# LongAoTianxia/Quantized_ViT

Hardware: AMD Instinct MI355X
Metric: images/sec ViT-B/16 int4 @224 batch 256; % int8-MFMA roofline (higher is better)
Workload: dtype int8; 1 GPU; vit_base_patch16_224 int4w/int8a forward, batch 256 per GPU; model=vit_base_patch16_224, global_batch=256, seq_len=197, parallelism=dp1

## Files before the change

### include/qvit_hip.h

```cpp
#ifndef QVIT_HIP_H
#define QVIT_HIP_H

#include <stdint.h>
#include <hip/hip_runtime_api.h>

#ifdef __cplusplus
extern "C" {
#endif

#define QVIT_OK          0
#define QVIT_EINVAL     -1
#define QVIT_EALIGN     -2
#define QVIT_ENULL      -3
#define QVIT_EHIP    -1000

#define QVIT_QT_LINEAR      0
#define QVIT_QT_NONLINEAR   1
#define QVIT_QT_ULTRA_ACT   2

#define QVIT_W4 4
#define QVIT_W8 8
#define QVIT_W4R 40
#define QVIT_W8R 80
#define QVIT_W16 16
#define QVIT_W24 24

#define QVIT_EPI_F32        0
#define QVIT_EPI_F32_RESID  1
#define QVIT_EPI_I8_GELU    2
#define QVIT_EPI_I8         3
#define QVIT_EPI_I32        4
#define QVIT_EPI_QKV_SPLIT  5

#define QVIT_ULTRA_CODES       0
#define QVIT_ULTRA_CODES_POOL  1
#define QVIT_ULTRA_F32         2

#define QVIT_ATT_F32        0
#define QVIT_ATT_I8         1

#define QVIT_U8_NCHW 0
#define QVIT_U8_NHWC 1

#define QVIT_TILE_N  256
#define QVIT_TILE_K  128

const char* qvit_strerror(int code);
const char* qvit_version(void);

int qvit_quantize_act_i8(const float* x, int64_t rows, int64_t cols, int64_t ldx,
                         int qtype, const float* d_quant, const float* q_m, const float* t_quant,
                         int levels, int8_t* codes, int64_t ldc, int64_t kpad, hipStream_t stream);

int qvit_fake_quant_f32(const float* x, int64_t n, int qtype, const float* d_quant,
                        const float* q_m, const float* t_quant, int levels, float* y,
                        hipStream_t stream);

int64_t qvit_quant_backward_workspace_bytes(int64_t n);
int qvit_quant_backward(const float* x, const float* grad_out, int64_t n, int qtype,
                        const float* d_quant, const float* q_m, const float* t_quant,
                        float clip_lo, float clip_hi, float dge_k,
                        float* grad_x, float* grad_scalars ,
                        void* workspace, int64_t workspace_bytes, hipStream_t stream);

int64_t qvit_quant_error_workspace_bytes(int64_t rows, int64_t cols, int ncand);
int qvit_quant_error(const float* x, int64_t rows, int64_t cols, int64_t ldx, int qtype, const float* d,
                     const float* q_m, const float* t, int ncand, int accumulate, double* err, int64_t* nclip,
                     void* workspace, int64_t workspace_bytes, hipStream_t stream);

#define QVIT_QAT_SGD    0
#define QVIT_QAT_ADAM   1
#define QVIT_QAT_ADAMW  2
#define QVIT_QAT_WARMUP 0
#define QVIT_QAT_RANGE  1
#define QVIT_QAT_FIX    2
int qvit_qat_step(const void* tensors, int ntensors, const void* chunks, int64_t nchunks, int variant,
                  int first_step, float lr, float lr_quant, float first_momentum, float second_momentum,
                  float alpha1, float alpha2, float weight_decay, float bias_correction1, float bias_correction2,
                  float clip_lo, float clip_hi, hipStream_t stream);
int qvit_qat_quant_step(const void* quants, int nquants, int32_t* bits, int stage, int first_fix, int variant,
                        int first_step, float lr, float lr_quant, float first_momentum, float second_momentum,
                        float alpha1, float alpha2, float weight_decay, float bias_correction1,
                        float bias_correction2, float clip_lo, float clip_hi, int min_bit_wt, int max_bit_wt,
                        int min_bit_act, int max_bit_act, hipStream_t stream);

int qvit_prune_scores(const void* groups, int ngroups, const void* members, int nmembers, const void* items,
                      int64_t nitems, double* sums, int variant, int first_step, float lr, float lr_quant,
                      float first_momentum, float second_momentum, float alpha1, float alpha2, float weight_decay,
                      float bias_correction1, float bias_correction2, float clip_lo, float clip_hi,
                      hipStream_t stream);
int qvit_prune_scores_fold(const void* groups, int ngroups, const void* items, int64_t nitems, const double* sums,
                           const void* units, int64_t nunits, double* unit_sums, hipStream_t stream);
int qvit_prune_scores_finish(const void* groups, int ngroups, const void* items, int64_t nitems, const double* sums,
                             double w_magnitude, double w_avg_magnitude, double w_cosine, double w_taylor1,
                             double w_taylor2, float* scores, hipStream_t stream);
int qvit_prune_joint_scalars(const void* quants, int nquants, int variant, int first_step, float lr, float lr_quant,
                             float first_momentum, float second_momentum, float alpha1, float alpha2,
                             float weight_decay, float bias_correction1, float bias_correction2, float clip_lo,
                             float clip_hi, int min_bit_act, int max_bit_act, hipStream_t stream);
int qvit_prune_joint_reduce(const void* groups, int ngroups, const void* members, int nmembers, const void* items,
                            int64_t nitems, double* partials, int variant, int first_step, float lr, float lr_quant,
                            float first_momentum, float second_momentum, float alpha1, float alpha2,
                            float weight_decay, float bias_correction1, float bias_correction2, float clip_lo,
                            float clip_hi, hipStream_t stream);
int qvit_prune_joint_finish(const void* groups, int ngroups, const double* partials, int64_t npartials, double lr,
                            int period, int t_in_period, int min_bit_wt, int max_bit_wt, float* gamma, int32_t* info,
                            hipStream_t stream);
int qvit_prune_joint_apply(const void* groups, int ngroups, const void* members, int nmembers, const void* items,
                           int64_t nitems, const float* gamma, int variant, int first_step, float lr, float lr_quant,
                           float first_momentum, float second_momentum, float alpha1, float alpha2,
                           float weight_decay, float bias_correction1, float bias_correction2, float clip_lo,
                           float clip_hi, hipStream_t stream);

int qvit_gelu_f32(const float* x, int64_t n, float* y, hipStream_t stream);

int64_t qvit_layernorm_quant_backward_workspace_bytes(int64_t rows, int64_t cols);
int qvit_layernorm_quant_backward(const float* x, int64_t rows, int64_t cols, int64_t ldx,
                                  const float* gamma, const float* beta, float eps,
                                  int qtype, const float* d_quant, const float* q_m, const float* t_quant,
                                  float clip_lo, float clip_hi,
                                  const float* grad_y, int64_t ldg, float* grad_x, int64_t ldo,
                                  float* grad_gamma, float* grad_beta, float* grad_scalars ,
                                  void* workspace, int64_t workspace_bytes, hipStream_t stream);
int qvit_gelu_quant_i8(const float* h, int64_t rows, int64_t cols, int64_t ldh, int qtype,
                       const float* d_quant, const float* q_m, const float* t_quant, int levels,
                       int8_t* codes, int64_t ldc, int64_t kpad, hipStream_t stream);
int64_t qvit_gelu_quant_backward_workspace_bytes(int64_t n);
int qvit_gelu_quant_backward(const float* h, const float* grad_y, int64_t n, int qtype,
                             const float* d_quant, const float* q_m, const float* t_quant,
                             float clip_lo, float clip_hi, float* grad_h, float* grad_scalars ,
                             void* workspace, int64_t workspace_bytes, hipStream_t stream);

int qvit_pack_weight(const float* w, int64_t n, int64_t k, int64_t ldw, int qtype,
                     const float* d_quant, const float* q_m, const float* t_quant, int wfmt,
                     void* packed, int64_t npad, int64_t kpad, int32_t* overflow,
                     hipStream_t stream);

int qvit_pack_weight_w4r(const void* packed, int64_t npad, int64_t kpad, void* out, hipStream_t stream);

int qvit_pack_weight_w8r(const void* packed, int64_t npad, int64_t kpad, void* out, hipStream_t stream);

int qvit_pad_bias(const float* bias, int64_t n, float* out, int64_t npad, hipStream_t stream);

int qvit_im2col_quant_i8(const float* x, int64_t B, int64_t C, int64_t H, int64_t W,
                         int kh, int kw, int sh, int sw, int ph, int pw, int dh, int dw,
                         int qtype, const float* d_quant, const float* q_m, const float* t_quant,
                         int levels, int8_t* codes, int64_t ldc, int64_t kpad, hipStream_t stream);

int qvit_im2col_u8_i8(const uint8_t* img, int64_t B, int64_t C, int64_t H, int64_t W, int layout,
                      int kh, int kw, int sh, int sw, int ph, int pw, int dh, int dw,
                      const int8_t* code_table, int8_t* codes, int64_t ldc, int64_t kpad, hipStream_t stream);

int qvit_u8_normalize_f32(const uint8_t* img, int64_t B, int64_t C, int64_t H, int64_t W, int layout,
                          const float* value_table, float* out, hipStream_t stream);

int qvit_layernorm_quant_i8(const float* x, int64_t rows, int64_t cols, int64_t ldx,
                            const float* gamma, const float* beta, float eps,
                            int qtype, const float* d_quant, const float* q_m,
                            const float* t_quant, int levels,
                            int8_t* codes, int64_t ldc, int64_t kpad,
                            const void* code_table, hipStream_t stream);

int qvit_gemm(const int8_t* A, int64_t M, int64_t K, int64_t lda,
              const void* Wp, int wfmt, int64_t N, int64_t npad,
              const float* d_act, const float* d_wt, const float* bias,
              int epilogue, void* C, int64_t ldc,
              int out_qtype, const float* out_d, const float* out_qm, const float* out_t,
              int out_levels, const void* epi_table, hipStream_t stream);

int qvit_layernorm_quant_i8_t32(const float* x, int64_t rows, int64_t cols, int64_t ldx, const float* gamma,
                                const float* beta, float eps, int qtype, const float* d_quant, const float* q_m,
                                const float* t_quant, int levels, int8_t* codes, int64_t kpad,
                                const void* code_table, hipStream_t stream);
int qvit_gemm_a32_fits(int64_t K, int wfmt, int64_t N, int64_t npad, int epilogue);
int qvit_gemm_a32(const int8_t* A, int64_t M, int64_t K, const void* Wp, int wfmt, int64_t N, int64_t npad,
                  const float* d_act, const float* d_wt, const float* bias, int epilogue, void* C, int64_t ldc,
                  int out_qtype, const float* out_d, const float* out_qm, const float* out_t, int out_levels,
                  const void* epi_table, hipStream_t stream);

int qvit_gemm_wonly(const float* X, int64_t M, int64_t K, int64_t ldx, const void* Wp, int wfmt,
                    int64_t N, int64_t npad, const float* d_wt, const float* bias, float* Y, int64_t ldy,
                    float* workspace, int64_t workspace_bytes, hipStream_t stream);

int64_t qvit_gemm_wgrad_workspace_bytes(int64_t M, int64_t N, int64_t K);
int qvit_gemm_wgrad(const float* G, int64_t M, int64_t N, int64_t ldg, const int8_t* A, int64_t K, int64_t lda,
                    const float* d_act, float* dW, int64_t ldw, void* workspace, int64_t workspace_bytes,
                    hipStream_t stream);

int64_t qvit_col2im_quant_backward_workspace_bytes(int64_t B, int64_t C, int64_t H, int64_t W, int kh, int kw,
                                                   int sh, int sw, int ph, int pw, int dh, int dw);
int qvit_col2im_quant_backward(const float* P, int64_t ldp, const float* x, int64_t B, int64_t C, int64_t H,
                               int64_t W, int kh, int kw, int sh, int sw, int ph, int pw, int dh, int dw, int qtype,
                               const float* d_quant, const float* q_m, const float* t_quant, float clip_lo,
                               float clip_hi, float* grad_x, float* grad_scalars , void* workspace,
                               int64_t workspace_bytes, hipStream_t stream);

int qvit_conv_wonly(const float* X, int64_t B, int64_t C, int64_t H, int64_t W, int kh, int kw, int sh, int sw,
                    int ph, int pw, int dh, int dw, const void* Wp, int wfmt, int64_t N, int64_t npad, int64_t K,
                    const float* d_wt, const float* bias, float* Y, float* workspace, int64_t workspace_bytes,
                    hipStream_t stream);
int qvit_conv_wonly_narrow(int enable);

int qvit_conv_wonly_bn_act(const float* X, int64_t B, int64_t C, int64_t H, int64_t W, int kh, int kw, int sh,
                           int sw, int ph, int pw, int dh, int dw, const void* Wp, int wfmt, int64_t N, int64_t npad,
                           int64_t K, const float* d_wt, const float* bias, const float* bn_alpha,
                           const float* bn_shift, int a_levels, float* Y, hipStream_t stream);

int qvit_gemm_resid_ln(const int8_t* A, int64_t M, int64_t K, int64_t lda, const void* Wp, int wfmt,
                       int64_t N, int64_t npad, const float* d_act, const float* d_wt, const float* bias,
                       float* C, int64_t ldc, const float* gamma, const float* beta, float eps,
                       int out_qtype, const float* out_d, const float* out_qm, const float* out_t,
                       int out_levels, const void* ln_table, int8_t* codes, int64_t ldcodes,
                       int64_t kpad_codes, int32_t* counters, hipStream_t stream);

#define QVIT_EPI_TABLE_MAX_NB 3800
#define QVIT_EPI_TABLE_BYTES(nb) ((16 + 8 * (nb) + 1023) / 1024 * 1024)
int qvit_epi_table_build(int epilogue, int out_qtype, const float* out_d, const float* out_qm,
                         const float* out_t, int out_levels, float v_lo, float w, int64_t nb,
                         void* table, hipStream_t stream);

int qvit_ultra_weight_codes(const float* w, int64_t cout, int64_t cin, int64_t ks, int w_bit,
                            int8_t* codes, int64_t kpad, int64_t cout_pad, float* values,
                            unsigned* workspace, hipStream_t stream);
int qvit_ultra_bn_fold(const float* gamma, const float* beta, const float* mean, const float* var,
                       float eps, int64_t n, float* alpha, float* shift, hipStream_t stream);
int qvit_ultra_conv0(const float* img, int64_t B, int64_t H, int64_t W, const float* wvals,
                     const float* alpha, const float* shift, int a_bit, int8_t* out, hipStream_t stream);
int qvit_ultra_conv(const int8_t* in, int64_t B, int64_t H, int64_t W, int64_t cin, int64_t ks,
                    const int8_t* wcodes, int64_t kpad, int64_t cout, int w_bit, int a_bit,
                    const float* alpha, const float* shift, int mode, void* out, int64_t ldo,
                    hipStream_t stream);
int qvit_ultra_tail(const int8_t* in, int64_t B, int64_t H, int64_t W, const int8_t* const* wcodes, int64_t kpad,
                    const float* const* alpha, const float* const* shift, const int8_t* hcodes, int64_t hkpad,
                    const float* hbias, int64_t hout, int w_bit, int a_bit, float* out, int64_t ldo,
                    const float* anchors, int64_t na, int64_t no, float stride, float* io, float* p,
                    hipStream_t stream);

int64_t qvit_ultra_weight_quant_backward_workspace_bytes(int64_t n);
int qvit_ultra_weight_quant_backward(const float* w, const float* grad_out, int64_t n, int w_bit, float* grad_w,
                                     void* workspace, int64_t workspace_bytes, hipStream_t stream);
int qvit_ultra_act_quant_backward(const float* x, const float* grad_out, int64_t n, float* grad_x,
                                  hipStream_t stream);
int64_t qvit_conv_wgrad_workspace_bytes(int64_t B, int64_t C, int64_t H, int64_t W, int64_t N, int kh, int kw,
                                        int sh, int sw, int ph, int pw, int dh, int dw);
int qvit_conv_wgrad(const float* G, const float* X, int64_t B, int64_t C, int64_t H, int64_t W, int64_t N, int kh,
                    int kw, int sh, int sw, int ph, int pw, int dh, int dw, int levels, float* dW, void* workspace,
                    int64_t workspace_bytes, hipStream_t stream);
int64_t qvit_bn_stats_workspace_bytes(int64_t B, int64_t C, int64_t H, int64_t W);
int qvit_bn_stats(const float* x, int64_t B, int64_t C, int64_t H, int64_t W, double eps, double factor,
                  float* running_mean, float* running_var, float* mean, float* var, float* invstd, void* workspace,
                  int64_t workspace_bytes, hipStream_t stream);
int qvit_bn_act_pool_forward(const float* x, int64_t B, int64_t C, int64_t H, int64_t W, const float* mean,
                             const float* invstd, const float* gamma, const float* beta, int levels, int pool,
                             float* out, uint8_t* flags, hipStream_t stream);
int64_t qvit_bn_act_pool_backward_workspace_bytes(int64_t B, int64_t C, int64_t H, int64_t W, int pool);
int qvit_bn_act_pool_backward_reduce(const float* x, const float* grad_out, const uint8_t* flags, int64_t B,
                                     int64_t C, int64_t H, int64_t W, const float* mean, const float* invstd,
                                     int pool, double* sums, void* workspace, int64_t workspace_bytes,
                                     hipStream_t stream);
int qvit_bn_act_pool_backward_dx(const float* x, const float* grad_out, const uint8_t* flags, int64_t B, int64_t C,
                                 int64_t H, int64_t W, const float* mean, const float* invstd, const float* gamma,
                                 const double* sums, int pool, float* dx, float* dgamma, float* dbeta,
                                 hipStream_t stream);
int qvit_ultra_conv0_int(const uint8_t* img, int64_t B, int64_t H, int64_t W, const int8_t* wcodes,
                         const int32_t* inc, const int32_t* bias, int shift_bits, int out_bit, int8_t* out,
                         hipStream_t stream);
int qvit_ultra_conv_int(const int8_t* in, int64_t B, int64_t H, int64_t W, int64_t cin, int64_t ks,
                        const int8_t* wcodes, int64_t kpad, int64_t cout, const int32_t* inc, const int32_t* bias,
                        int shift_bits, int out_bit, int pool, int8_t* out, int64_t ldo, hipStream_t stream);
int qvit_yolo_decode(const float* head, int64_t B, int64_t ny, int64_t nx, int64_t na, int64_t no,
                     int64_t ldh, const float* anchors, float stride, float* io, float* p,
                     hipStream_t stream);

int qvit_attention(const float* qkv, int64_t B, int64_t N, int64_t H, int64_t head_dim, int64_t ldq,
                   float scale, float in_scale, int out_mode, void* out, int64_t ldo,
                   int out_qtype, const float* out_d, const float* out_qm, const float* out_t,
                   int out_levels, hipStream_t stream);

int64_t qvit_attention_backward_workspace_bytes(int64_t B, int64_t N, int64_t H);
int qvit_attention_backward(const float* qkv, const float* out, const float* grad_out, int64_t B, int64_t N,
                            int64_t H, int64_t head_dim, int64_t ldq, int64_t ldo, int64_t ldgo, float scale,
                            float in_scale, float g_scale, float* grad_qkv, int64_t ldg, void* workspace,
                            int64_t workspace_bytes, hipStream_t stream);

int qvit_gemm_qkv_split(const int8_t* A, int64_t M, int64_t K, int64_t lda,
                        const void* Wp, int wfmt, int64_t N, int64_t npad,
                        const float* d_act, const float* d_wt, const float* bias,
                        int64_t seq, float in_scale, void* qkv_hi, void* qkv_lo, hipStream_t stream);

int qvit_gemm_qkv_split_hd(const int8_t* A, int64_t M, int64_t K, int64_t lda,
                           const void* Wp, int wfmt, int64_t N, int64_t npad,
                           const float* d_act, const float* d_wt, const float* bias,
                           int64_t seq, int64_t head_dim, float in_scale, void* qkv_hi, void* qkv_lo,
                           hipStream_t stream);

int qvit_attention_split(const void* qkv_hi, const void* qkv_lo, int64_t B, int64_t N, int64_t H,
                         int64_t head_dim, float scale, float in_scale, int out_mode, void* out,
                         int64_t ldo, int out_qtype, const float* out_d, const float* out_qm,
                         const float* out_t, int out_levels, const void* epi_table, hipStream_t stream);

int qvit_qkv_attention(const int8_t* A, int64_t B, int64_t N, int64_t K, int64_t lda, const void* Wp,
                       int wfmt, int64_t npad, const float* d_act, const float* d_wt, const float* bias,
                       int64_t H, int64_t head_dim, float scale, float in_scale, int out_mode, void* out,
                       int64_t ldo, int out_qtype, const float* out_d, const float* out_qm,
                       const float* out_t, int out_levels, const void* epi_table, hipStream_t stream);

int qvit_qkv_attention_q(const int8_t* A, int64_t B, int64_t N, int64_t NQ, int64_t K, int64_t lda,
                         const void* Wp, int wfmt, int64_t npad, const float* d_act, const float* d_wt,
                         const float* bias, int64_t H, int64_t head_dim, float scale, float in_scale,
                         int out_mode, void* out, int64_t ldo, int out_qtype, const float* out_d,
                         const float* out_qm, const float* out_t, int out_levels, const void* epi_table,
                         hipStream_t stream);

#ifdef __cplusplus
}
#endif
#endif
```

### quantized_vit_amd/_lib.py

```python
from __future__ import annotations

import ctypes
import os
import threading
from typing import Optional, Tuple

import torch

_HERE = os.path.dirname(os.path.abspath(__file__))
LIB_PATH = os.environ.get("QVIT_LIB") or os.path.join(_HERE, "libqvit_hip.so")

QT_LINEAR = 0
QT_NONLINEAR = 1
QT_ULTRA_ACT = 2
QT_FORCE_CAREFUL = 0x100

W4 = 4
W8 = 8
W4R = 40
W8R = 80
W16 = 16
W24 = 24

EPI_F32 = 0
EPI_F32_RESID = 1
EPI_I8_GELU = 2
EPI_I8 = 3
EPI_I32 = 4
EPI_QKV_SPLIT = 5

ATT_F32 = 0
ATT_I8 = 1

ULTRA_CODES = 0
ULTRA_CODES_POOL = 1
ULTRA_F32 = 2

EPI_TABLE_MAX_NB = 3800

QAT_SGD, QAT_ADAM, QAT_ADAMW = 0, 1, 2
QAT_WARMUP, QAT_RANGE, QAT_FIX = 0, 1, 2
QAT_CHUNK = 4096
QAT_TENSOR_BYTES = 48
QAT_QUANT_BYTES = 64
PRUNE_GROUP_BYTES = 64
PRUNE_MEMBER_BYTES = 48
PRUNE_ITEM_BYTES = 16
PRUNE_IMPORTANT, PRUNE_REDUNDANT, PRUNE_PRUNED = 0, 1, 2

U8_NCHW = 0
U8_NHWC = 1
U8_MAX_C = 16

TILE_N = 256
TILE_K = 128

_c_p = ctypes.c_void_p
_i64 = ctypes.c_int64
_i32 = ctypes.c_int
_f32 = ctypes.c_float
_f64 = ctypes.c_double

_SIGNATURES = {
    "qvit_quantize_act_i8": [_c_p, _i64, _i64, _i64, _i32, _c_p, _c_p, _c_p, _i32, _c_p, _i64, _i64, _c_p],
    "qvit_fake_quant_f32": [_c_p, _i64, _i32, _c_p, _c_p, _c_p, _i32, _c_p, _c_p],
    "qvit_quant_backward": [_c_p, _c_p, _i64, _i32, _c_p, _c_p, _c_p, _f32, _f32, _f32, _c_p, _c_p, _c_p, _i64, _c_p],
    "qvit_quant_error": [_c_p, _i64, _i64, _i64, _i32, _c_p, _c_p, _c_p, _i32, _i32, _c_p, _c_p, _c_p, _i64, _c_p],
    "qvit_qat_step": [_c_p, _i32, _c_p, _i64, _i32, _i32] + [_f32] * 11 + [_c_p],
    "qvit_qat_quant_step": [_c_p, _i32, _c_p, _i32, _i32, _i32, _i32] + [_f32] * 11 + [_i32] * 4 + [_c_p],
    "qvit_prune_scores": [_c_p, _i32, _c_p, _i32, _c_p, _i64, _c_p, _i32, _i32] + [_f32] * 11 + [_c_p],
    "qvit_prune_scores_fold": [_c_p, _i32, _c_p, _i64, _c_p, _c_p, _i64, _c_p, _c_p],
    "qvit_prune_scores_finish": [_c_p, _i32, _c_p, _i64, _c_p] + [_f64] * 5 + [_c_p, _c_p],
    "qvit_prune_joint_scalars": [_c_p, _i32, _i32, _i32] + [_f32] * 11 + [_i32, _i32, _c_p],
    "qvit_prune_joint_reduce": [_c_p, _i32, _c_p, _i32, _c_p, _i64, _c_p, _i32, _i32] + [_f32] * 11 + [_c_p],
    "qvit_prune_joint_finish": [_c_p, _i32, _c_p, _i64, _f64, _i32, _i32, _i32, _i32, _c_p, _c_p, _c_p],
    "qvit_prune_joint_apply": [_c_p, _i32, _c_p, _i32, _c_p, _i64, _c_p, _i32, _i32] + [_f32] * 11 + [_c_p],
    "qvit_gelu_f32": [_c_p, _i64, _c_p, _c_p],
    "qvit_layernorm_quant_backward": [_c_p, _i64, _i64, _i64, _c_p, _c_p, _f32, _i32, _c_p, _c_p, _c_p, _f32, _f32,
                                      _c_p, _i64, _c_p, _i64, _c_p, _c_p, _c_p, _c_p, _i64, _c_p],
    "qvit_gelu_quant_i8": [_c_p, _i64, _i64, _i64, _i32, _c_p, _c_p, _c_p, _i32, _c_p, _i64, _i64, _c_p],
    "qvit_gelu_quant_backward": [_c_p, _c_p, _i64, _i32, _c_p, _c_p, _c_p, _f32, _f32, _c_p, _c_p, _c_p, _i64, _c_p],
    "qvit_pack_weight": [_c_p, _i64, _i64, _i64, _i32, _c_p, _c_p, _c_p, _i32, _c_p, _i64, _i64, _c_p, _c_p],
    "qvit_pad_bias": [_c_p, _i64, _c_p, _i64, _c_p],
    "qvit_pack_weight_w4r": [_c_p, _i64, _i64, _c_p, _c_p],
    "qvit_pack_weight_w8r": [_c_p, _i64, _i64, _c_p, _c_p],
    "qvit_im2col_quant_i8": [_c_p, _i64, _i64, _i64, _i64, _i32, _i32, _i32, _i32, _i32, _i32, _i32, _i32,
                             _i32, _c_p, _c_p, _c_p, _i32, _c_p, _i64, _i64, _c_p],
    "qvit_im2col_u8_i8": [_c_p, _i64, _i64, _i64, _i64, _i32, _i32, _i32, _i32, _i32, _i32, _i32, _i32, _i32,
                          _c_p, _c_p, _i64, _i64, _c_p],
    "qvit_u8_normalize_f32": [_c_p, _i64, _i64, _i64, _i64, _i32, _c_p, _c_p, _c_p],
    "qvit_layernorm_quant_i8": [_c_p, _i64, _i64, _i64, _c_p, _c_p, _f32, _i32, _c_p, _c_p, _c_p, _i32,
                                _c_p, _i64, _i64, _c_p, _c_p],
    "qvit_gemm": [_c_p, _i64, _i64, _i64, _c_p, _i32, _i64, _i64, _c_p, _c_p, _c_p, _i32, _c_p, _i64,
                  _i32, _c_p, _c_p, _c_p, _i32, _c_p, _c_p],
    "qvit_layernorm_quant_i8_t32": [_c_p, _i64, _i64, _i64, _c_p, _c_p, _f32, _i32, _c_p, _c_p, _c_p, _i32, _c_p,
                                    _i64, _c_p, _c_p],
    "qvit_gemm_a32_fits": [_i64, _i32, _i64, _i64, _i32],
    "qvit_gemm_a32": [_c_p, _i64, _i64, _c_p, _i32, _i64, _i64, _c_p, _c_p, _c_p, _i32, _c_p, _i64, _i32, _c_p, _c_p,
                      _c_p, _i32, _c_p, _c_p],
    "qvit_gemm_wonly": [_c_p, _i64, _i64, _i64, _c_p, _i32, _i64, _i64, _c_p, _c_p, _c_p, _i64, _c_p, _i64, _c_p],
    "qvit_gemm_wgrad": [_c_p, _i64, _i64, _i64, _c_p, _i64, _i64, _c_p, _c_p, _i64, _c_p, _i64, _c_p],
    "qvit_col2im_quant_backward": [_c_p, _i64, _c_p, _i64, _i64, _i64, _i64, _i32, _i32, _i32, _i32, _i32, _i32, _i32,
                                   _i32, _i32, _c_p, _c_p, _c_p, _f32, _f32, _c_p, _c_p, _c_p, _i64, _c_p],
    "qvit_conv_wonly": [_c_p, _i64, _i64, _i64, _i64, _i32, _i32, _i32, _i32, _i32, _i32, _i32, _i32, _c_p, _i32,
                        _i64, _i64, _i64, _c_p, _c_p, _c_p, _c_p, _i64, _c_p],
    "qvit_conv_wonly_bn_act": [_c_p, _i64, _i64, _i64, _i64, _i32, _i32, _i32, _i32, _i32, _i32, _i32, _i32, _c_p,
                               _i32, _i64, _i64, _i64, _c_p, _c_p, _c_p, _c_p, _i32, _c_p, _c_p],
    "qvit_conv_wonly_narrow": [_i32],
    "qvit_epi_table_build": [_i32, _i32, _c_p, _c_p, _c_p, _i32, _f32, _f32, _i64, _c_p, _c_p],
    "qvit_gemm_resid_ln": [_c_p, _i64, _i64, _i64, _c_p, _i32, _i64, _i64, _c_p, _c_p, _c_p, _c_p, _i64, _c_p, _c_p,
                           _f32, _i32, _c_p, _c_p, _c_p, _i32, _c_p, _c_p, _i64, _i64, _c_p, _c_p],
    "qvit_ultra_weight_codes": [_c_p, _i64, _i64, _i64, _i32, _c_p, _i64, _i64, _c_p, _c_p, _c_p],
    "qvit_ultra_bn_fold": [_c_p, _c_p, _c_p, _c_p, _f32, _i64, _c_p, _c_p, _c_p],
    "qvit_ultra_conv0": [_c_p, _i64, _i64, _i64, _c_p, _c_p, _c_p, _i32, _c_p, _c_p],
    "qvit_ultra_conv": [_c_p, _i64, _i64, _i64, _i64, _i64, _c_p, _i64, _i64, _i32, _i32, _c_p, _c_p, _i32, _c_p,
                        _i64, _c_p],
    "qvit_ultra_tail": [_c_p, _i64, _i64, _i64, _c_p, _i64, _c_p, _c_p, _c_p, _i64, _c_p, _i64, _i32, _i32, _c_p,
                        _i64, _c_p, _i64, _i64, _f32, _c_p, _c_p, _c_p],
    "qvit_ultra_conv0_int": [_c_p, _i64, _i64, _i64, _c_p, _c_p, _c_p, _i32, _i32, _c_p, _c_p],
    "qvit_ultra_conv_int": [_c_p, _i64, _i64, _i64, _i64, _i64, _c_p, _i64, _i64, _c_p, _c_p, _i32, _i32, _i32,
                            _c_p, _i64, _c_p],
    "qvit_yolo_decode": [_c_p, _i64, _i64, _i64, _i64, _i64, _i64, _c_p, _f32, _c_p, _c_p, _c_p],
    "qvit_ultra_weight_quant_backward": [_c_p, _c_p, _i64, _i32, _c_p, _c_p, _i64, _c_p],
    "qvit_ultra_act_quant_backward": [_c_p, _c_p, _i64, _c_p, _c_p],
    "qvit_conv_wgrad": [_c_p, _c_p, _i64, _i64, _i64, _i64, _i64, _i32, _i32, _i32, _i32, _i32, _i32, _i32, _i32,
                        _i32, _c_p, _c_p, _i64, _c_p],
    "qvit_bn_stats": [_c_p, _i64, _i64, _i64, _i64, _f64, _f64, _c_p, _c_p, _c_p, _c_p, _c_p, _c_p, _i64, _c_p],
    "qvit_bn_act_pool_forward": [_c_p, _i64, _i64, _i64, _i64, _c_p, _c_p, _c_p, _c_p, _i32, _i32, _c_p, _c_p, _c_p],
    "qvit_bn_act_pool_backward_reduce": [_c_p, _c_p, _c_p, _i64, _i64, _i64, _i64, _c_p, _c_p, _i32, _c_p, _c_p, _i64,
                                         _c_p],
    "qvit_bn_act_pool_backward_dx": [_c_p, _c_p, _c_p, _i64, _i64, _i64, _i64, _c_p, _c_p, _c_p, _c_p, _i32, _c_p,
                                     _c_p, _c_p, _c_p],
    "qvit_attention": [_c_p, _i64, _i64, _i64, _i64, _i64, _f32, _f32, _i32, _c_p, _i64, _i32, _c_p, _c_p, _c_p,
                       _i32, _c_p],
    "qvit_gemm_qkv_split": [_c_p, _i64, _i64, _i64, _c_p, _i32, _i64, _i64, _c_p, _c_p, _c_p, _i64, _f32, _c_p,
                            _c_p, _c_p],
    "qvit_gemm_qkv_split_hd": [_c_p, _i64, _i64, _i64, _c_p, _i32, _i64, _i64, _c_p, _c_p, _c_p, _i64, _i64, _f32, _c_p,
                               _c_p, _c_p],
    "qvit_qkv_attention": [_c_p, _i64, _i64, _i64, _i64, _c_p, _i32, _i64, _c_p, _c_p, _c_p, _i64, _i64, _f32, _f32,
                           _i32, _c_p, _i64, _i32, _c_p, _c_p, _c_p, _i32, _c_p, _c_p],
    "qvit_qkv_attention_q": [_c_p, _i64, _i64, _i64, _i64, _i64, _c_p, _i32, _i64, _c_p, _c_p, _c_p, _i64, _i64, _f32,
                             _f32, _i32, _c_p, _i64, _i32, _c_p, _c_p, _c_p, _i32, _c_p, _c_p],
    "qvit_attention_split": [_c_p, _c_p, _i64, _i64, _i64, _i64, _f32, _f32, _i32, _c_p, _i64, _i32, _c_p, _c_p,
                             _c_p, _i32, _c_p, _c_p],
    "qvit_attention_backward": [_c_p, _c_p, _c_p, _i64, _i64, _i64, _i64, _i64, _i64, _i64, _f32, _f32, _f32, _c_p,
                                _i64, _c_p, _i64, _c_p],
}
INT64_FUNCS = {
    "qvit_quant_backward_workspace_bytes": [_i64],
    "qvit_quant_error_workspace_bytes": [_i64, _i64, _i32],
    "qvit_layernorm_quant_backward_workspace_bytes": [_i64, _i64],
    "qvit_gelu_quant_backward_workspace_bytes": [_i64],
    "qvit_attention_backward_workspace_bytes": [_i64, _i64, _i64],
    "qvit_gemm_wgrad_workspace_bytes": [_i64, _i64, _i64],
    "qvit_col2im_quant_backward_workspace_bytes": [_i64, _i64, _i64, _i64, _i32, _i32, _i32, _i32, _i32, _i32, _i32,
                                                   _i32],
    "qvit_ultra_weight_quant_backward_workspace_bytes": [_i64],
    "qvit_conv_wgrad_workspace_bytes": [_i64, _i64, _i64, _i64, _i64, _i32, _i32, _i32, _i32, _i32, _i32, _i32, _i32],
    "qvit_bn_stats_workspace_bytes": [_i64, _i64, _i64, _i64],
    "qvit_bn_act_pool_backward_workspace_bytes": [_i64, _i64, _i64, _i64, _i32],
}
STRING_FUNCS = {"qvit_strerror": [_i32], "qvit_version": []}
EXPORTED_SYMBOLS = sorted(list(_SIGNATURES) + list(INT64_FUNCS) + list(STRING_FUNCS))

_lock = threading.Lock()
_lib: Optional[ctypes.CDLL] = None


class QvitError(RuntimeError):
    pass


def load(path: str = LIB_PATH) -> ctypes.CDLL:
    global _lib
    with _lock:
        if _lib is not None:
            return _lib
        if not os.path.exists(path):
            raise QvitError(
                f"{path} is missing: build it with `python -m quantized_vit_amd.build` "
                "(the HIP extension is required; there is no CPU fallback)")
        lib = ctypes.CDLL(path, mode=ctypes.RTLD_GLOBAL)
        for name, args in _SIGNATURES.items():
            if path != LIB_PATH and not hasattr(lib, name):
                continue
            fn = getattr(lib, name)
            fn.argtypes = args
            fn.restype = ctypes.c_int
        for name, args in INT64_FUNCS.items():
            if path != LIB_PATH and not hasattr(lib, name):
                continue
            fn = getattr(lib, name)
            fn.argtypes = args
            fn.restype = ctypes.c_int64
        for name, args in STRING_FUNCS.items():
            fn = getattr(lib, name)
            fn.argtypes = args
            fn.restype = ctypes.c_char_p
        _lib = lib
        return lib


def version() -> str:
    return load().qvit_version().decode()


def build_id(path: Optional[str] = None) -> Optional[str]:
    import hashlib
    p = path or (getattr(_lib, "_name", None) if _lib is not None else None) or LIB_PATH
    try:
        with open(p + ".srcsha") as f:
            digest = f.read().strip()
        if digest:
            return "src-" + digest[:16]
    except OSError:
        pass
    try:
        with open(p, "rb") as f:
            return hashlib.sha256(f.read()).hexdigest()[:16]
    except OSError:
        return None


def _check(code: int, what: str) -> None:
    if code != 0:
        msg = load().qvit_strerror(code).decode()
        raise QvitError(f"{what} failed: {msg} (status {code})")


def _ptr(t: Optional[torch.Tensor]) -> Optional[int]:
    return None if t is None else t.data_ptr()


def _stream(dev: torch.device) -> int:
    return torch.cuda.current_stream(dev).cuda_stream


def _require_gpu(t: torch.Tensor, name: str) -> None:
    if not t.is_cuda:
        raise QvitError(f"{name} must be a ROCm device tensor (got {t.device}); the HIP path has no CPU fallback")


def quantize_act_i8(x2d: torch.Tensor, qtype: int, d: Optional[torch.Tensor], qm: Optional[torch.Tensor],
                    t: Optional[torch.Tensor], levels: int, out: torch.Tensor, kpad: int) -> torch.Tensor:
    _require_gpu(x2d, "input")
    assert x2d.dtype == torch.float32 and x2d.dim() == 2 and x2d.stride(1) == 1
    rows, cols = x2d.shape
    _check(load().qvit_quantize_act_i8(_ptr(x2d), rows, cols, x2d.stride(0), qtype, _ptr(d), _ptr(qm), _ptr(t),
                                       levels, _ptr(out), out.stride(0), kpad, _stream(x2d.device)),
           "qvit_quantize_act_i8")
    return out


def fake_quant_f32(x: torch.Tensor, qtype: int, d: Optional[torch.Tensor], qm: Optional[torch.Tensor],
                   t: Optional[torch.Tensor], levels: int = 0) -> torch.Tensor:
    _require_gpu(x, "input")
    xc = x.contiguous().float()
    y = torch.empty_like(xc)
    _check(load().qvit_fake_quant_f32(_ptr(xc), xc.numel(), qtype, _ptr(d), _ptr(qm), _ptr(t), levels, _ptr(y),
                                      _stream(x.device)), "qvit_fake_quant_f32")
    return y


def quant_backward(x: torch.Tensor, grad_out: torch.Tensor, qtype: int, d: torch.Tensor, qm: torch.Tensor,
                   t: Optional[torch.Tensor], clip_lo: float, clip_hi: float, dge_k: float = 0.0,
                   grad_x: Optional[torch.Tensor] = None):
    _require_gpu(x, "input")
    _require_gpu(grad_out, "grad_out")
    xc = x.detach().contiguous().float()
    gc = grad_out.detach().contiguous().float()
    if xc.numel() != gc.numel():
        raise QvitError(f"quant_backward: grad_out has {gc.numel()} elements for an input of {xc.numel()}")
    if grad_x is None:
        grad_x = torch.empty_like(xc)
    assert grad_x.is_cuda and grad_x.dtype == torch.float32 and grad_x.is_contiguous() and \
        grad_x.numel() == xc.numel()
    n = xc.numel()
    lib = load()
    nbytes = int(lib.qvit_quant_backward_workspace_bytes(n))
    ws = torch.empty(nbytes // 8, dtype=torch.float64, device=xc.device)
    scalars = torch.empty(3, dtype=torch.float32, device=xc.device)
    _check(lib.qvit_quant_backward(_ptr(xc), _ptr(gc), n, qtype, _ptr(d), _ptr(qm), _ptr(t), float(clip_lo),
                                   float(clip_hi), float(dge_k), _ptr(grad_x), _ptr(scalars), _ptr(ws), nbytes,
                                   _stream(xc.device)), "qvit_quant_backward")
    return grad_x, scalars


QUANT_ERROR_MAX_CAND = 64


def quant_error(x2d: torch.Tensor, qtype: int, d: torch.Tensor, q_m: torch.Tensor, t: Optional[torch.Tensor],
                err: Optional[torch.Tensor] = None, nclip: Optional[torch.Tensor] = None, accumulate: bool = False):
    _require_gpu(x2d, "input")
    if x2d.dtype != torch.float32 or x2d.dim() != 2 or (x2d.shape[1] > 1 and x2d.stride(1) != 1):
        raise QvitError(f"quant_error: the input must be a float32 matrix with unit column stride (got {x2d.dtype}, "
                        f"shape {tuple(x2d.shape)}, strides {tuple(x2d.stride())})")
    dev = x2d.device
    ncand = d.numel()
    for name, v in (("d", d), ("q_m", q_m)):
        if not (v.is_cuda and v.dtype == torch.float32 and v.dim() == 1 and v.is_contiguous() and v.numel() == ncand):
            raise QvitError(f"quant_error: {name} must be a contiguous float32 device vector of {ncand} candidates")
    if accumulate and (err is None or nclip is None):
        raise QvitError("quant_error: accumulate needs the err and nclip buffers to add to")
    if err is None:
        err = torch.empty(ncand, dtype=torch.float64, device=dev)
    if nclip is None:
        nclip = torch.empty(ncand, dtype=torch.int64, device=dev)
    for name, v, dt in (("err", err, torch.float64), ("nclip", nclip, torch.int64)):
        if not (v.is_cuda and v.dtype == dt and v.is_contiguous() and v.numel() == ncand):
            raise QvitError(f"quant_error: {name} must be a contiguous {dt} device vector of {ncand} elements")
    rows, cols = x2d.shape
    ldx = x2d.stride(0) if rows > 1 else max(cols, x2d.stride(0))
    lib = load()
    ws = _workspace(int(lib.qvit_quant_error_workspace_bytes(rows, cols, ncand)), "qvit_quant_error_workspace_bytes",
                    None, dev)
    _check(lib.qvit_quant_error(_ptr(x2d) if x2d.numel() else None, rows, cols, ldx, qtype, _ptr(d), _ptr(q_m), _ptr(t),
                                ncand, int(bool(accumulate)), _ptr(err), _ptr(nclip), _ptr(ws),
                                ws.numel() * ws.element_size(), _stream(dev)), "qvit_quant_error")
    return err, nclip


def qat_step(tensors: torch.Tensor, ntensors: int, chunks: torch.Tensor, nchunks: int, hyper: tuple) -> None:
    _require_gpu(tensors, "tensor table")
    _require_gpu(chunks, "chunk list")
    _check(load().qvit_qat_step(_ptr(tensors), ntensors, _ptr(chunks), nchunks, *hyper, _stream(tensors.device)),
           "qvit_qat_step")


def qat_quant_step(quants: torch.Tensor, nquants: int, bits: torch.Tensor, stage: int, first_fix: bool, hyper: tuple,
                   bit_ranges: tuple) -> None:
    _require_gpu(quants, "quantizer table")
    assert bits.is_cuda and bits.dtype == torch.int32 and bits.is_contiguous() and bits.numel() >= nquants
    _check(load().qvit_qat_quant_step(_ptr(quants), nquants, _ptr(bits), stage, int(bool(first_fix)), *hyper,
                                      *bit_ranges, _stream(quants.device)), "qvit_qat_quant_step")


def prune_scores(groups: torch.Tensor, ngroups: int, members: torch.Tensor, nmembers: int, items: torch.Tensor,
                 nitems: int, sums: torch.Tensor, weights: tuple, scores: torch.Tensor, hyper: tuple,
                 units: Optional[torch.Tensor] = None, nunits: int = 0,
                 unit_sums: Optional[torch.Tensor] = None) -> None:
    _require_gpu(groups, "group table")
    nscores = nitems if units is None else nunits
    assert sums.dtype == torch.float64 and sums.numel() >= 3 * nitems and scores.dtype == torch.float32 and \
        scores.numel() >= nscores
    lib, st = load(), _stream(groups.device)
    _check(lib.qvit_prune_scores(_ptr(groups), ngroups, _ptr(members), nmembers, _ptr(items), nitems, _ptr(sums),
                                 *hyper, st), "qvit_prune_scores")
    if units is not None:
        assert unit_sums is not None and unit_sums.dtype == torch.float64 and unit_sums.numel() >= 3 * nunits
        _check(lib.qvit_prune_scores_fold(_ptr(groups), ngroups, _ptr(items), nitems, _ptr(sums), _ptr(units), nunits,
                                          _ptr(unit_sums), st), "qvit_prune_scores_fold")
        items, nitems, sums = units, nunits, unit_sums
    _check(lib.qvit_prune_scores_finish(_ptr(groups), ngroups, _ptr(items), nitems, _ptr(sums),
                                        *[float(w) for w in weights], _ptr(scores), st), "qvit_prune_scores_finish")


def prune_joint_scalars(quants: torch.Tensor, nquants: int, hyper: tuple, min_bit_act: int, max_bit_act: int) -> None:
    _require_gpu(quants, "quantizer table")
    _check(load().qvit_prune_joint_scalars(_ptr(quants), nquants, *hyper, min_bit_act, max_bit_act,
                                           _stream(quants.device)), "qvit_prune_joint_scalars")


def prune_joint_reduce(groups: torch.Tensor, ngroups: int, members: torch.Tensor, nmembers: int, items: torch.Tensor,
                       nitems: int, partials: torch.Tensor, hyper: tuple) -> None:
    _require_gpu(groups, "group table")
    assert partials.dtype == torch.float64 and partials.numel() >= 6 * nitems
    _check(load().qvit_prune_joint_reduce(_ptr(groups), ngroups, _ptr(members), nmembers, _ptr(items), nitems,
                                          _ptr(partials), *hyper, _stream(groups.device)), "qvit_prune_joint_reduce")


def prune_joint_finish(groups: torch.Tensor, ngroups: int, partials: torch.Tensor, npartials: int, lr: float,
                       period: int, t_in_period: int, min_bit_wt: int, max_bit_wt: int, gamma: torch.Tensor,
                       info: torch.Tensor) -> None:
    _require_gpu(groups, "group table")
    assert partials.dtype == torch.float64 and partials.numel() >= 6 * npartials
    assert gamma.dtype == torch.float32 and gamma.numel() >= ngroups and info.dtype == torch.int32 and \
        info.numel() >= ngroups
    _check(load().qvit_prune_joint_finish(_ptr(groups), ngroups, _ptr(partials), npartials, float(lr), period,
                                          t_in_period, min_bit_wt, max_bit_wt, _ptr(gamma), _ptr(info),
                                          _stream(groups.device)), "qvit_prune_joint_finish")


def prune_joint_apply(groups: torch.Tensor, ngroups: int, members: torch.Tensor, nmembers: int, items: torch.Tensor,
                      nitems: int, gamma: torch.Tensor, hyper: tuple) -> None:
    _require_gpu(groups, "group table")
    assert gamma.dtype == torch.float32 and gamma.numel() >= ngroups
    _check(load().qvit_prune_joint_apply(_ptr(groups), ngroups, _ptr(members), nmembers, _ptr(items), nitems,
                                         _ptr(gamma), *hyper, _stream(groups.device)), "qvit_prune_joint_apply")


def gelu_f32(x: torch.Tensor) -> torch.Tensor:
    _require_gpu(x, "input")
    xc = x.contiguous().float()
    y = torch.empty_like(xc)
    _check(load().qvit_gelu_f32(_ptr(xc), xc.numel(), _ptr(y), _stream(x.device)), "qvit_gelu_f32")
    return y


LN_BWD_MAX_COLS = 2048


def _rows_ok(t: torch.Tensor) -> bool:
    return (t.is_cuda and t.dtype == torch.float32 and t.dim() == 2 and t.stride(1) == 1 and t.stride(0) % 4 == 0
            and t.stride(0) >= t.shape[1] and t.data_ptr() % 16 == 0)


def layernorm_quant_backward_fits(x2d: torch.Tensor, gamma: Optional[torch.Tensor],
                                  beta: Optional[torch.Tensor]) -> bool:
    cols = x2d.shape[1] if x2d.dim() == 2 else 0
    vec = lambda v: (v is not None and v.is_cuda and v.dtype == torch.float32 and v.is_contiguous()
                     and v.numel() == cols and v.data_ptr() % 16 == 0)
    return _rows_ok(x2d) and cols % 4 == 0 and 0 < cols <= LN_BWD_MAX_COLS and vec(gamma) and vec(beta)


def layernorm_quant_backward(x2d: torch.Tensor, gamma: torch.Tensor, beta: torch.Tensor, eps: float, qtype: int,
                             d: torch.Tensor, qm: torch.Tensor, t: Optional[torch.Tensor], clip_lo: float,
                             clip_hi: float, grad_y: torch.Tensor, grad_x: Optional[torch.Tensor] = None,
                             want_gamma: bool = True, want_beta: bool = True):
    _require_gpu(x2d, "input")
    _require_gpu(grad_y, "grad_y")
    assert x2d.dtype == torch.float32 and grad_y.dtype == torch.float32 and x2d.dim() == 2
    assert x2d.stride(1) == 1 and grad_y.stride(1) == 1 and tuple(grad_y.shape) == tuple(x2d.shape)
    rows, cols = x2d.shape
    if grad_x is None:
        grad_x = torch.empty((rows, cols), dtype=torch.float32, device=x2d.device)
    assert grad_x.is_cuda and grad_x.dtype == torch.float32 and grad_x.stride(1) == 1 and \
        tuple(grad_x.shape) == (rows, cols)
    lib = load()
    nbytes = int(lib.qvit_layernorm_quant_backward_workspace_bytes(rows, cols))
    if nbytes < 0:
        _check(nbytes, "qvit_layernorm_quant_backward_workspace_bytes")
    ws = torch.empty((nbytes + 7) // 8, dtype=torch.float64, device=x2d.device)
    gg = torch.empty(cols, dtype=torch.float32, device=x2d.device) if want_gamma else None
    gb = torch.empty(cols, dtype=torch.float32, device=x2d.device) if want_beta else None
    scalars = torch.empty(3, dtype=torch.float32, device=x2d.device)
    _check(lib.qvit_layernorm_quant_backward(_ptr(x2d), rows, cols, x2d.stride(0), _ptr(gamma), _ptr(beta),
                                             float(eps), qtype, _ptr(d), _ptr(qm), _ptr(t), float(clip_lo),
                                             float(clip_hi), _ptr(grad_y), grad_y.stride(0), _ptr(grad_x),
                                             grad_x.stride(0), _ptr(gg), _ptr(gb), _ptr(scalars), _ptr(ws),
                                             ws.numel() * 8, _stream(x2d.device)), "qvit_layernorm_quant_backward")
    return grad_x, gg, gb, scalars


def gelu_quant_i8(h2d: torch.Tensor, qtype: int, d: Optional[torch.Tensor], qm: Optional[torch.Tensor],
                  t: Optional[torch.Tensor], levels: int, out: torch.Tensor, kpad: int) -> torch.Tensor:
    _require_gpu(h2d, "input")
    assert h2d.dtype == torch.float32 and h2d.dim() == 2 and h2d.stride(1) == 1
    rows, cols = h2d.shape
    _check(load().qvit_gelu_quant_i8(_ptr(h2d), rows, cols, h2d.stride(0), qtype, _ptr(d), _ptr(qm), _ptr(t), levels,
                                     _ptr(out), out.stride(0), kpad, _stream(h2d.device)), "qvit_gelu_quant_i8")
    return out


def gelu_quant_backward(h: torch.Tensor, grad_y: torch.Tensor, qtype: int, d: torch.Tensor, qm: torch.Tensor,
                        t: Optional[torch.Tensor], clip_lo: float, clip_hi: float,
                        grad_h: Optional[torch.Tensor] = None):
    _require_gpu(h, "input")
    _require_gpu(grad_y, "grad_y")
    assert h.dtype == torch.float32 and grad_y.dtype == torch.float32 and h.is_contiguous() and \
        grad_y.is_contiguous() and h.numel() == grad_y.numel()
    if grad_h is None:
        grad_h = torch.empty_like(h)
    assert grad_h.is_cuda and grad_h.dtype == torch.float32 and grad_h.is_contiguous() and \
        grad_h.numel() == h.numel()
    n = h.numel()
    lib = load()
    nbytes = int(lib.qvit_gelu_quant_backward_workspace_bytes(n))
    ws = torch.empty(nbytes // 8, dtype=torch.float64, device=h.device)
    scalars = torch.empty(3, dtype=torch.float32, device=h.device)
    _check(lib.qvit_gelu_quant_backward(_ptr(h), _ptr(grad_y), n, qtype, _ptr(d), _ptr(qm), _ptr(t), float(clip_lo),
                                        float(clip_hi), _ptr(grad_h), _ptr(scalars), _ptr(ws), nbytes,
                                        _stream(h.device)), "qvit_gelu_quant_backward")
    return grad_h, scalars


def pack_weight(w2d: torch.Tensor, qtype: int, d: torch.Tensor, qm: torch.Tensor, t: Optional[torch.Tensor],
                wfmt: int, npad: int, kpad: int, overflow: Optional[torch.Tensor]) -> torch.Tensor:
    _require_gpu(w2d, "weight")
    assert w2d.dtype == torch.float32 and w2d.stride(1) == 1
    n, k = w2d.shape
    nbytes = npad * kpad // 2 if wfmt == W4 else npad * kpad
    packed = torch.empty(nbytes, dtype=torch.uint8, device=w2d.device)
    _check(load().qvit_pack_weight(_ptr(w2d), n, k, w2d.stride(0), qtype, _ptr(d), _ptr(qm), _ptr(t), wfmt,
                                   _ptr(packed), npad, kpad, _ptr(overflow), _stream(w2d.device)),
           "qvit_pack_weight")
    return packed


def pack_weight_w4r(packed: torch.Tensor, npad: int, kpad: int) -> torch.Tensor:
    _require_gpu(packed, "packed weights")
    assert packed.dtype == torch.uint8 and packed.is_contiguous() and packed.numel() == npad * kpad // 2
    out = torch.empty_like(packed)
    _check(load().qvit_pack_weight_w4r(_ptr(packed), npad, kpad, _ptr(out), _stream(packed.device)),
           "qvit_pack_weight_w4r")
    return out


def pack_weight_w8r(packed: torch.Tensor, npad: int, kpad: int) -> torch.Tensor:
    _require_gpu(packed, "packed weights")
    assert packed.dtype == torch.uint8 and packed.is_contiguous() and packed.numel() == npad * kpad // 2
    out = torch.empty(npad * kpad, dtype=torch.uint8, device=packed.device)
    _check(load().qvit_pack_weight_w8r(_ptr(packed), npad, kpad, _ptr(out), _stream(packed.device)),
           "qvit_pack_weight_w8r")
    return out


def pack_weight_wide(codes: torch.Tensor, npad: int, kpad: int):
    _require_gpu(codes, "weight codes")
    c = codes.detach().float().contiguous()
    cmax = float(c.abs().max()) if c.numel() else 0.0
    if cmax >= 2 ** 23:
        raise QvitError("pack_weight_wide: a weight code reaches 2^23")
    ndig = 2 if cmax <= 32639 else 3
    digits = []
    r = c
    for _ in range(ndig):
        d = torch.remainder(r + 128.0, 256.0) - 128.0
        digits.append(d)
        r = (r - d) / 256.0
    if float(r.abs().max()) if r.numel() else 0.0:
        raise QvitError("pack_weight_wide: codes do not fit the digits")
    one = torch.ones(1, device=c.device)
    big = torch.full((1,), 1024.0, device=c.device)
    ovf = torch.zeros(1, dtype=torch.int32, device=c.device)
    imgs = [pack_weight(d.contiguous(), QT_LINEAR, one, big, None, W8, npad, kpad, ovf) for d in reversed(digits)]
    if int(ovf.item()) != 0:
        raise QvitError("pack_weight_wide: a digit left the int8 range")
    return torch.cat(imgs), (W16 if ndig == 2 else W24)


def pad_bias(bias: Optional[torch.Tensor], n: int, npad: int, device: torch.device) -> torch.Tensor:
    out = torch.empty(npad, dtype=torch.float32, device=device)
    b = None if bias is None else bias.detach().contiguous().float()
    _check(load().qvit_pad_bias(_ptr(b), n, _ptr(out), npad, _stream(device)), "qvit_pad_bias")
    return out


def im2col_quant_i8(x: torch.Tensor, kh: int, kw: int, sh: int, sw: int, ph: int, pw: int, dh: int, dw: int,
                    qtype: int, d, qm, t, levels: int, out: torch.Tensor, kpad: int) -> torch.Tensor:
    _require_gpu(x, "input")
    assert x.dtype == torch.float32 and x.is_contiguous() and x.dim() == 4
    B, C, H, W = x.shape
    _check(load().qvit_im2col_quant_i8(_ptr(x), B, C, H, W, kh, kw, sh, sw, ph, pw, dh, dw, qtype, _ptr(d),
                                       _ptr(qm), _ptr(t), levels, _ptr(out), out.stride(0), kpad,
                                       _stream(x.device)), "qvit_im2col_quant_i8")
    return out


def u8_image_layout(img: torch.Tensor) -> Tuple[torch.Tensor, int]:
    assert img.dtype == torch.uint8 and img.dim() == 4
    if img.is_contiguous():
        return img, U8_NCHW
    if img.is_contiguous(memory_format=torch.channels_last):
        return img, U8_NHWC
    return img.contiguous(), U8_NCHW


def im2col_u8_i8(img: torch.Tensor, kh: int, kw: int, sh: int, sw: int, ph: int, pw: int, dh: int, dw: int,
                 code_table: torch.Tensor, out: torch.Tensor, kpad: int) -> torch.Tensor:
    _require_gpu(img, "input")
    img, layout = u8_image_layout(img)
    B, C, H, W = img.shape
    assert code_table.dtype == torch.int8 and code_table.is_contiguous() and tuple(code_table.shape) == (C, 256)
    _check(load().qvit_im2col_u8_i8(_ptr(img), B, C, H, W, layout, kh, kw, sh, sw, ph, pw, dh, dw, _ptr(code_table),
                                    _ptr(out), out.stride(0), kpad, _stream(img.device)), "qvit_im2col_u8_i8")
    return out


def u8_normalize_f32(img: torch.Tensor, value_table: torch.Tensor) -> torch.Tensor:
    _require_gpu(img, "input")
    img, layout = u8_image_layout(img)
    B, C, H, W = img.shape
    assert value_table.dtype == torch.float32 and value_table.is_contiguous() and \
        tuple(value_table.shape) == (C, 256)
    out = torch.empty((B, C, H, W), dtype=torch.float32, device=img.device)
    _check(load().qvit_u8_normalize_f32(_ptr(img), B, C, H, W, layout, _ptr(value_table), _ptr(out),
                                        _stream(img.device)), "qvit_u8_normalize_f32")
    return out


def layernorm_quant_i8(x2d: torch.Tensor, gamma: Optional[torch.Tensor], beta: Optional[torch.Tensor], eps: float,
                       qtype: int, d, qm, t, levels: int, out: torch.Tensor, kpad: int,
                       code_table: Optional[torch.Tensor] = None) -> torch.Tensor:
    _require_gpu(x2d, "input")
    assert x2d.dtype == torch.float32 and x2d.stride(1) == 1
    rows, cols = x2d.shape
    _check(load().qvit_layernorm_quant_i8(_ptr(x2d), rows, cols, x2d.stride(0), _ptr(gamma), _ptr(beta), eps, qtype,
                                          _ptr(d), _ptr(qm), _ptr(t), levels, _ptr(out), out.stride(0), kpad,
                                          _ptr(code_table), _stream(x2d.device)), "qvit_layernorm_quant_i8")
    return out


def gemm(A: torch.Tensor, M: int, K: int, packed: torch.Tensor, wfmt: int, N: int, npad: int,
         d_act: Optional[torch.Tensor], d_wt: Optional[torch.Tensor], bias_pad: Optional[torch.Tensor],
         epilogue: int, C: torch.Tensor, out_qtype: int = 0, out_d=None, out_qm=None, out_t=None,
         out_levels: int = 0, epi_table: Optional[torch.Tensor] = None) -> torch.Tensor:
    _require_gpu(A, "codes")
    _check(load().qvit_gemm(_ptr(A), M, K, A.stride(0), _ptr(packed), wfmt, N, npad, _ptr(d_act), _ptr(d_wt),
                            _ptr(bias_pad), epilogue, _ptr(C), C.stride(0), out_qtype, _ptr(out_d), _ptr(out_qm),
                            _ptr(out_t), out_levels, _ptr(epi_table), _stream(A.device)), "qvit_gemm")
    return C


def t32_rows(M: int) -> int:
    return (M + 63) // 64 * 64


def t32_to_rows(codes_t32: torch.Tensor, M: int, kpad: int) -> torch.Tensor:
    R = t32_rows(M)
    t = codes_t32.view(-1)[:R * kpad].view(R // 32, kpad // 32, 2, 32, 16)
    return t.permute(0, 3, 1, 2, 4).reshape(R, kpad)[:M]


def rows_to_t32(codes: torch.Tensor, kpad: int) -> torch.Tensor:
    M = codes.shape[0]
    R = t32_rows(M)
    full = torch.zeros((R, kpad), dtype=torch.int8, device=codes.device)
    full[:M] = codes[:, :kpad]
    return full.view(R // 32, 32, kpad // 32, 2, 16).permute(0, 2, 3, 1, 4).contiguous().view(-1)


def layernorm_quant_i8_t32(x2d: torch.Tensor, gamma: Optional[torch.Tensor], beta: Optional[torch.Tensor], eps: float,
                           qtype: int, d, qm, t, levels: int, out: torch.Tensor, kpad: int,
                           code_table: Optional[torch.Tensor] = None) -> torch.Tensor:
    _require_gpu(x2d, "input")
    assert x2d.dtype == torch.float32 and x2d.stride(1) == 1
    rows, cols = x2d.shape
    assert out.numel() >= t32_rows(rows) * kpad
    _check(load().qvit_layernorm_quant_i8_t32(_ptr(x2d), rows, cols, x2d.stride(0), _ptr(gamma), _ptr(beta), eps,
                                              qtype, _ptr(d), _ptr(qm), _ptr(t), levels, _ptr(out), kpad,
                                              _ptr(code_table), _stream(x2d.device)), "qvit_layernorm_quant_i8_t32")
    return out


def gemm_a32_fits(K: int, wfmt: int, N: int, npad: int, epilogue: int) -> bool:
    lib = load()
    if not hasattr(lib, "qvit_gemm_a32_fits"):
        return False
    return bool(lib.qvit_gemm_a32_fits(K, wfmt, N, npad, epilogue))


def gemm_a32(A: torch.Tensor, M: int, K: int, packed: torch.Tensor, wfmt: int, N: int, npad: int, d_act, d_wt,
             bias_pad: Optional[torch.Tensor], epilogue: int, C: torch.Tensor, out_qtype: int = 0, out_d=None,
             out_qm=None, out_t=None, out_levels: int = 0, epi_table: Optional[torch.Tensor] = None) -> torch.Tensor:
    _require_gpu(A, "codes")
    assert A.numel() >= t32_rows(M) * K
    _check(load().qvit_gemm_a32(_ptr(A), M, K, _ptr(packed), wfmt, N, npad, _ptr(d_act), _ptr(d_wt), _ptr(bias_pad),
                                epilogue, _ptr(C), C.stride(0), out_qtype, _ptr(out_d), _ptr(out_qm), _ptr(out_t),
                                out_levels, _ptr(epi_table), _stream(A.device)), "qvit_gemm_a32")
    return C


WONLY_WS_MAX = 64 << 20


def wonly_workspace(device: torch.device, M: int, npad: int) -> Optional[torch.Tensor]:
    need = min(256 * M * npad * 4, WONLY_WS_MAX)
    return torch.empty(need // 4 + 4, dtype=torch.float32, device=device)


def gemm_wonly(X: torch.Tensor, M: int, K: int, packed: torch.Tensor, wfmt: int, N: int, npad: int,
               d_wt: torch.Tensor, bias_pad: Optional[torch.Tensor], Y: torch.Tensor, split: bool = True) -> torch.Tensor:
    _require_gpu(X, "activations")
    small = (npad // 256) * ((M + 63) // 64) < 128
    ws = wonly_workspace(X.device, M, npad) if (split and small) else None
    _check(load().qvit_gemm_wonly(_ptr(X), M, K, X.stride(0), _ptr(packed), wfmt, N, npad, _ptr(d_wt),
                                  _ptr(bias_pad), _ptr(Y), Y.stride(0), _ptr(ws), 0 if ws is None else ws.numel() * 4,
                                  _stream(X.device)), "qvit_gemm_wonly")
    return Y


def gemm_wgrad_splits(M: int, N: int, K: int) -> int:
    r = lambda v: (v + 127) // 128 * 128
    nbytes = int(load().qvit_gemm_wgrad_workspace_bytes(M, N, K))
    if nbytes < 0:
        raise QvitError(f"qvit_gemm_wgrad_workspace_bytes({M}, {N}, {K}) failed (status {nbytes})")
    return nbytes // (r(N) * r(K) * 4)


def gemm_wgrad(G: torch.Tensor, codes: torch.Tensor, K: int, d_act: torch.Tensor,
               out: Optional[torch.Tensor] = None, workspace: Optional[torch.Tensor] = None) -> torch.Tensor:
    _require_gpu(G, "grad_out")
    _require_gpu(codes, "codes")
    assert G.dim() == 2 and codes.dim() == 2 and codes.dtype == torch.int8 and codes.shape[0] == G.shape[0]
    assert codes.shape[1] >= K >= 1
    M, N = G.shape
    if G.dtype != torch.float32 or G.stride(1) != 1 or G.stride(0) % 4 or G.stride(0) < N or G.data_ptr() % 16:
        gp = torch.zeros((M, (N + 3) // 4 * 4), dtype=torch.float32, device=G.device)
        gp[:, :N] = G
        G = gp
    if codes.stride(1) != 1 or codes.stride(0) % 16 or codes.stride(0) < K or codes.data_ptr() % 16:
        cp = torch.zeros((M, (K + 15) // 16 * 16), dtype=torch.int8, device=codes.device)
        cp[:, :K] = codes[:, :K]
        codes = cp
    if out is None:
        out = torch.empty((N, K), dtype=torch.float32, device=G.device)
    assert out.dtype == torch.float32 and out.shape[0] == N and out.shape[1] >= K and out.stride(1) == 1
    if M == 0:
        out[:, :K] = 0
        return out
    lib = load()
    nbytes = int(lib.qvit_gemm_wgrad_workspace_bytes(M, N, K))
    if nbytes < 0:
        _check(nbytes, "qvit_gemm_wgrad_workspace_bytes")
    if workspace is None:
        workspace = torch.empty(nbytes // 4, dtype=torch.float32, device=G.device)
    _check(lib.qvit_gemm_wgrad(_ptr(G), M, N, G.stride(0), _ptr(codes), K, codes.stride(0), _ptr(d_act), _ptr(out),
                               out.stride(0), _ptr(workspace), workspace.numel() * workspace.element_size(),
                               _stream(G.device)), "qvit_gemm_wgrad")
    return out


def conv_out_hw(H: int, W: int, kernel_size, stride, padding, dilation) -> Tuple[int, int]:
    (kh, kw), (sh, sw), (ph, pw), (dh, dw) = kernel_size, stride, padding, dilation
    return (H + 2 * ph - dh * (kh - 1) - 1) // sh + 1, (W + 2 * pw - dw * (kw - 1) - 1) // sw + 1


def col2im_quant_backward(P: torch.Tensor, x: Optional[torch.Tensor], xshape, kernel_size, stride, padding, dilation,
                          qtype: int = QT_LINEAR, d: Optional[torch.Tensor] = None, qm: Optional[torch.Tensor] = None,
                          t: Optional[torch.Tensor] = None, clip_lo: float = 0.0, clip_hi: float = 0.0,
                          grad_x: Optional[torch.Tensor] = None, workspace: Optional[torch.Tensor] = None):
    _require_gpu(P, "P")
    B, C, H, W = (int(v) for v in xshape)
    (kh, kw), (sh, sw), (ph, pw), (dh, dw) = kernel_size, stride, padding, dilation
    geo = (B, C, H, W, kh, kw, sh, sw, ph, pw, dh, dw)
    OH, OW = conv_out_hw(H, W, kernel_size, stride, padding, dilation)
    K = C * kh * kw
    if P.dim() != 2 or P.shape[0] != B * OH * OW or P.shape[1] < K:
        raise QvitError(f"col2im_quant_backward: P of shape {tuple(P.shape)} for {B * OH * OW} patch rows of {K}")
    if P.dtype != torch.float32 or P.stride(1) != 1 or (P.shape[0] > 1 and P.stride(0) < K):
        P = P.detach().float().contiguous()
    dev = P.device
    if x is not None:
        _require_gpu(x, "input")
        x = x.detach()
        if x.dtype != torch.float32 or not x.is_contiguous():
            x = x.float().contiguous()
        if tuple(x.shape) != (B, C, H, W):
            raise QvitError(f"col2im_quant_backward: input of shape {tuple(x.shape)} for an image of {(B, C, H, W)}")
    if grad_x is None:
        grad_x = torch.empty((B, C, H, W), dtype=torch.float32, device=dev)
    assert grad_x.is_cuda and grad_x.dtype == torch.float32 and grad_x.is_contiguous() and \
        tuple(grad_x.shape) == (B, C, H, W)
    lib = load()
    scalars, nbytes = None, 0
    if x is not None:
        nbytes = int(lib.qvit_col2im_quant_backward_workspace_bytes(*geo))
        workspace = _workspace(nbytes, "qvit_col2im_quant_backward_workspace_bytes", workspace, dev)
        nbytes = workspace.numel() * workspace.element_size()
        scalars = torch.empty(3, dtype=torch.float32, device=dev)
    ldp = P.stride(0) if P.shape[0] > 1 else max(P.shape[1], 1)
    _check(lib.qvit_col2im_quant_backward(_ptr(P), ldp, _ptr(x), *geo, qtype, _ptr(d), _ptr(qm), _ptr(t),
                                          float(clip_lo), float(clip_hi), _ptr(grad_x), _ptr(scalars),
                                          _ptr(workspace) if x is not None else None, nbytes, _stream(dev)),
           "qvit_col2im_quant_backward")
    return grad_x, scalars


def conv_wonly(x: torch.Tensor, kernel_size, stride, padding, dilation, packed: torch.Tensor, wfmt: int, N: int,
               npad: int, kpad: int, d_wt: torch.Tensor, bias_pad: Optional[torch.Tensor],
               split: bool = True) -> torch.Tensor:
    _require_gpu(x, "activations")
    if x.dtype != torch.float32 or not x.is_contiguous():
        x = x.float().contiguous()
    B, C, H, W = x.shape
    (kh, kw), (sh, sw), (ph, pw), (dh, dw) = kernel_size, stride, padding, dilation
    OH, OW = conv_out_hw(H, W, kernel_size, stride, padding, dilation)
    y = torch.empty((B, N, OH, OW), dtype=torch.float32, device=x.device)
    M = B * OH * OW
    small = split and (npad // 256) * ((M + 63) // 64) < 128 and not narrow_conv_fits(wfmt, N, C * kh * kw, H, W)
    ws = wonly_workspace(x.device, M, npad) if small else None
    _check(load().qvit_conv_wonly(_ptr(x), B, C, H, W, kh, kw, sh, sw, ph, pw, dh, dw, _ptr(packed), wfmt, N, npad,
                                  kpad, _ptr(d_wt), _ptr(bias_pad), _ptr(y), _ptr(ws),
                                  0 if ws is None else ws.numel() * 4, _stream(x.device)), "qvit_conv_wonly")
    return y


def conv_wonly_bn_act(x: torch.Tensor, kernel_size, stride, padding, dilation, packed: torch.Tensor, wfmt: int,
                      N: int, npad: int, kpad: int, d_wt: torch.Tensor, bias_pad: Optional[torch.Tensor],
                      bn_alpha: torch.Tensor, bn_shift: torch.Tensor, a_levels: int) -> Optional[torch.Tensor]:
    _require_gpu(x, "activations")
    (kh, kw), (sh, sw), (ph, pw), (dh, dw) = kernel_size, stride, padding, dilation
    if not narrow_conv_fits(wfmt, N, x.shape[1] * kh * kw, x.shape[2], x.shape[3]):
        return None
    if x.dtype != torch.float32 or not x.is_contiguous():
        x = x.float().contiguous()
    B, C, H, W = x.shape
    OH, OW = conv_out_hw(H, W, kernel_size, stride, padding, dilation)
    y = torch.empty((B, N, OH, OW), dtype=torch.float32, device=x.device)
    _check(load().qvit_conv_wonly_bn_act(_ptr(x), B, C, H, W, kh, kw, sh, sw, ph, pw, dh, dw, _ptr(packed), wfmt, N,
                                       npad, kpad, _ptr(d_wt), _ptr(bias_pad), _ptr(bn_alpha), _ptr(bn_shift),
                                       a_levels, _ptr(y), _stream(x.device)), "qvit_conv_wonly_bn_act")
    return y


NARROW_W_MAX = 24 * 1024
NARROW_K_MAX = 1024


def narrow_conv_fits(wfmt: int, N: int, kreal: int, H: int = 0, W: int = 0) -> bool:
    if N > 64 or wfmt not in (W4, W8) or not conv_wonly_narrow(-1) or H >= 32767 or W >= 32767:
        return False
    nke = (kreal + 63) // 64
    return (nke * 64 <= NARROW_K_MAX
            and nke * 16 * ((N + 15) // 16) * (32 if wfmt == W4 else 64) <= NARROW_W_MAX)


def conv_wonly_narrow(enable: int = -1) -> bool:
    return bool(load().qvit_conv_wonly_narrow(int(enable)))


def resid_ln_counters(device: torch.device, rows: int, npad: int) -> torch.Tensor:
    return torch.empty(max((rows + 127) // 128, 1), dtype=torch.int32, device=device)


def gemm_resid_ln(A: torch.Tensor, M: int, K: int, packed: torch.Tensor, wfmt: int, N: int, npad: int,
                  d_act, d_wt, bias_pad, C: torch.Tensor, gamma, beta, eps: float, out_qtype: int, out_d, out_qm,
                  out_t, out_levels: int, ln_table, codes: torch.Tensor, kpad_codes: int) -> torch.Tensor:
    _require_gpu(A, "codes")
    cnt = resid_ln_counters(A.device, M, npad)
    _check(load().qvit_gemm_resid_ln(_ptr(A), M, K, A.stride(0), _ptr(packed), wfmt, N, npad, _ptr(d_act),
                                     _ptr(d_wt), _ptr(bias_pad), _ptr(C), C.stride(0), _ptr(gamma), _ptr(beta), eps,
                                     out_qtype, _ptr(out_d), _ptr(out_qm), _ptr(out_t), out_levels, _ptr(ln_table),
                                     _ptr(codes), codes.stride(0), kpad_codes, _ptr(cnt), _stream(A.device)),
           "qvit_gemm_resid_ln")
    return codes


def epi_table_build(epilogue: int, out_qtype: int, out_d, out_qm, out_t, out_levels: int, v_lo: float, w: float,
                    nb: int, device: torch.device) -> torch.Tensor:
    table = torch.zeros((16 + 8 * nb + 1023) // 1024 * 1024, dtype=torch.uint8, device=device)
    _check(load().qvit_epi_table_build(epilogue, out_qtype, _ptr(out_d), _ptr(out_qm), _ptr(out_t), out_levels,
                                       v_lo, w, nb, _ptr(table), _stream(device)), "qvit_epi_table_build")
    return table


def attention(qkv: torch.Tensor, B: int, N: int, H: int, head_dim: int, scale: float, out: torch.Tensor,
              out_mode: int = ATT_F32, in_scale: float = 1.0, out_qtype: int = 0, out_d=None, out_qm=None,
              out_t=None, out_levels: int = 0) -> torch.Tensor:
    _require_gpu(qkv, "qkv")
    assert qkv.dtype == torch.float32 and qkv.stride(1) == 1
    _check(load().qvit_attention(_ptr(qkv), B, N, H, head_dim, qkv.stride(0), scale, in_scale, out_mode, _ptr(out),
                                 out.stride(0), out_qtype, _ptr(out_d), _ptr(out_qm), _ptr(out_t), out_levels,
                                 _stream(qkv.device)), "qvit_attention")
    return out


def attention_backward_workspace_bytes(B: int, N: int, H: int) -> int:
    return int(load().qvit_attention_backward_workspace_bytes(B, N, H))


def attention_backward(qkv: torch.Tensor, out: torch.Tensor, grad_out: torch.Tensor, B: int, N: int, H: int,
                       head_dim: int, scale: float, in_scale: float = 1.0, g_scale: float = 1.0,
                       grad_qkv: Optional[torch.Tensor] = None) -> torch.Tensor:
    for t, name in ((qkv, "qkv"), (out, "out"), (grad_out, "grad_out")):
        _require_gpu(t, name)
        assert t.dtype == torch.float32 and t.dim() == 2 and t.stride(1) == 1 and t.shape[0] == B * N, name
    if grad_qkv is None:
        grad_qkv = torch.empty((B * N, 3 * H * head_dim), dtype=torch.float32, device=qkv.device)
    _require_gpu(grad_qkv, "grad_qkv")
    assert grad_qkv.dtype == torch.float32 and grad_qkv.dim() == 2 and grad_qkv.stride(1) == 1
    lib = load()
    nbytes = int(lib.qvit_attention_backward_workspace_bytes(B, N, H))
    if nbytes < 0:
        _check(nbytes, "qvit_attention_backward_workspace_bytes")
    ws = torch.empty(max(nbytes, 16) // 4, dtype=torch.float32, device=qkv.device)
    _check(lib.qvit_attention_backward(_ptr(qkv), _ptr(out), _ptr(grad_out), B, N, H, head_dim, qkv.stride(0),
                                       out.stride(0), grad_out.stride(0), scale, in_scale, g_scale, _ptr(grad_qkv),
                                       grad_qkv.stride(0), _ptr(ws), nbytes, _stream(qkv.device)),
           "qvit_attention_backward")
    return grad_qkv


def gemm_qkv_split(A: torch.Tensor, M: int, K: int, packed: torch.Tensor, wfmt: int, N: int, npad: int,
                   d_act: torch.Tensor, d_wt: torch.Tensor, bias_pad: Optional[torch.Tensor], seq: int,
                   in_scale: float, hi: torch.Tensor, lo: torch.Tensor, head_dim: int = 64):
    _require_gpu(A, "codes")
    assert hi.dtype == torch.float16 and lo.dtype == torch.float16 and hi.is_contiguous() and lo.is_contiguous()
    assert hi.numel() >= M * N and lo.numel() >= M * N
    if head_dim != 64:
        _check(load().qvit_gemm_qkv_split_hd(_ptr(A), M, K, A.stride(0), _ptr(packed), wfmt, N, npad, _ptr(d_act),
                                             _ptr(d_wt), _ptr(bias_pad), seq, head_dim, in_scale, _ptr(hi), _ptr(lo),
                                             _stream(A.device)), "qvit_gemm_qkv_split_hd")
        return hi, lo
    _check(load().qvit_gemm_qkv_split(_ptr(A), M, K, A.stride(0), _ptr(packed), wfmt, N, npad, _ptr(d_act),
                                      _ptr(d_wt), _ptr(bias_pad), seq, in_scale, _ptr(hi), _ptr(lo),
                                      _stream(A.device)), "qvit_gemm_qkv_split")
    return hi, lo


def attention_split(hi: torch.Tensor, lo: torch.Tensor, B: int, N: int, H: int, head_dim: int, scale: float,
                    out: torch.Tensor, out_mode: int = ATT_F32, in_scale: float = 1.0, out_qtype: int = 0,
                    out_d=None, out_qm=None, out_t=None, out_levels: int = 0,
                    epi_table: Optional[torch.Tensor] = None) -> torch.Tensor:
    _require_gpu(hi, "qkv_hi")
    assert hi.dtype == torch.float16 and lo.dtype == torch.float16
    assert hi.numel() >= B * 3 * H * N * head_dim and lo.numel() >= B * 3 * H * N * head_dim
    _check(load().qvit_attention_split(_ptr(hi), _ptr(lo), B, N, H, head_dim, scale, in_scale, out_mode, _ptr(out),
                                       out.stride(0), out_qtype, _ptr(out_d), _ptr(out_qm), _ptr(out_t), out_levels,
                                       _ptr(epi_table), _stream(hi.device)), "qvit_attention_split")
    return out


QKV_ATT_MAX_N = 208
QKV_ATT_MAX_C = 768


def qkv_attention(codes: torch.Tensor, B: int, N: int, K: int, packed: torch.Tensor, npad: int,
                  d_act: torch.Tensor, d_wt: torch.Tensor, bias_pad: Optional[torch.Tensor], H: int, scale: float,
                  out: torch.Tensor, out_mode: int = ATT_F32, in_scale: float = 1.0, out_qtype: int = 0,
                  out_d=None, out_qm=None, out_t=None, out_levels: int = 0,
                  epi_table: Optional[torch.Tensor] = None, wfmt: int = W4) -> torch.Tensor:
    _require_gpu(codes, "codes")
    _check(load().qvit_qkv_attention(_ptr(codes), B, N, K, codes.stride(0), _ptr(packed), wfmt, npad, _ptr(d_act),
                                     _ptr(d_wt), _ptr(bias_pad), H, 64, scale, in_scale, out_mode, _ptr(out),
                                     out.stride(0), out_qtype, _ptr(out_d), _ptr(out_qm), _ptr(out_t), out_levels,
                                     _ptr(epi_table), _stream(codes.device)), "qvit_qkv_attention")
    return out


QKV_ATT_MAX_NQ = 32


def qkv_attention_q(codes: torch.Tensor, B: int, N: int, NQ: int, K: int, packed: torch.Tensor, npad: int,
                    d_act: torch.Tensor, d_wt: torch.Tensor, bias_pad: Optional[torch.Tensor], H: int, scale: float,
                    out: torch.Tensor, out_mode: int = ATT_F32, in_scale: float = 1.0, out_qtype: int = 0,
                    out_d=None, out_qm=None, out_t=None, out_levels: int = 0,
                    epi_table: Optional[torch.Tensor] = None, wfmt: int = W4) -> torch.Tensor:
    _require_gpu(codes, "codes")
    _check(load().qvit_qkv_attention_q(_ptr(codes), B, N, NQ, K, codes.stride(0), _ptr(packed), wfmt, npad,
                                       _ptr(d_act), _ptr(d_wt), _ptr(bias_pad), H, 64, scale, in_scale, out_mode,
                                       _ptr(out), out.stride(0), out_qtype, _ptr(out_d), _ptr(out_qm), _ptr(out_t),
                                       out_levels, _ptr(epi_table), _stream(codes.device)), "qvit_qkv_attention_q")
    return out


def ultra_weight_codes(w: torch.Tensor, w_bit: int, kpad: int, cout_pad: int, values: bool = False):
    _require_gpu(w, "weight")
    w = w.detach().float().contiguous()
    cout, cin, ks, ks2 = w.shape
    assert ks == ks2
    codes = torch.empty((cout_pad, kpad), dtype=torch.int8, device=w.device)
    vals = torch.empty_like(w) if values else None
    ws = torch.empty(1, dtype=torch.int32, device=w.device)
    _check(load().qvit_ultra_weight_codes(_ptr(w), cout, cin, ks, w_bit, _ptr(codes), kpad, cout_pad, _ptr(vals),
                                          _ptr(ws), _stream(w.device)), "qvit_ultra_weight_codes")
    return (codes, vals) if values else codes


def ultra_bn_fold(bn, device) -> tuple:
    n = bn.num_features
    alpha = torch.empty(n, device=device)
    shift = torch.empty(n, device=device)
    g = bn.weight.detach().float().contiguous() if bn.weight is not None else None
    b = bn.bias.detach().float().contiguous() if bn.bias is not None else None
    _check(load().qvit_ultra_bn_fold(_ptr(g), _ptr(b), _ptr(bn.running_mean), _ptr(bn.running_var), float(bn.eps), n,
                                     _ptr(alpha), _ptr(shift), _stream(device)), "qvit_ultra_bn_fold")
    return alpha, shift


def ultra_conv0(img: torch.Tensor, wvals: torch.Tensor, alpha, shift, a_bit: int) -> torch.Tensor:
    _require_gpu(img, "image")
    assert img.dtype == torch.float32 and img.is_contiguous() and img.shape[1] == 3
    assert wvals.shape == (16, 3, 3, 3) and wvals.is_contiguous()
    B, _, H, W = img.shape
    out = torch.empty((B, H // 2, W // 2, 16), dtype=torch.int8, device=img.device)
    _check(load().qvit_ultra_conv0(_ptr(img), B, H, W, _ptr(wvals), _ptr(alpha), _ptr(shift), a_bit, _ptr(out),
                                   _stream(img.device)), "qvit_ultra_conv0")
    return out


def ultra_conv(x: torch.Tensor, ks: int, wcodes: torch.Tensor, cout: int, w_bit: int, a_bit: int, alpha, shift,
               mode: int) -> torch.Tensor:
    _require_gpu(x, "codes")
    assert x.dtype == torch.int8 and x.is_contiguous()
    B, H, W, cin = x.shape
    if mode == ULTRA_CODES_POOL:
        out = torch.empty((B, H // 2, W // 2, cout), dtype=torch.int8, device=x.device)
    elif mode == ULTRA_CODES:
        out = torch.empty((B, H, W, cout), dtype=torch.int8, device=x.device)
    else:
        out = torch.empty((B, H, W, cout), dtype=torch.float32, device=x.device)
    _check(load().qvit_ultra_conv(_ptr(x), B, H, W, cin, ks, _ptr(wcodes), wcodes.shape[1], cout, w_bit, a_bit,
                                  _ptr(alpha), _ptr(shift), mode, _ptr(out), cout, _stream(x.device)),
           "qvit_ultra_conv")
    return out


def ultra_tail(x: torch.Tensor, wcodes, alphas, shifts, hcodes: torch.Tensor, hbias: torch.Tensor, hout: int,
               w_bit: int, a_bit: int, decode=None):
    _require_gpu(x, "codes")
    assert x.dtype == torch.int8 and x.is_contiguous() and x.shape[3] == 64
    B, H, W, _ = x.shape
    arr = lambda ts: (ctypes.c_void_p * 4)(*[t.data_ptr() for t in ts])
    if decode is None:
        out = torch.empty((B, H, W, hout), dtype=torch.float32, device=x.device)
        io = p = anchors = None
        na = no = 0
        stride = 0.0
    else:
        anchors, na, no, stride = decode
        out = None
        io = torch.empty((B, na, H, W, no), device=x.device)
        p = torch.empty_like(io)
    _check(load().qvit_ultra_tail(_ptr(x), B, H, W, arr(wcodes), wcodes[0].shape[1], arr(alphas), arr(shifts),
                                  _ptr(hcodes), hcodes.shape[1], _ptr(hbias), hout, w_bit, a_bit, _ptr(out), hout,
                                  _ptr(anchors), na, no, float(stride), _ptr(io), _ptr(p), _stream(x.device)),
           "qvit_ultra_tail")
    return out if decode is None else (io.view(B, -1, no), p)


def ultra_conv0_int(img_u8: torch.Tensor, wcodes: torch.Tensor, inc: torch.Tensor, bias: torch.Tensor,
                    shift_bits: int, out_bit: int) -> torch.Tensor:
    _require_gpu(img_u8, "image")
    assert img_u8.dtype == torch.uint8 and img_u8.is_contiguous() and img_u8.shape[1] == 3
    assert wcodes.shape == (16, 3, 3, 3) and wcodes.dtype == torch.int8 and wcodes.is_contiguous()
    assert inc.dtype == torch.int32 and bias.dtype == torch.int32 and inc.numel() >= 16 and bias.numel() >= 16
    B, _, H, W = img_u8.shape
    out = torch.empty((B, H // 2, W // 2, 16), dtype=torch.int8, device=img_u8.device)
    _check(load().qvit_ultra_conv0_int(_ptr(img_u8), B, H, W, _ptr(wcodes), _ptr(inc), _ptr(bias), shift_bits,
                                       out_bit, _ptr(out), _stream(img_u8.device)), "qvit_ultra_conv0_int")
    return out


def ultra_conv_int(x: torch.Tensor, ks: int, wcodes: torch.Tensor, cout: int, inc: torch.Tensor, bias: torch.Tensor,
                   shift_bits: int, out_bit: int, pool: bool) -> torch.Tensor:
    _require_gpu(x, "codes")
    assert x.dtype == torch.int8 and x.is_contiguous()
    assert inc.dtype == torch.int32 and bias.dtype == torch.int32 and inc.numel() >= cout and bias.numel() >= cout
    B, H, W, cin = x.shape
    shape = (B, H // 2, W // 2, cout) if pool else (B, H, W, cout)
    out = torch.empty(shape, dtype=torch.int8, device=x.device)
    _check(load().qvit_ultra_conv_int(_ptr(x), B, H, W, cin, ks, _ptr(wcodes), wcodes.shape[1], cout, _ptr(inc),
                                      _ptr(bias), shift_bits, out_bit, 1 if pool else 0, _ptr(out), cout,
                                      _stream(x.device)), "qvit_ultra_conv_int")
    return out


def yolo_decode(head: torch.Tensor, na: int, no: int, anchors: torch.Tensor, stride: float):
    _require_gpu(head, "head")
    B, ny, nx, C = head.shape
    io = torch.empty((B, na, ny, nx, no), device=head.device)
    p = torch.empty_like(io)
    _check(load().qvit_yolo_decode(_ptr(head), B, ny, nx, na, no, C, _ptr(anchors), stride, _ptr(io), _ptr(p),
                                   _stream(head.device)), "qvit_yolo_decode")
    return io.view(B, -1, no), p


def ultra_weight_quant_backward(w: torch.Tensor, grad_out: torch.Tensor, w_bit: int,
                                grad_w: Optional[torch.Tensor] = None) -> torch.Tensor:
    _require_gpu(w, "weight")
    _require_gpu(grad_out, "grad_out")
    wc = w.detach().contiguous().float()
    gc = grad_out.detach().contiguous().float()
    if wc.numel() != gc.numel():
        raise QvitError(f"ultra_weight_quant_backward: grad_out has {gc.numel()} elements for {wc.numel()} weights")
    if grad_w is None:
        grad_w = torch.empty_like(wc)
    assert grad_w.is_cuda and grad_w.dtype == torch.float32 and grad_w.is_contiguous() and \
        grad_w.numel() == wc.numel()
    n = wc.numel()
    lib = load()
    nbytes = int(lib.qvit_ultra_weight_quant_backward_workspace_bytes(n))
    ws = torch.empty(nbytes // 8, dtype=torch.float64, device=wc.device)
    _check(lib.qvit_ultra_weight_quant_backward(_ptr(wc), _ptr(gc), n, w_bit, _ptr(grad_w), _ptr(ws), nbytes,
                                                _stream(wc.device)), "qvit_ultra_weight_quant_backward")
    return grad_w


def ultra_act_quant_backward(x: torch.Tensor, grad_out: torch.Tensor,
                             grad_x: Optional[torch.Tensor] = None) -> torch.Tensor:
    _require_gpu(x, "input")
    _require_gpu(grad_out, "grad_out")
    xc = x.detach().contiguous().float()
    gc = grad_out.detach().contiguous().float()
    if xc.numel() != gc.numel():
        raise QvitError(f"ultra_act_quant_backward: grad_out has {gc.numel()} elements for an input of {xc.numel()}")
    if xc.data_ptr() % 16:
        xc = xc.clone()
    if gc.data_ptr() % 16:
        gc = gc.clone()
    if grad_x is None:
        grad_x = torch.empty_like(xc)
    assert grad_x.is_cuda and grad_x.dtype == torch.float32 and grad_x.is_contiguous() and \
        grad_x.numel() == xc.numel()
    if xc.numel():
        _check(load().qvit_ultra_act_quant_backward(_ptr(xc), _ptr(gc), xc.numel(), _ptr(grad_x),
                                                    _stream(xc.device)), "qvit_ultra_act_quant_backward")
    return grad_x


def conv_wgrad(G: torch.Tensor, x: torch.Tensor, kernel_size, stride, padding, dilation, levels: int,
               out: Optional[torch.Tensor] = None, workspace: Optional[torch.Tensor] = None) -> torch.Tensor:
    _require_gpu(G, "grad_out")
    _require_gpu(x, "input")
    assert G.dim() == 4 and x.dim() == 4 and G.shape[0] == x.shape[0]
    if G.dtype != torch.float32 or not G.is_contiguous():
        G = G.float().contiguous()
    if x.dtype != torch.float32 or not x.is_contiguous():
        x = x.float().contiguous()
    B, C, H, W = x.shape
    N = G.shape[1]
    (kh, kw), (sh, sw), (ph, pw), (dh, dw) = kernel_size, stride, padding, dilation
    OH, OW = conv_out_hw(H, W, kernel_size, stride, padding, dilation)
    if tuple(G.shape) != (B, N, OH, OW):
        raise QvitError(f"conv_wgrad: grad_out {tuple(G.shape)} for an output of {(B, N, OH, OW)}")
    if out is None:
        out = torch.empty((N, C, kh, kw), dtype=torch.float32, device=G.device)
    assert out.dtype == torch.float32 and out.is_contiguous() and tuple(out.shape) == (N, C, kh, kw)
    if B == 0:
        return out.zero_()
    lib = load()
    nbytes = int(lib.qvit_conv_wgrad_workspace_bytes(B, C, H, W, N, kh, kw, sh, sw, ph, pw, dh, dw))
    if nbytes < 0:
        _check(nbytes, "qvit_conv_wgrad_workspace_bytes")
    if workspace is None:
        workspace = torch.empty(nbytes // 4, dtype=torch.float32, device=G.device)
    _check(lib.qvit_conv_wgrad(_ptr(G), _ptr(x), B, C, H, W, N, kh, kw, sh, sw, ph, pw, dh, dw, int(levels),
                               _ptr(out), _ptr(workspace), workspace.numel() * workspace.element_size(),
                               _stream(G.device)), "qvit_conv_wgrad")
    return out


def _f32c(t: torch.Tensor, name: str) -> torch.Tensor:
    _require_gpu(t, name)
    t = t.detach()
    return t if t.dtype == torch.float32 and t.is_contiguous() else t.float().contiguous()


def _workspace(nbytes: int, what: str, workspace: Optional[torch.Tensor], dev) -> torch.Tensor:
    if nbytes < 0:
        _check(nbytes, what)
    if workspace is None:
        workspace = torch.empty(nbytes // 8, dtype=torch.float64, device=dev)
    return workspace


def bn_stats(x: torch.Tensor, eps: float, factor: float = 0.0, running_mean: Optional[torch.Tensor] = None,
             running_var: Optional[torch.Tensor] = None, workspace: Optional[torch.Tensor] = None):
    x = _f32c(x, "input")
    B, C, H, W = x.shape
    lib = load()
    ws = _workspace(int(lib.qvit_bn_stats_workspace_bytes(B, C, H, W)), "qvit_bn_stats_workspace_bytes", workspace,
                    x.device)
    for r in (running_mean, running_var):
        assert r is None or (r.is_cuda and r.dtype == torch.float32 and r.is_contiguous() and r.numel() == C)
    stats = torch.empty((3, C), dtype=torch.float32, device=x.device)
    _check(lib.qvit_bn_stats(_ptr(x), B, C, H, W, float(eps), float(factor), _ptr(running_mean), _ptr(running_var),
                             _ptr(stats[0]), _ptr(stats[1]), _ptr(stats[2]), _ptr(ws),
                             ws.numel() * ws.element_size(), _stream(x.device)), "qvit_bn_stats")
    return stats[0], stats[1], stats[2]


def bn_act_pool_forward(x: torch.Tensor, mean: torch.Tensor, invstd: torch.Tensor, gamma: Optional[torch.Tensor],
                        beta: Optional[torch.Tensor], levels: int, pool: bool):
    x = _f32c(x, "input")
    B, C, H, W = x.shape
    shape = (B, C, H // 2, W // 2) if pool else (B, C, H, W)
    out = torch.empty(shape, dtype=torch.float32, device=x.device)
    flags = torch.empty(shape, dtype=torch.uint8, device=x.device)
    gamma = None if gamma is None else _f32c(gamma, "gamma")
    beta = None if beta is None else _f32c(beta, "beta")
    _check(load().qvit_bn_act_pool_forward(_ptr(x), B, C, H, W, _ptr(mean), _ptr(invstd), _ptr(gamma), _ptr(beta),
                                           int(levels), int(bool(pool)), _ptr(out), _ptr(flags), _stream(x.device)),
           "qvit_bn_act_pool_forward")
    return out, flags


def bn_act_pool_backward(x: torch.Tensor, grad_out: torch.Tensor, flags: torch.Tensor, mean: torch.Tensor,
                         invstd: torch.Tensor, gamma: Optional[torch.Tensor], pool: bool, want_dgamma: bool = True,
                         want_dbeta: bool = True, workspace: Optional[torch.Tensor] = None):
    x = _f32c(x, "input")
    g = _f32c(grad_out, "grad_out")
    B, C, H, W = x.shape
    pool = int(bool(pool))
    if tuple(g.shape) != tuple(flags.shape) or tuple(g.shape) != ((B, C, H // 2, W // 2) if pool else (B, C, H, W)):
        raise QvitError(f"bn_act_pool_backward: grad_out {tuple(g.shape)}, flags {tuple(flags.shape)} for an input "
                        f"of {tuple(x.shape)}, pool {pool}")
    lib = load()
    ws = _workspace(int(lib.qvit_bn_act_pool_backward_workspace_bytes(B, C, H, W, pool)),
                    "qvit_bn_act_pool_backward_workspace_bytes", workspace, x.device)
    sums = torch.empty((2, C), dtype=torch.float64, device=x.device)
    _check(lib.qvit_bn_act_pool_backward_reduce(_ptr(x), _ptr(g), _ptr(flags), B, C, H, W, _ptr(mean), _ptr(invstd),
                                                pool, _ptr(sums), _ptr(ws), ws.numel() * ws.element_size(),
                                                _stream(x.device)), "qvit_bn_act_pool_backward_reduce")
    dx = torch.empty_like(x)
    dgamma = torch.empty(C, dtype=torch.float32, device=x.device) if want_dgamma else None
    dbeta = torch.empty(C, dtype=torch.float32, device=x.device) if want_dbeta else None
    gamma = None if gamma is None else _f32c(gamma, "gamma")
    _check(lib.qvit_bn_act_pool_backward_dx(_ptr(x), _ptr(g), _ptr(flags), B, C, H, W, _ptr(mean), _ptr(invstd),
                                            _ptr(gamma), _ptr(sums), pool, _ptr(dx), _ptr(dgamma), _ptr(dbeta),
                                            _stream(x.device)), "qvit_bn_act_pool_backward_dx")
    return dx, dgamma, dbeta, sums
```

### quantized_vit_amd/csrc/gemm_w4a8.hip

```cpp
#include <cmath>
#include <cstddef>
#include <type_traits>

#include "diag_stamps.h"
#include "ln_common.h"
#include "qvit_common.h"

namespace {

typedef int v4i __attribute__((ext_vector_type(4)));

constexpr int EPI_RESID_LN = 16;
constexpr int EPI_QKV_SPLIT80 = 17;
constexpr bool is_qkv_split(int epi) { return epi == QVIT_EPI_QKV_SPLIT || epi == EPI_QKV_SPLIT80; }

constexpr int BN = 256;
constexpr int BK = 64;
constexpr int KTILE = 128;
constexpr int RING = 3;
#ifndef QVIT_GEMM_ALEAD
#define QVIT_GEMM_ALEAD 2
#endif
constexpr int ALEAD = QVIT_GEMM_ALEAD;
static_assert(ALEAD == 2 || ALEAD == 3, "the tail steps are written out for 2 or 3");
constexpr int EPI_LD = 68;
constexpr int EPI_ROWS = 16;
constexpr int EPI_WAVE_BYTES = EPI_ROWS * EPI_LD * 4;

template <int WFMT, int WM>
struct Geo {
  static constexpr int NT = 256 * WM;
  static constexpr int NWAVES = 4 * WM;
  static constexpr int BM = 128 * WM;
  static constexpr int XBYTES = BM * BK;
  static constexpr int WROW = (WFMT == QVIT_W4) ? BK / 2 : BK;
  static constexpr int WBYTES = BN * WROW;
  static constexpr int STAGE = XBYTES + WBYTES;
  static constexpr int RING_BYTES = RING * STAGE;
  static constexpr int EPI_BYTES = NWAVES * EPI_WAVE_BYTES;
  static constexpr int BIAS_BYTES = BN * 4;
  static constexpr int QP_BYTES = 64;
  static constexpr int LDS = RING_BYTES + EPI_BYTES + BIAS_BYTES + QP_BYTES;
  static constexpr int XPIECES = XBYTES / 1024 / NWAVES;
  static constexpr int WPIECES = WBYTES / 1024 / NWAVES;
  static constexpr int DMA_PER_STAGE = XPIECES + WPIECES;
  static constexpr int MIN_BLOCKS = (WFMT == QVIT_W4 && WM == 1) ? 2 : 1;
  static constexpr int TABLE_MAX_NB = (EPI_BYTES - 16) / 8;
};

QVIT_DEV uint32_t nib16_lo(uint32_t p) { return (p << 4) & 0xF0F0F0F0u; }
QVIT_DEV uint32_t nib16_hi(uint32_t p) { return p & 0xF0F0F0F0u; }

QVIT_DEV void ldw32(v4i& a, v4i& b, const void* sbase, uint32_t voff) {
  asm volatile("; qvit_asm_load\n\t"
               "global_load_dwordx4 %0, %2, %3\n\t"
               "global_load_dwordx4 %1, %2, %3 offset:16"
               : "=&v"(a), "=&v"(b)
               : "v"(voff), "s"(sbase)
               : "memory");
}

QVIT_DEV void ldw64(v4i& a, v4i& b, v4i& c, v4i& d, const void* sbase, uint32_t voff) {
  asm volatile("; qvit_asm_load\n\t"
               "global_load_dwordx4 %0, %4, %5\n\t"
               "global_load_dwordx4 %1, %4, %5 offset:16\n\t"
               "global_load_dwordx4 %2, %4, %5 offset:32\n\t"
               "global_load_dwordx4 %3, %4, %5 offset:48"
               : "=&v"(a), "=&v"(b), "=&v"(c), "=&v"(d)
               : "v"(voff), "s"(sbase)
               : "memory");
}

__global__ void pack_w4r_kernel(const int8_t* __restrict__ src, int8_t* __restrict__ dst, int64_t nunits) {
  const int64_t u = (int64_t)blockIdx.x * blockDim.x + threadIdx.x;
  if (u >= nunits) return;
  const int64_t c = u >> 10;
  const int w = (int)(u >> 8) & 3, ln = (int)(u >> 2) & 63, r = (int)u & 3;
  const int lfr = ln & 15, lfq = ln >> 4;
  const int row = 64 * w + 16 * r + lfr;
  *reinterpret_cast<uint2*>(dst + c * 8192 + w * 2048 + ln * 32 + r * 8) =
      *reinterpret_cast<const uint2*>(src + c * 8192 + row * 32 + ((lfq ^ (((lfr >> 3) & 1) << 1)) << 3));
}

__global__ void pack_w8r_kernel(const int8_t* __restrict__ src, int8_t* __restrict__ dst, int64_t nunits) {
  const int64_t u = (int64_t)blockIdx.x * blockDim.x + threadIdx.x;
  if (u >= nunits) return;
  const int64_t c = u >> 10;
  const int w = (int)(u >> 8) & 3, ln = (int)(u >> 2) & 63, r = (int)u & 3;
  const int lfr = ln & 15, lfq = ln >> 4;
  const int row = 64 * w + 16 * r + lfr;
  const uint2 p = *reinterpret_cast<const uint2*>(src + c * 8192 + row * 32 + ((lfq ^ (((lfr >> 3) & 1) << 1)) << 3));
  *reinterpret_cast<uint4*>(dst + c * 16384 + w * 4096 + ln * 64 + r * 16) =
      make_uint4(nib16_lo(p.x), nib16_hi(p.x), nib16_lo(p.y), nib16_hi(p.y));
}

template <int N>
QVIT_DEV void stage_sync() {
  __builtin_amdgcn_s_waitcnt(0xC07F);
  asm volatile("s_waitcnt vmcnt(%0)\n\ts_barrier" ::"n"(N) : "memory");
}

struct EpiArgs {
  const float* d_act;
  const float* d_wt;
  const float* bias;
  int out_qtype;
  const float* out_d;
  const float* out_qm;
  const float* out_t;
  int out_levels;
  const int8_t* table;
  int seq;
  float inv_seq;
  float in_scale;
  _Float16* lo;
  const float* ln_gamma;
  const float* ln_beta;
  float ln_eps;
  const int8_t* ln_table;
  int8_t* ln_codes;
  int64_t ln_ldc;
  int ln_kpad;
  int* ln_cnt;
};

QVIT_DEV float epi_F(float v, int gelu, const QParams& qp) { return quant_code(gelu ? gelu_ref(v) : v, qp); }

QVIT_DEV int fkey(float f) {
  const int i = __float_as_int(f);
  return i >= 0 ? i : (int)(0x80000000u - (unsigned)i);
}
QVIT_DEV float funkey(int k) { return __int_as_float(k >= 0 ? k : (int)(0x80000000u - (unsigned)k)); }

__global__ void epi_table_kernel(int gelu, int out_qtype, const float* out_d, const float* out_qm, const float* out_t,
                                 int out_levels, float c0, float inv_w, int nb, int8_t* table) {
  const QParams qp = load_qparams(out_qtype, out_d, out_qm, out_t, out_levels);
  EpiTableHdr* hdr = reinterpret_cast<EpiTableHdr*>(table);
  EpiTableEnt* ent = reinterpret_cast<EpiTableEnt*>(table + sizeof(EpiTableHdr));
  const int j = blockIdx.x * blockDim.x + threadIdx.x;
  const float C = c0 + 8388608.f;
  const float top = epi_top(nb);
  if (j == 0) {
    hdr->c0 = C;
    hdr->inv_w = inv_w;
    hdr->nb = nb;
  }
  if (j >= nb) return;
  auto first_at_least = [&](int b) {
    int lo = fkey(-3.0e38f), hi = fkey(3.0e38f);
    while (lo < hi) {
      const int mid = lo + ((hi - lo) >> 1);
      if (epi_bucket(funkey(mid), C, inv_w, top) >= b) hi = mid;
      else lo = mid + 1;
    }
    return lo;
  };
  const int ks = (j == 0) ? fkey(-3.0e38f) : first_at_least(j);
  const int ke = (j == nb - 1) ? fkey(3.0e38f) : first_at_least(j + 1) - 1;
  const float cs = epi_F(funkey(ks), gelu, qp), ce = epi_F(funkey(ke), gelu, qp);
  bool ok = fabsf(cs - ce) <= 1.f && !(isnan(cs) || isnan(ce));
  float thr = INFINITY;
  if (cs != ce) {
    int lo = ks, hi = ke;
    while (lo < hi) {
      const int mid = lo + ((hi - lo) >> 1);
      if (epi_F(funkey(mid), gelu, qp) != cs) hi = mid;
      else lo = mid + 1;
    }
    thr = funkey(lo);
  }
  if (j == 0 || j == nb - 1) {
    const float far = epi_F(j == 0 ? -1.0e30f : 1.0e30f, gelu, qp);
    if (far != (j == 0 ? cs : ce)) ok = false;
  }
  EpiTableEnt e;
  e.thr = thr;
  e.lo = to_i8_sat(cs);
  e.hi = to_i8_sat(ce);
  e.pad = 0;
  if (j == 0) {
    if (cs != ce) {
      ok = false;
    } else {
      e.thr = -INFINITY;
      e.lo = to_i8_sat(epi_F(NAN, gelu, qp));
    }
  }
  ent[j] = e;
  if (!ok) atomicAnd(&hdr->valid, 0);
}


template <int WFMT>
struct Frags {
  v4i x[8];
  uint2 w4[4];
  v4i wq[4];
  v4i w8[4];
};

template <bool SC1>
QVIT_DEV void st_resid(float* dst, float4 o, const float* C0, int M, int64_t ldc) {
  if constexpr (SC1) {
    typedef float f4v __attribute__((ext_vector_type(4)));
    const __amdgpu_buffer_rsrc_t r = __builtin_amdgcn_make_buffer_rsrc(const_cast<float*>(C0), (short)0,
                                                                        (int)((int64_t)M * ldc * 4), 0x00020000);
    __builtin_amdgcn_raw_buffer_store_b128(f4v{o.x, o.y, o.z, o.w}, r, (int)((dst - C0) * 4), 0, 16);
  } else {
    *reinterpret_cast<float4*>(dst) = o;
  }
}

template <int WFMT, int EPI, int WM, int RW, bool L2 = false>
__global__ __launch_bounds__((Geo<WFMT, WM>::NT), (Geo<WFMT, WM>::MIN_BLOCKS)) void gemm_kernel(
    const int8_t* __restrict__ A, int M, int K, int64_t lda, const int8_t* __restrict__ Wp, int N, int npad,
    void* __restrict__ C, int64_t ldc, EpiArgs ep) {
  using G = Geo<WFMT, WM>;
  constexpr int BM = G::BM;
  constexpr int XBYTES = G::XBYTES;
  constexpr bool I8OUT = (EPI == QVIT_EPI_I8 || EPI == QVIT_EPI_I8_GELU);
  static_assert(!L2 || RW != 0, "the two-ahead activation ring is for register weights");
  constexpr int RINGN = L2 ? ALEAD + 2 : RING;
  constexpr int SLOT = L2 ? XBYTES : G::STAGE;
  constexpr int RING_B = RINGN * SLOT;
  __shared__ __attribute__((aligned(16))) int8_t smem[RING_B + G::EPI_BYTES + G::BIAS_BYTES + G::QP_BYTES];
  int8_t* epi_lds = smem + RING_B;
  const float* bias_l = reinterpret_cast<const float*>(smem + RING_B + G::EPI_BYTES);
  QParams* qp_l = reinterpret_cast<QParams*>(smem + RING_B + G::EPI_BYTES + G::BIAS_BYTES);
  const bool has_bias = (EPI != QVIT_EPI_I32) && ep.bias != nullptr;
  constexpr bool REGW = RW != 0;
  static_assert(!RW || (WFMT == QVIT_W4 && WM == 1), "register weights: the W4 4-wave tile");
  constexpr int WREG = RW == 2 ? 4 : 2;
  constexpr int WIMG = RW == 2 ? 2 * G::WBYTES : G::WBYTES;

  const int tid = threadIdx.x;
  const int lane = tid & 63;
  const int wave = __builtin_amdgcn_readfirstlane(tid >> 6);
  const int wn = wave & 3;
  const int wm = wave >> 2;
  const int fr = lane & 15;
  const int fq = lane >> 4;

  const int nb_n = npad / BN;
  const int ntiles = nb_n * ((M + BM - 1) / BM);
  const int xcd = blockIdx.x & 7, slot = blockIdx.x >> 3, team = gridDim.x >> 3;
  const int per = ntiles >> 3, rem = ntiles & 7;
  const int lo = xcd * per + (xcd < rem ? xcd : rem);
  const int hi = lo + per + (xcd < rem ? 1 : 0);
  int t = lo + slot;
  if (t >= hi) return;

  float alpha = 0.f;
  if (EPI != QVIT_EPI_I32) alpha = (*ep.d_act) * (*ep.d_wt) * (WFMT == QVIT_W4 ? 0.0625f : 1.f);
  bool use_table = false;
  float t_c0 = 0.f, t_invw = 0.f, t_top = 0.f;
  int t_nb = 1;
  if (I8OUT && ep.table != nullptr) {
    const EpiTableHdr h = *reinterpret_cast<const EpiTableHdr*>(ep.table);
    use_table = h.valid != 0 && h.nb <= G::TABLE_MAX_NB;
    t_c0 = h.c0;
    t_invw = h.inv_w;
    t_nb = h.nb;
    t_top = epi_top(h.nb);
    if (use_table) {
      const v4i* src = reinterpret_cast<const v4i*>(ep.table);
      for (int i = tid; i < (16 + 8 * t_nb + 15) / 16; i += G::NT) reinterpret_cast<v4i*>(epi_lds)[i] = src[i];
    }
  }
  if (I8OUT && !use_table && tid == 0) *qp_l = load_qparams(ep.out_qtype, ep.out_d, ep.out_qm, ep.out_t, ep.out_levels);

  constexpr int WROWS_PER_PIECE = 1024 / G::WROW;
  constexpr int WROWS_PER_WAVE = BN / G::NWAVES;
  const int nk = K / BK;
  constexpr bool PEEL = !I8OUT && RW != 2;
  uint32_t wlane = 0;
  auto tile_w = [&](int tt) -> uint32_t {
    return __builtin_amdgcn_readfirstlane((uint32_t)(tt % nb_n) * (uint32_t)(nk * WIMG));
  };
  auto tile_m0 = [&](int tt) -> int { return __builtin_amdgcn_readfirstlane((tt / nb_n) * BM); };
  auto lane_a = [&](int ln) -> uint32_t {
    return (uint32_t)(ln >> 2) * (uint32_t)lda + (uint32_t)(((ln & 3) ^ (((ln >> 4) & 1) << 1)) << 4);
  };
  uint32_t alane = 0;
  const uint32_t lds0 = lds_addr(smem);
  auto issue = [&](int m0, uint32_t wt, int kt, int rslot) __attribute__((always_inline)) {
    const uint32_t sx = lds0 + (uint32_t)(rslot * SLOT);
    const uint32_t sw = sx + XBYTES;
    if (m0 + BM <= M) {
      const int8_t* abase = A + (int64_t)(m0 + 32 * wave) * lda + kt * BK;
#pragma unroll
      for (int j = 0; j < G::XPIECES; ++j)
        dma16s(abase + (int64_t)(16 * j) * lda, alane, __builtin_amdgcn_readfirstlane(sx + (32 * wave + 16 * j) * BK));
    } else {
      const int ln = lane_opaque();
#pragma unroll
      for (int j = 0; j < G::XPIECES; ++j) {
        const int row = 32 * wave + 16 * j + (ln >> 2);
        int gm = m0 + row;
        gm = gm < M ? gm : M - 1;
        const uint32_t a = (uint32_t)gm * (uint32_t)lda + (uint32_t)(((ln & 3) ^ (((row >> 2) & 1) << 1)) * 16);
        dma16s(A + kt * BK, a, __builtin_amdgcn_readfirstlane(sx + (32 * wave + 16 * j) * BK));
      }
    }
    if constexpr (!REGW) {
      const uint32_t wl = wlane;
      const int8_t* wbase = Wp + wt + (uint32_t)kt * G::WBYTES + (uint32_t)(wave * (G::WPIECES * 1024));
#pragma unroll
      for (int j = 0; j < G::WPIECES; ++j)
        dma16s(wbase + j * 1024, wl, __builtin_amdgcn_readfirstlane(sw + (WROWS_PER_WAVE * wave + WROWS_PER_PIECE * j) * G::WROW));
    }
  };
  auto issue_w = [&](uint32_t wt, int kt, Frags<WFMT>& f) __attribute__((always_inline)) {
    if constexpr (RW == 1) {
      const int8_t* wbase = Wp + wt + (uint32_t)kt * WIMG + (uint32_t)(wave * (WIMG / 4));
      ldw32(f.wq[0], f.wq[1], wbase, wlane * 2u);
    } else if constexpr (RW == 2) {
      const int8_t* wbase = Wp + wt + (uint32_t)kt * WIMG + (uint32_t)(wave * (WIMG / 4));
      ldw64(f.wq[0], f.wq[1], f.wq[2], f.wq[3], wbase, wlane * 4u);
    }
  };
  auto pin = [&](Frags<WFMT>& f) __attribute__((always_inline)) {
    if constexpr (RW == 1) asm volatile("; qvit_pin %0 %1" : "+v"(f.wq[0]), "+v"(f.wq[1]));
    if constexpr (RW == 2)
      asm volatile("; qvit_pin %0 %1 %2 %3" : "+v"(f.wq[0]), "+v"(f.wq[1]), "+v"(f.wq[2]), "+v"(f.wq[3]));
  };
  int xoff = 0, woff = 0;
  auto lane_offsets = [&](int ln) __attribute__((always_inline)) {
    const int lfr = ln & 15, lfq = ln >> 4;
    xoff = (128 * wm + lfr) * BK + ((lfq ^ (((lfr >> 2) & 1) << 1)) << 4);
    woff = (WFMT == QVIT_W4) ? (64 * wn + lfr) * G::WROW + ((lfq ^ (((lfr >> 3) & 1) << 1)) << 3)
                             : (64 * wn + lfr) * G::WROW + ((lfq ^ (((lfr >> 2) & 1) << 1)) << 4);
    wlane = (uint32_t)ln * 16u;
    alane = lane_a(ln);
  };
  auto read_frags = [&](int rslot, Frags<WFMT>& f) {
    const int8_t* sx = smem + rslot * SLOT;
    const int8_t* sw = sx + XBYTES;
#pragma unroll
    for (int s = 0; s < 8; ++s) f.x[s] = *reinterpret_cast<const v4i*>(sx + xoff + s * 16 * BK);
    if constexpr (!REGW) {
#pragma unroll
      for (int r = 0; r < 4; ++r) {
        if (WFMT == QVIT_W4)
          f.w4[r] = *reinterpret_cast<const uint2*>(sw + woff + r * 16 * G::WROW);
        else
          f.w8[r] = *reinterpret_cast<const v4i*>(sw + woff + r * 16 * G::WROW);
      }
    }
  };

  v4i acc[4][8];
  auto mfma_stage = [&](const Frags<WFMT>& f, auto zeroc) __attribute__((always_inline)) {
    constexpr bool ZERO = decltype(zeroc)::value;
#pragma unroll
    for (int r = 0; r < 4; ++r) {
      v4i wf;
      if constexpr (RW == 2) {
        wf = f.wq[r];
      } else if (WFMT == QVIT_W4) {
        uint2 p = f.w4[r];
        if constexpr (REGW) {
          const v4i q = f.wq[r >> 1];
          p = (r & 1) ? make_uint2((uint32_t)q[2], (uint32_t)q[3]) : make_uint2((uint32_t)q[0], (uint32_t)q[1]);
        }
        wf = v4i{(int)nib16_lo(p.x), (int)nib16_hi(p.x), (int)nib16_lo(p.y), (int)nib16_hi(p.y)};
      } else {
        wf = f.w8[r];
      }
#pragma unroll
      for (int s = 0; s < 8; ++s)
        acc[r][s] = __builtin_amdgcn_mfma_i32_16x16x64_i8(wf, f.x[s], ZERO ? v4i{0, 0, 0, 0} : acc[r][s], 0, 0, 0);
    }
  };

  constexpr int D = G::XPIECES + (REGW ? WREG : G::WPIECES);
  auto step_core = [&](Frags<WFMT>& cur, Frags<WFMT>& nxt, int next_slot, bool read,
                       auto zeroc) __attribute__((always_inline)) {
    if (read) read_frags(next_slot, nxt);
    __builtin_amdgcn_sched_barrier(0);
    mfma_stage(cur, zeroc);
    __builtin_amdgcn_sched_barrier(0);
  };

  auto ln_after_tile = [&](int m0) __attribute__((always_inline)) {
    int* flag = reinterpret_cast<int*>(qp_l);
    asm volatile("s_waitcnt vmcnt(0)" ::: "memory");
    __builtin_amdgcn_s_waitcnt(0xC07F);
    asm volatile("s_barrier" ::: "memory");
    if (tid == 0) {
      const int old = __hip_atomic_fetch_add(ep.ln_cnt + m0 / BM, 1, __ATOMIC_RELAXED, __HIP_MEMORY_SCOPE_AGENT);
      *flag = old == nb_n - 1 ? 1 : 0;
    }
    __builtin_amdgcn_s_waitcnt(0xC07F);
    asm volatile("s_barrier" ::: "memory");
    if (*flag == 0) return;
    const int8_t* ent = nullptr;
    float c0 = 0.f, inv_w = 0.f, top = 0.f;
    QParams qp{};
    if (ep.ln_table != nullptr) {
      const EpiTableHdr h = *reinterpret_cast<const EpiTableHdr*>(ep.ln_table);
      if (h.valid != 0 && h.nb >= 1 && h.nb <= G::TABLE_MAX_NB) {
        const v4i* src = reinterpret_cast<const v4i*>(ep.ln_table);
        for (int i = tid; i < (16 + 8 * h.nb + 15) / 16; i += G::NT) reinterpret_cast<v4i*>(epi_lds)[i] = src[i];
        ent = epi_lds + sizeof(EpiTableHdr);
        c0 = h.c0;
        inv_w = h.inv_w;
        top = epi_top(h.nb);
      }
    }
    if (ent == nullptr) qp = load_qparams(ep.out_qtype, ep.out_d, ep.out_qm, ep.out_t, ep.out_levels);
    const int ln = lane_opaque();
    const int cols = N;
    float4 gam[4], bet[4];
#pragma unroll
    for (int i = 0; i < 4; ++i) {
      const int c = 4 * (ln + 64 * i);
      const bool in = c < cols;
      gam[i] = (in && ep.ln_gamma) ? *reinterpret_cast<const float4*>(ep.ln_gamma + c) : make_float4(1.f, 1.f, 1.f, 1.f);
      bet[i] = (in && ep.ln_beta) ? *reinterpret_cast<const float4*>(ep.ln_beta + c) : make_float4(0.f, 0.f, 0.f, 0.f);
    }
    __builtin_amdgcn_s_waitcnt(0xC07F);
    asm volatile("s_barrier" ::: "memory");
    typedef float f4v __attribute__((ext_vector_type(4)));
    const __amdgpu_buffer_rsrc_t rsrc = __builtin_amdgcn_make_buffer_rsrc(
        const_cast<void*>(static_cast<const void*>(C)), (short)0, (int)((int64_t)M * ldc * 4), 0x00020000);
    auto job = [&](auto nvc, auto modec) __attribute__((always_inline)) {
      constexpr int NV = decltype(nvc)::value;
      constexpr int MODE = decltype(modec)::value;
      const int rend = (m0 + BM < M ? m0 + BM : M);
      auto ld = [&](int r, f4v (&t)[NV]) __attribute__((always_inline)) {
        const int rr = r < M ? r : M - 1;
#pragma unroll
        for (int i = 0; i < NV; ++i) {
          const int c = 4 * (ln + 64 * i);
          t[i] = __builtin_amdgcn_raw_buffer_load_b128(rsrc, (int)(((int64_t)rr * ldc + (c < cols ? c : 0)) * 4), 0, 16);
        }
      };
      auto row = [&](int r, const f4v (&t)[NV]) __attribute__((always_inline)) {
        float4 v[NV];
#pragma unroll
        for (int i = 0; i < NV; ++i)
          v[i] = (4 * (ln + 64 * i) < cols) ? make_float4(t[i][0], t[i][1], t[i][2], t[i][3])
                                            : make_float4(0.f, 0.f, 0.f, 0.f);
        uint32_t word[NV];
        auto gb = [&](int i, float4& g, float4& bb) {
          g = gam[i];
          bb = bet[i];
        };
        ln_quant_row<NV, decltype(gb), MODE>(v, ln, cols, ep.ln_eps, gb, ent, c0, inv_w, top, qp, word);
        if (r < rend) {
          int8_t* cr = ep.ln_codes + (int64_t)r * ep.ln_ldc;
#pragma unroll
          for (int i = 0; i < NV; ++i) {
            const int c = 4 * (ln + 64 * i);
            if (c < cols) *reinterpret_cast<uint32_t*>(cr + c) = word[i];
          }
          for (int c = cols + ln; c < ep.ln_kpad; c += 64) cr[c] = 0;
        }
      };
      f4v t0[NV], t1[NV], t2[NV];
      const int r0 = m0 + wave;
      ld(r0, t0);
      ld(r0 + 4, t1);
#pragma unroll 1
      for (int r = r0; r < rend; r += 12) {
        ld(r + 8, t2);
        row(r, t0);
        ld(r + 12, t0);
        row(r + 4, t1);
        ld(r + 16, t1);
        row(r + 8, t2);
      }
    };
    if (ent == nullptr) job(std::integral_constant<int, 4>{}, std::integral_constant<int, 2>{});
    else if (cols <= 768) job(std::integral_constant<int, 3>{}, std::integral_constant<int, 1>{});
    else job(std::integral_constant<int, 4>{}, std::integral_constant<int, 1>{});
  };

  int g = 0;
  {
    lane_offsets(lane_opaque());
    const int am0 = tile_m0(t);
    const uint32_t w0 = tile_w(t);
    issue(am0, w0, 0, 0);
    issue(am0, w0, 1, 1);
    if constexpr (L2)
      for (int j = 2; j <= ALEAD; ++j) issue(am0, w0, j, j);
  }
  Frags<WFMT> fa, fb;
  QVIT_STAMP_DECL
  QVIT_LSTAMP_DECL
  for (;;) {
    const int tnext = t + team;
    const bool has_next = tnext < hi;
    const int m0 = tile_m0(t), n0 = (t % nb_n) * BN;
    if (nk == 2 || !PEEL) {
#pragma unroll
      for (int r = 0; r < 4; ++r)
#pragma unroll
        for (int s = 0; s < 8; ++s) acc[r][s] = v4i{0, 0, 0, 0};
    }

    if constexpr (L2) {
    constexpr int XP = G::XPIECES;
    QVIT_STAMP(5);
    const uint32_t cw = tile_w(t);
    const int ln = lane_opaque();
    lane_offsets(ln);
    issue_w(cw, 0, fa);
    __builtin_amdgcn_s_waitcnt(0xC07F);
    stage_sync<ALEAD * XP + WREG>();
    QVIT_STAMP(0);
    QVIT_LSTAMP(0);
    if (has_bias && wave == 0)
      dma16(ep.bias + n0 + ln * 4, __builtin_amdgcn_readfirstlane(lds0 + RING_B + G::EPI_BYTES));
    read_frags(g % RINGN, fa);
    auto lstep = [&](int kt, Frags<WFMT>& cur, Frags<WFMT>& nxt, auto zeroc) __attribute__((always_inline)) {
      __builtin_amdgcn_s_waitcnt(0xC07F);
      __builtin_amdgcn_sched_barrier(0);
      issue_w(cw, kt + 1, nxt);
      issue(m0, cw, kt + ALEAD + 1, (g + kt + ALEAD + 1) % RINGN);
      QVIT_STAMP(1);
      stage_sync<2 * XP + WREG>();
      pin(cur);
      QVIT_STAMP(2);
      step_core(cur, nxt, (g + kt + 1) % RINGN, true, zeroc);
      QVIT_STAMP(3);
    };
    __builtin_amdgcn_s_waitcnt(0xC07F);
    __builtin_amdgcn_sched_barrier(0);
    issue_w(cw, 1, fb);
    issue(m0, cw, ALEAD + 1, (g + ALEAD + 1) % RINGN);
    QVIT_STAMP(1);
    stage_sync<XP + WREG>();
    pin(fa);
    QVIT_STAMP(2);
    if constexpr (PEEL) step_core(fa, fb, (g + 1) % RINGN, true, std::true_type{});
    else step_core(fa, fb, (g + 1) % RINGN, true, std::false_type{});
    QVIT_STAMP(3);
    int kt = 1;
    if constexpr (ALEAD & 1) {
      lstep(1, fb, fa, std::false_type{});
      kt = 2;
      for (; kt + 1 <= nk - ALEAD - 2; kt += 2) {
        lstep(kt, fa, fb, std::false_type{});
        lstep(kt + 1, fb, fa, std::false_type{});
      }
    } else {
      for (; kt + 1 <= nk - ALEAD - 2; kt += 2) {
        lstep(kt, fb, fa, std::false_type{});
        lstep(kt + 1, fa, fb, std::false_type{});
      }
    }
    const uint32_t nw = has_next ? tile_w(tnext) : 0u;
    const int nm0 = has_next ? tile_m0(tnext) : 0;
    auto tstep = [&](auto jc, Frags<WFMT>& cur, Frags<WFMT>& nxt) __attribute__((always_inline)) {
      constexpr int j = decltype(jc)::value;
      const int tk = nk - ALEAD - 1 + j;
      __builtin_amdgcn_s_waitcnt(0xC07F);
      __builtin_amdgcn_sched_barrier(0);
      if constexpr (j < ALEAD) issue_w(cw, tk + 1, nxt);
      constexpr int NW = j < ALEAD ? WREG : 0;
      if (has_next) {
        issue(nm0, nw, j, (g + nk + j) % RINGN);
        if constexpr (j < ALEAD) stage_sync<2 * XP + NW>();
        else asm volatile("s_waitcnt vmcnt(%0)" ::"n"(2 * XP) : "memory");
      } else {
        if constexpr (j < ALEAD) stage_sync<(j == 0 ? XP : 0) + NW>();
        else asm volatile("s_waitcnt vmcnt(0)" ::: "memory");
      }
      pin(cur);
      step_core(cur, nxt, (g + tk + 1) % RINGN, j < ALEAD, std::false_type{});
    };
    if constexpr (ALEAD & 1) {
      tstep(std::integral_constant<int, 0>{}, fa, fb);
      tstep(std::integral_constant<int, 1>{}, fb, fa);
      tstep(std::integral_constant<int, 2>{}, fa, fb);
      tstep(std::integral_constant<int, 3>{}, fb, fa);
    } else {
      tstep(std::integral_constant<int, 0>{}, fb, fa);
      tstep(std::integral_constant<int, 1>{}, fa, fb);
      tstep(std::integral_constant<int, 2>{}, fb, fa);
    }
    QVIT_STAMP(3);
    QVIT_LSTAMP(1);
    } else {
    QVIT_STAMP(5);
    const uint32_t cw = tile_w(t);
    const int ln = lane_opaque();
    lane_offsets(ln);
    issue_w(cw, 0, fa);
    __builtin_amdgcn_s_waitcnt(0xC07F);
    stage_sync<D>();
    QVIT_STAMP(0);
    QVIT_LSTAMP(0);
    {
      if (has_bias && wave == 0)
        dma16(ep.bias + n0 + ln * 4, __builtin_amdgcn_readfirstlane(lds0 + RING_B + G::EPI_BYTES));
    }
    read_frags(g % RINGN, fa);
    int kt = 0;
    if (PEEL && nk > 2) {
      __builtin_amdgcn_s_waitcnt(0xC07F);
      __builtin_amdgcn_sched_barrier(0);
      issue(m0, cw, 2, (g + 2) % RINGN);
      issue_w(cw, 1, fb);
      QVIT_STAMP(1);
      stage_sync<D>();
      pin(fa);
      QVIT_STAMP(2);
      step_core(fa, fb, (g + 1) % RING, true, std::true_type{});
      QVIT_STAMP(3);
      __builtin_amdgcn_s_waitcnt(0xC07F);
      __builtin_amdgcn_sched_barrier(0);
      issue(m0, cw, 3, (g + 3) % RINGN);
      issue_w(cw, 2, fa);
      QVIT_STAMP(1);
      stage_sync<D>();
      pin(fb);
      QVIT_STAMP(2);
      step_core(fb, fa, (g + 2) % RING, true, std::false_type{});
      QVIT_STAMP(3);
      kt = 2;
    }
    for (; kt < nk - 2; kt += 2) {
      __builtin_amdgcn_s_waitcnt(0xC07F);
      __builtin_amdgcn_sched_barrier(0);
      issue(m0, cw, kt + 2, (g + kt + 2) % RINGN);
      issue_w(cw, kt + 1, fb);
      QVIT_STAMP(1);
      stage_sync<D>();
      pin(fa);
      QVIT_STAMP(2);
      step_core(fa, fb, (g + kt + 1) % RING, true, std::false_type{});
      QVIT_STAMP(3);
      __builtin_amdgcn_s_waitcnt(0xC07F);
      __builtin_amdgcn_sched_barrier(0);
      issue(m0, cw, kt + 3, (g + kt + 3) % RINGN);
      issue_w(cw, kt + 2, fa);
      QVIT_STAMP(1);
      stage_sync<D>();
      pin(fb);
      QVIT_STAMP(2);
      step_core(fb, fa, (g + kt + 2) % RING, true, std::false_type{});
      QVIT_STAMP(3);
    }
    __builtin_amdgcn_s_waitcnt(0xC07F);
    __builtin_amdgcn_sched_barrier(0);
    const uint32_t nw = has_next ? tile_w(tnext) : 0u;
    const int nm0 = has_next ? tile_m0(tnext) : 0;
    issue_w(cw, nk - 1, fb);
    if (has_next) {
      issue(nm0, nw, 0, (g + nk) % RINGN);
      stage_sync<D>();
    } else {
      stage_sync<REGW ? WREG : 0>();
    }
    pin(fa);
    step_core(fa, fb, (g + nk - 1) % RING, true, std::false_type{});
    __builtin_amdgcn_s_waitcnt(0xC07F);
    __builtin_amdgcn_sched_barrier(0);
    if (has_next) {
      issue(nm0, nw, 1, (g + nk + 1) % RINGN);
      if constexpr (REGW) asm volatile("s_waitcnt vmcnt(%0)" ::"n"(G::XPIECES) : "memory");
    } else {
      if constexpr (REGW) asm volatile("s_waitcnt vmcnt(0)" ::: "memory");
    }
    pin(fb);
    step_core(fb, fa, 0, false, std::false_type{});
    QVIT_STAMP(3);
    QVIT_LSTAMP(1);

    }

    if (WFMT == QVIT_W4 && EPI == QVIT_EPI_I32) {
#pragma unroll
      for (int r = 0; r < 4; ++r)
#pragma unroll
        for (int sr = 0; sr < 8; ++sr)
#pragma unroll
          for (int j = 0; j < 4; ++j) acc[r][sr][j] >>= 4;
    }
    {
    const int el = lane_opaque();
    if (I8OUT) __builtin_amdgcn_s_setprio(1);
    const int efr = el & 15, efq = el >> 4;
    if (I8OUT && use_table) {
      const int8_t* tlb = epi_lds + sizeof(EpiTableHdr);
      const int nbase = n0 + 64 * wn + 16 * efq;
      float bcol[16];
#pragma unroll
      for (int r = 0; r < 4; ++r) {
        float4 b = make_float4(0.f, 0.f, 0.f, 0.f);
        if (has_bias) b = *reinterpret_cast<const float4*>(bias_l + (nbase - n0) + 4 * r);
        bcol[4 * r] = b.x; bcol[4 * r + 1] = b.y; bcol[4 * r + 2] = b.z; bcol[4 * r + 3] = b.w;
      }
      const bool fast16 = ((ldc & 15) == 0) && ((((uintptr_t)C) & 15) == 0) && ((N & 15) == 0);
      float v[2][4][4];
      uint2 e[2][4][4];
      auto look = [&](int sr, int b) __attribute__((always_inline)) {
#pragma unroll
        for (int r = 0; r < 4; ++r)
#pragma unroll
          for (int j = 0; j < 4; ++j) {
            v[b][r][j] = fmaf(alpha, (float)acc[r][sr][j], bcol[4 * r + j]);
            e[b][r][j] = *epi_entry(tlb, v[b][r][j], t_c0, t_invw, t_top);
          }
      };
      look(0, 0);
#pragma unroll
      for (int sr = 0; sr < 8; ++sr) {
        const int cb = sr & 1;
        if (sr + 1 < 8) look(sr + 1, cb ^ 1);
        __builtin_amdgcn_sched_barrier(0);
        const int m = m0 + 128 * wm + 16 * sr + efr;
        uint32_t wd[4];
#pragma unroll
        for (int r = 0; r < 4; ++r) {
          epi_select_byte<0>(wd[r], v[cb][r][0], __uint_as_float(e[cb][r][0].x), e[cb][r][0].y);
          epi_select_byte<1>(wd[r], v[cb][r][1], __uint_as_float(e[cb][r][1].x), e[cb][r][1].y);
          epi_select_byte<2>(wd[r], v[cb][r][2], __uint_as_float(e[cb][r][2].x), e[cb][r][2].y);
          epi_select_byte<3>(wd[r], v[cb][r][3], __uint_as_float(e[cb][r][3].x), e[cb][r][3].y);
        }
        int8_t* dst = reinterpret_cast<int8_t*>(C) + (int64_t)m * ldc + nbase;
        if (fast16) {
          if (m < M && nbase < N) *reinterpret_cast<uint4*>(dst) = make_uint4(wd[0], wd[1], wd[2], wd[3]);
        } else if (m < M) {
#pragma unroll
          for (int q = 0; q < 16; ++q)
            if (nbase + q < N) dst[q] = (int8_t)((wd[q >> 2] >> (8 * (q & 3))) & 0xff);
        }
        __builtin_amdgcn_sched_barrier(0);
      }
    } else if (EPI == QVIT_EPI_F32_RESID || EPI == EPI_RESID_LN) {
      int* stg = reinterpret_cast<int*>(epi_lds + wave * EPI_WAVE_BYTES);
      const int prow = el >> 4, pcol = 4 * (el & 15);
      const int n = n0 + 64 * wn + pcol;
      const bool nfull = n + 4 <= N;
      float4 b4 = make_float4(0.f, 0.f, 0.f, 0.f);
      if (has_bias) b4 = *reinterpret_cast<const float4*>(bias_l + (n - n0));
      float* Cf = reinterpret_cast<float*>(C);
      float4 old[2][4];
      if (m0 + BM <= M && n0 + BN <= N) {
        typedef float f4v __attribute__((ext_vector_type(4)));
        f4v ov0[4], ov1[4];
        auto ld = [&](int sr, f4v (&ov)[4]) __attribute__((always_inline)) {
#pragma unroll
          for (int i = 0; i < 4; ++i) {
            const float* src = Cf + (int64_t)(m0 + 128 * wm + 16 * sr + 4 * i + prow) * ldc + n;
            asm volatile("; qvit_asm_load\n\tglobal_load_dwordx4 %0, %1, off" : "=v"(ov[i]) : "v"(src) : "memory");
          }
        };
        auto pass = [&](int sr, f4v (&ov)[4]) __attribute__((always_inline)) {
          __builtin_amdgcn_s_waitcnt(0xC07F);
#pragma unroll
          for (int r = 0; r < 4; ++r)
            *reinterpret_cast<v4i*>(stg + efr * EPI_LD + 16 * efq + 4 * r) = acc[r][sr];
          __builtin_amdgcn_s_waitcnt(0xC07F);
          __builtin_amdgcn_wave_barrier();
          if (sr == 0 || sr == 7)
            asm volatile("s_waitcnt vmcnt(4)\n\t; qvit_pin %0 %1 %2 %3"
                         : "+v"(ov[0]), "+v"(ov[1]), "+v"(ov[2]), "+v"(ov[3]) :: "memory");
          else
            asm volatile("s_waitcnt vmcnt(8)\n\t; qvit_pin %0 %1 %2 %3"
                         : "+v"(ov[0]), "+v"(ov[1]), "+v"(ov[2]), "+v"(ov[3]) :: "memory");
#pragma unroll
          for (int i = 0; i < 4; ++i) {
            const int row = 4 * i + prow;
            const int m = m0 + 128 * wm + 16 * sr + row;
            const v4i a4 = *reinterpret_cast<const v4i*>(stg + row * EPI_LD + pcol);
            float4 o = make_float4(alpha * (float)a4[0] + b4.x, alpha * (float)a4[1] + b4.y,
                                   alpha * (float)a4[2] + b4.z, alpha * (float)a4[3] + b4.w);
            o.x += ov[i][0]; o.y += ov[i][1]; o.z += ov[i][2]; o.w += ov[i][3];
            st_resid<EPI == EPI_RESID_LN>(Cf + (int64_t)m * ldc + n, o, Cf, M, ldc);
          }
        };
        ld(0, ov0);
#pragma unroll
        for (int sr = 0; sr < 8; sr += 2) {
          ld(sr + 1, ov1);
          pass(sr, ov0);
          if (sr + 2 < 8) ld(sr + 2, ov0);
          pass(sr + 1, ov1);
        }
      } else {
      auto load_old = [&](int sr, float4 (&ov)[4]) __attribute__((always_inline)) {
#pragma unroll
        for (int i = 0; i < 4; ++i) {
          const int m = m0 + 128 * wm + 16 * sr + 4 * i + prow;
          ov[i] = (m < M && nfull) ? *reinterpret_cast<const float4*>(Cf + (int64_t)m * ldc + n)
                                   : make_float4(0.f, 0.f, 0.f, 0.f);
        }
      };
      load_old(0, old[0]);
#pragma unroll
      for (int sr = 0; sr < 8; ++sr) {
        if (sr + 1 < 8) load_old(sr + 1, old[(sr + 1) & 1]);
        __builtin_amdgcn_s_waitcnt(0xC07F);
#pragma unroll
        for (int r = 0; r < 4; ++r)
          *reinterpret_cast<v4i*>(stg + efr * EPI_LD + 16 * efq + 4 * r) = acc[r][sr];
        __builtin_amdgcn_s_waitcnt(0xC07F);
        __builtin_amdgcn_wave_barrier();
#pragma unroll
        for (int i = 0; i < 4; ++i) {
          const int row = 4 * i + prow;
          const int m = m0 + 128 * wm + 16 * sr + row;
          const v4i a4 = *reinterpret_cast<const v4i*>(stg + row * EPI_LD + pcol);
          if (m < M) {
            float4 o = make_float4(alpha * (float)a4[0] + b4.x, alpha * (float)a4[1] + b4.y,
                                   alpha * (float)a4[2] + b4.z, alpha * (float)a4[3] + b4.w);
            float* dst = Cf + (int64_t)m * ldc + n;
            if (nfull) {
              const float4 ov = old[sr & 1][i];
              o.x += ov.x; o.y += ov.y; o.z += ov.z; o.w += ov.w;
              st_resid<EPI == EPI_RESID_LN>(dst, o, Cf, M, ldc);
            } else {
              const float v[4] = {o.x, o.y, o.z, o.w};
              for (int j = 0; j < 4; ++j)
                if (n + j < N) dst[j] = dst[j] + v[j];
            }
          }
        }
      }
      }
    } else if (is_qkv_split(EPI)) {
      constexpr int PD = EPI == EPI_QKV_SPLIT80 ? 80 : 64;
      int* stg = reinterpret_cast<int*>(epi_lds + wave * EPI_WAVE_BYTES);
      const int prow = el >> 3, pcol = 8 * (el & 7);
      const int nw = n0 + 64 * wn;
      float bb[8];
#pragma unroll
      for (int j = 0; j < 8; ++j) bb[j] = has_bias ? bias_l[nw - n0 + pcol + j] : 0.f;
      const int64_t pstride = (int64_t)ep.seq * PD;
#pragma unroll
      for (int sr = 0; sr < 8; ++sr) {
        __builtin_amdgcn_s_waitcnt(0xC07F);
#pragma unroll
        for (int r = 0; r < 4; ++r)
          *reinterpret_cast<v4i*>(stg + efr * EPI_LD + 16 * efq + 4 * r) = acc[r][sr];
        __builtin_amdgcn_s_waitcnt(0xC07F);
        __builtin_amdgcn_wave_barrier();
#pragma unroll
        for (int i = 0; i < 2; ++i) {
          const int row = 8 * i + prow;
          const int m = m0 + 128 * wm + 16 * sr + row;
          const v4i a0 = *reinterpret_cast<const v4i*>(stg + row * EPI_LD + pcol);
          const v4i a1 = *reinterpret_cast<const v4i*>(stg + row * EPI_LD + pcol + 4);
          if (m < M && (PD == 64 ? nw : nw + pcol) < N) {
            int bimg = (int)((float)m * ep.inv_seq);
            bimg -= (bimg * ep.seq > m) ? 1 : 0;
            bimg += ((bimg + 1) * ep.seq <= m) ? 1 : 0;
            const int tok = m - bimg * ep.seq;
            int64_t e;
            if constexpr (PD == 64)
              e = ((int64_t)bimg * (N >> 6) + (nw >> 6)) * pstride + (int64_t)tok * 64 + pcol;
            else
              e = ((int64_t)bimg * (N / PD) + (nw + pcol) / PD) * pstride + (int64_t)tok * PD + (nw + pcol) % PD;
            uint32_t hw[4], lw[4];
#pragma unroll
            for (int j = 0; j < 8; j += 2) {
              const int a_0 = (j < 4) ? a0[j] : a1[j - 4], a_1 = (j < 4) ? a0[j + 1] : a1[j - 3];
              const float x0 = (alpha * (float)a_0 + bb[j]) * ep.in_scale;
              const float x1 = (alpha * (float)a_1 + bb[j + 1]) * ep.in_scale;
              const _Float16 h0 = (_Float16)x0, h1 = (_Float16)x1;
              const _Float16 l0 = (_Float16)(x0 - (float)h0), l1 = (_Float16)(x1 - (float)h1);
              hw[j >> 1] = (uint32_t)__builtin_bit_cast(uint16_t, h0) | ((uint32_t)__builtin_bit_cast(uint16_t, h1) << 16);
              lw[j >> 1] = (uint32_t)__builtin_bit_cast(uint16_t, l0) | ((uint32_t)__builtin_bit_cast(uint16_t, l1) << 16);
            }
            *reinterpret_cast<uint4*>(reinterpret_cast<_Float16*>(C) + e) = make_uint4(hw[0], hw[1], hw[2], hw[3]);
            *reinterpret_cast<uint4*>(ep.lo + e) = make_uint4(lw[0], lw[1], lw[2], lw[3]);
          }
        }
      }
    } else {
      int* stg = reinterpret_cast<int*>(epi_lds + wave * EPI_WAVE_BYTES);
      const int prow = el >> 4;
      const int pcol = 4 * (el & 15);
      const int n = n0 + 64 * wn + pcol;
      const bool nfull = n + 4 <= N;
      float4 b4 = make_float4(0.f, 0.f, 0.f, 0.f);
      if (has_bias) b4 = *reinterpret_cast<const float4*>(bias_l + (n - n0));
      QParams qp;
      if (I8OUT) qp = *qp_l;
#pragma unroll
      for (int sr = 0; sr < 8; ++sr) {
        __builtin_amdgcn_s_waitcnt(0xC07F);
#pragma unroll
        for (int r = 0; r < 4; ++r)
          *reinterpret_cast<v4i*>(stg + efr * EPI_LD + 16 * efq + 4 * r) = acc[r][sr];
        __builtin_amdgcn_s_waitcnt(0xC07F);
        __builtin_amdgcn_wave_barrier();
#pragma unroll 1
        for (int i = 0; i < 4; ++i) {
          const int row = 4 * i + prow;
          const int m = m0 + 128 * wm + 16 * sr + row;
          const v4i a4 = *reinterpret_cast<const v4i*>(stg + row * EPI_LD + pcol);
          if (m < M) {
            if (EPI == QVIT_EPI_I32) {
              int32_t* dst = reinterpret_cast<int32_t*>(C) + (int64_t)m * ldc + n;
              if (nfull) {
                *reinterpret_cast<v4i*>(dst) = a4;
              } else {
                for (int j = 0; j < 4; ++j)
                  if (n + j < N) dst[j] = a4[j];
              }
            } else if (EPI == QVIT_EPI_F32 || EPI == QVIT_EPI_F32_RESID) {
              float4 o = make_float4(alpha * (float)a4[0] + b4.x, alpha * (float)a4[1] + b4.y,
                                     alpha * (float)a4[2] + b4.z, alpha * (float)a4[3] + b4.w);
              float* dst = reinterpret_cast<float*>(C) + (int64_t)m * ldc + n;
              if (nfull) {
                if (EPI == QVIT_EPI_F32_RESID) {
                  const float4 old = *reinterpret_cast<const float4*>(dst);
                  o.x += old.x; o.y += old.y; o.z += old.z; o.w += old.w;
                }
                *reinterpret_cast<float4*>(dst) = o;
              } else {
                const float ov[4] = {o.x, o.y, o.z, o.w};
                for (int j = 0; j < 4; ++j)
                  if (n + j < N) dst[j] = (EPI == QVIT_EPI_F32_RESID) ? dst[j] + ov[j] : ov[j];
              }
            } else {
              const float bb[4] = {b4.x, b4.y, b4.z, b4.w};
              float v[4], k[4];
              bool need[4];
#pragma unroll
              for (int j = 0; j < 4; ++j) {
                v[j] = alpha * (float)a4[j] + bb[j];
                if (EPI == QVIT_EPI_I8_GELU) v[j] = gelu_ref(v[j]);
                k[j] = quant_fast(v[j], qp, need[j]);
              }
              if (__any(need[0] | need[1] | need[2] | need[3])) {
#pragma unroll
                for (int j = 0; j < 4; ++j)
                  if (need[j]) k[j] = quant_fixup(v[j], qp);
              }
              uint32_t word = 0;
#pragma unroll
              for (int j = 0; j < 4; ++j) word |= ((uint32_t)(uint8_t)to_i8_sat(k[j])) << (8 * j);
              int8_t* dst = reinterpret_cast<int8_t*>(C) + (int64_t)m * ldc + n;
              if (nfull) {
                *reinterpret_cast<uint32_t*>(dst) = word;
              } else {
                for (int j = 0; j < 4; ++j)
                  if (n + j < N) dst[j] = (int8_t)((word >> (8 * j)) & 0xff);
              }
            }
          }
        }
      }
    }
    }
    if (I8OUT) __builtin_amdgcn_s_setprio(0);
    QVIT_STAMP(4);
    QVIT_LSTAMP(2);
    if constexpr (EPI == EPI_RESID_LN) {
      ln_after_tile(m0);
      QVIT_STAMP(6);
    }
    if (!has_next) break;
    t = tnext;
    g += nk;
  }
  QVIT_STAMP_FLUSH;
  QVIT_LSTAMP_FLUSH;
  asm volatile("s_waitcnt vmcnt(0)" ::: "memory");
}

#ifndef QVIT_GEMM_L2
#define QVIT_GEMM_L2 1
#endif
constexpr bool GEMM_L2 = QVIT_GEMM_L2 != 0;

template <int WFMT, int EPI, int RW = 0>
int launch(const int8_t* A, int64_t M, int64_t K, int64_t lda, const void* Wp, int64_t N, int64_t npad,
           void* C, int64_t ldc, const EpiArgs& ep, hipStream_t stream) {
  constexpr int WMV = 1;
  using G = Geo<WFMT, WMV>;
  const int64_t span = (int64_t)0xFFFFFFFF - K;
  int64_t rows = span / lda / G::BM * G::BM;
  if (rows < G::BM || npad * (K / (WFMT == QVIT_W4 && RW != 2 ? 2 : 1)) > span) return QVIT_EINVAL;
  if (is_qkv_split(EPI) && rows < M) return QVIT_EINVAL;
  const int64_t esize = (EPI == QVIT_EPI_I8 || EPI == QVIT_EPI_I8_GELU) ? 1 : 4;
  for (int64_t m0 = 0; m0 < M; m0 += rows) {
    const int64_t mc = (M - m0 < rows) ? M - m0 : rows;
    const int64_t ntiles = (npad / BN) * ((mc + G::BM - 1) / G::BM);
    int64_t grid = (int64_t)qvit_device_cus() * G::MIN_BLOCKS / 8 * 8;
    const int64_t need = (ntiles + 7) / 8 * 8;
    if (grid > need) grid = need;
    if (grid < 8) grid = 8;
    void* Cc = reinterpret_cast<int8_t*>(C) + (is_qkv_split(EPI) ? 0 : m0 * ldc * esize);
    EpiArgs epc = ep;
    if (EPI == EPI_RESID_LN) {
      epc.ln_cnt = ep.ln_cnt + m0 / G::BM;
      epc.ln_codes = ep.ln_codes + m0 * ep.ln_ldc;
    }
    if (RW != 0 && K / BK >= ALEAD + 2 && GEMM_L2)
      hipLaunchKernelGGL((gemm_kernel<WFMT, EPI, WMV, RW, RW != 0>), dim3((unsigned)grid), dim3(G::NT), 0, stream,
                         A + m0 * lda, (int)mc, (int)K, lda, reinterpret_cast<const int8_t*>(Wp), (int)N, (int)npad, Cc,
                         ldc, epc);
    else
      hipLaunchKernelGGL((gemm_kernel<WFMT, EPI, WMV, RW>), dim3((unsigned)grid), dim3(G::NT), 0, stream,
                         A + m0 * lda, (int)mc, (int)K, lda, reinterpret_cast<const int8_t*>(Wp), (int)N, (int)npad, Cc,
                         ldc, epc);
    const hipError_t e = hipGetLastError();
    if (e != hipSuccess) return qvit_hip_status(e);
  }
  return QVIT_OK;
}

template <int WFMT, int RW = 0>
int dispatch_epi(int epilogue, const int8_t* A, int64_t M, int64_t K, int64_t lda, const void* Wp, int64_t N,
                 int64_t npad, void* C, int64_t ldc, const EpiArgs& ep, hipStream_t stream) {
  switch (epilogue) {
    case QVIT_EPI_F32: return launch<WFMT, QVIT_EPI_F32, RW>(A, M, K, lda, Wp, N, npad, C, ldc, ep, stream);
    case QVIT_EPI_F32_RESID: return launch<WFMT, QVIT_EPI_F32_RESID, RW>(A, M, K, lda, Wp, N, npad, C, ldc, ep, stream);
    case QVIT_EPI_I8_GELU: return launch<WFMT, QVIT_EPI_I8_GELU, RW>(A, M, K, lda, Wp, N, npad, C, ldc, ep, stream);
    case QVIT_EPI_I8: return launch<WFMT, QVIT_EPI_I8, RW>(A, M, K, lda, Wp, N, npad, C, ldc, ep, stream);
    case QVIT_EPI_I32: return launch<WFMT, QVIT_EPI_I32, RW>(A, M, K, lda, Wp, N, npad, C, ldc, ep, stream);
    case QVIT_EPI_QKV_SPLIT:
      return launch<WFMT, QVIT_EPI_QKV_SPLIT, RW>(A, M, K, lda, Wp, N, npad, C, ldc, ep, stream);
    default: return QVIT_EINVAL;
  }
}

}

extern "C" int qvit_epi_table_build(int epilogue, int out_qtype, const float* out_d, const float* out_qm,
                                    const float* out_t, int out_levels, float v_lo, float w, int64_t nb, void* table,
                                    hipStream_t stream) {
  if (!table) return QVIT_ENULL;
  if (epilogue != QVIT_EPI_I8 && epilogue != QVIT_EPI_I8_GELU) return QVIT_EINVAL;
  if (nb < 1 || nb > QVIT_EPI_TABLE_MAX_NB || !(w > 0.f) || !std::isfinite(v_lo) || !std::isfinite(v_lo + w * nb))
    return QVIT_EINVAL;
  if (qvit_out_quant_status(out_qtype, out_d, out_qm, out_levels)) return QVIT_EINVAL;
  if (qvit_misaligned(15, table)) return QVIT_EALIGN;
  const int one = 1;
  hipError_t e = hipMemcpyAsync(reinterpret_cast<int8_t*>(table) + offsetof(EpiTableHdr, valid), &one, sizeof(int),
                                hipMemcpyHostToDevice, stream);
  if (e != hipSuccess) return qvit_hip_status(e);
  hipLaunchKernelGGL(epi_table_kernel, dim3((unsigned)((nb + 63) / 64)), dim3(64), 0, stream,
                     epilogue == QVIT_EPI_I8_GELU ? 1 : 0, out_qtype, out_d, out_qm, out_t, out_levels,
                     -(v_lo * (1.0f / w)), 1.0f / w, (int)nb, reinterpret_cast<int8_t*>(table));
  return qvit_launch_status();
}

extern "C" int qvit_pack_weight_w4r(const void* packed, int64_t npad, int64_t kpad, void* out, hipStream_t stream) {
  if (!packed || !out) return QVIT_ENULL;
  if (npad <= 0 || npad % BN || kpad <= 0 || kpad % KTILE || npad > INT32_MAX / 2 || kpad > 65536) return QVIT_EINVAL;
  if (qvit_misaligned(15, packed, out)) return QVIT_EALIGN;
  if (packed == out) return QVIT_EINVAL;
  const int64_t units = npad * kpad / 16;
  hipLaunchKernelGGL(pack_w4r_kernel, dim3((unsigned)((units + 255) / 256)), dim3(256), 0, stream,
                     reinterpret_cast<const int8_t*>(packed), reinterpret_cast<int8_t*>(out), units);
  return qvit_launch_status();
}

extern "C" int qvit_pack_weight_w8r(const void* packed, int64_t npad, int64_t kpad, void* out, hipStream_t stream) {
  if (!packed || !out) return QVIT_ENULL;
  if (npad <= 0 || npad % BN || kpad <= 0 || kpad % KTILE || npad > INT32_MAX / 2 || kpad > 65536) return QVIT_EINVAL;
  if (qvit_misaligned(15, packed, out)) return QVIT_EALIGN;
  if (packed == out) return QVIT_EINVAL;
  const int64_t units = npad * kpad / 16;
  hipLaunchKernelGGL(pack_w8r_kernel, dim3((unsigned)((units + 255) / 256)), dim3(256), 0, stream,
                     reinterpret_cast<const int8_t*>(packed), reinterpret_cast<int8_t*>(out), units);
  return qvit_launch_status();
}

extern "C" int qvit_gemm(const int8_t* A, int64_t M, int64_t K, int64_t lda, const void* Wp, int wfmt, int64_t N,
                         int64_t npad, const float* d_act, const float* d_wt, const float* bias, int epilogue,
                         void* C, int64_t ldc, int out_qtype, const float* out_d, const float* out_qm,
                         const float* out_t, int out_levels, const void* epi_table, hipStream_t stream) {
  if (!A || !Wp || !C) return QVIT_ENULL;
  if (wfmt != QVIT_W4 && wfmt != QVIT_W4R && wfmt != QVIT_W8R && wfmt != QVIT_W8) return QVIT_EINVAL;
  if (M < 0 || K <= 0 || K % KTILE || lda < K || N <= 0 || npad < N || npad % BN) return QVIT_EINVAL;
  if (M > INT32_MAX / 2 || npad > INT32_MAX / 2 || K > (1 << 24)) return QVIT_EINVAL;
  if (wfmt != QVIT_W8 && K > 65536) return QVIT_EINVAL;
  if ((lda % 16) || qvit_misaligned(15, A, Wp)) return QVIT_EALIGN;
  if (epilogue < QVIT_EPI_F32 || epilogue > QVIT_EPI_I32) return QVIT_EINVAL;
  const bool i8out = epilogue == QVIT_EPI_I8 || epilogue == QVIT_EPI_I8_GELU;
  if (ldc < N) return QVIT_EINVAL;
  if (i8out) {
    if ((ldc % 4) || qvit_misaligned(3, C)) return QVIT_EALIGN;
    if (qvit_out_quant_status(out_qtype, out_d, out_qm, out_levels)) return QVIT_EINVAL;
  } else {
    if ((ldc % 4) || qvit_misaligned(15, C)) return QVIT_EALIGN;
  }
  if (epilogue != QVIT_EPI_I32 && (!d_act || !d_wt)) return QVIT_ENULL;
  if (qvit_misaligned(15, bias)) return QVIT_EALIGN;
  if (M == 0) return QVIT_OK;
  if (qvit_misaligned(15, epi_table)) return QVIT_EALIGN;
  EpiArgs ep{d_act, d_wt, bias, out_qtype, out_d, out_qm, out_t, out_levels,
             (i8out ? reinterpret_cast<const int8_t*>(epi_table) : nullptr), 1, 1.f, 1.f, nullptr};
  if (wfmt == QVIT_W4) return dispatch_epi<QVIT_W4>(epilogue, A, M, K, lda, Wp, N, npad, C, ldc, ep, stream);
  if (wfmt == QVIT_W4R) return dispatch_epi<QVIT_W4, 1>(epilogue, A, M, K, lda, Wp, N, npad, C, ldc, ep, stream);
  if (wfmt == QVIT_W8R) return dispatch_epi<QVIT_W4, 2>(epilogue, A, M, K, lda, Wp, N, npad, C, ldc, ep, stream);
  return dispatch_epi<QVIT_W8>(epilogue, A, M, K, lda, Wp, N, npad, C, ldc, ep, stream);
}

extern "C" int qvit_gemm_resid_ln(const int8_t* A, int64_t M, int64_t K, int64_t lda, const void* Wp, int wfmt,
                                  int64_t N, int64_t npad, const float* d_act, const float* d_wt, const float* bias,
                                  float* C, int64_t ldc, const float* gamma, const float* beta, float eps,
                                  int out_qtype, const float* out_d, const float* out_qm, const float* out_t,
                                  int out_levels, const void* ln_table, int8_t* codes, int64_t ldcodes,
                                  int64_t kpad_codes, int32_t* counters, hipStream_t stream) {
  if (!A || !Wp || !C || !codes || !counters || !d_act || !d_wt) return QVIT_ENULL;
  if (wfmt != QVIT_W4 && wfmt != QVIT_W8) return QVIT_EINVAL;
  if (M < 0 || K <= 0 || K % KTILE || lda < K || N <= 0 || N > 1024 || N % 4 || npad < N || npad % BN)
    return QVIT_EINVAL;
  if (M > INT32_MAX / 2 || K > (1 << 24) || (wfmt == QVIT_W4 && K > 65536)) return QVIT_EINVAL;
  if (ldc < N || kpad_codes < N || ldcodes < kpad_codes || M * ldc * 4 > 0x7FFFFFFF) return QVIT_EINVAL;
  if ((lda % 16) || qvit_misaligned(15, A, Wp)) return QVIT_EALIGN;
  if ((ldc % 4) || (ldcodes % 4) || qvit_misaligned(15, C, bias, gamma, beta, ln_table)) return QVIT_EALIGN;
  if (qvit_misaligned(3, codes, counters)) return QVIT_EALIGN;
  if (qvit_out_quant_status(out_qtype, out_d, out_qm, out_levels)) return QVIT_EINVAL;
  if (M == 0) return QVIT_OK;
  const hipError_t ez = hipMemsetAsync(counters, 0, (size_t)((M + 127) / 128) * sizeof(int32_t), stream);
  if (ez != hipSuccess) return qvit_hip_status(ez);
  EpiArgs ep{d_act, d_wt, bias, out_qtype, out_d, out_qm, out_t, out_levels, nullptr, 1, 1.f, 1.f, nullptr,
             gamma, beta, eps, reinterpret_cast<const int8_t*>(ln_table), codes, ldcodes, (int)kpad_codes,
             reinterpret_cast<int*>(counters)};
  if (wfmt == QVIT_W4) return launch<QVIT_W4, EPI_RESID_LN>(A, M, K, lda, Wp, N, npad, C, ldc, ep, stream);
  return launch<QVIT_W8, EPI_RESID_LN>(A, M, K, lda, Wp, N, npad, C, ldc, ep, stream);
}

QVIT_GEMM_STAMP_READER

template <int EPI>
static int qkv_split_launch(const int8_t* A, int64_t M, int64_t K, int64_t lda, const void* Wp, int wfmt, int64_t N,
                            int64_t npad, void* qkv_hi, const EpiArgs& ep, hipStream_t stream) {
  if (wfmt == QVIT_W4) return launch<QVIT_W4, EPI>(A, M, K, lda, Wp, N, npad, qkv_hi, N, ep, stream);
  if (wfmt == QVIT_W4R) return launch<QVIT_W4, EPI, 1>(A, M, K, lda, Wp, N, npad, qkv_hi, N, ep, stream);
  if (wfmt == QVIT_W8R) return launch<QVIT_W4, EPI, 2>(A, M, K, lda, Wp, N, npad, qkv_hi, N, ep, stream);
  return launch<QVIT_W8, EPI>(A, M, K, lda, Wp, N, npad, qkv_hi, N, ep, stream);
}

static int qkv_split(const int8_t* A, int64_t M, int64_t K, int64_t lda, const void* Wp, int wfmt, int64_t N,
                     int64_t npad, const float* d_act, const float* d_wt, const float* bias, int64_t seq,
                     int64_t head_dim, float in_scale, void* qkv_hi, void* qkv_lo, hipStream_t stream) {
  if (!A || !Wp || !qkv_hi || !qkv_lo || !d_act || !d_wt) return QVIT_ENULL;
  if (wfmt != QVIT_W4 && wfmt != QVIT_W4R && wfmt != QVIT_W8R && wfmt != QVIT_W8) return QVIT_EINVAL;
  if (head_dim != 64 && head_dim != 80) return QVIT_EINVAL;
  if (M < 0 || K <= 0 || K % KTILE || lda < K || N <= 0 || N % head_dim || npad < N || npad % BN) return QVIT_EINVAL;
  if (M > INT32_MAX / 2 || npad > INT32_MAX / 2 || K > (1 << 24)) return QVIT_EINVAL;
  if (seq <= 0 || seq > (1 << 20) || M % seq || !(in_scale > 0.f)) return QVIT_EINVAL;
  if (wfmt != QVIT_W8 && K > 65536) return QVIT_EINVAL;
  if ((lda % 16) || qvit_misaligned(15, A, Wp)) return QVIT_EALIGN;
  if (qvit_misaligned(15, qkv_hi, qkv_lo)) return QVIT_EALIGN;
  if (qvit_misaligned(15, bias)) return QVIT_EALIGN;
  if (M == 0) return QVIT_OK;
  EpiArgs ep{d_act, d_wt, bias, 0, nullptr, nullptr, nullptr, 0, nullptr, (int)seq, 1.0f / (float)seq, in_scale,
             reinterpret_cast<_Float16*>(qkv_lo)};
  if (head_dim == 80) return qkv_split_launch<EPI_QKV_SPLIT80>(A, M, K, lda, Wp, wfmt, N, npad, qkv_hi, ep, stream);
  return qkv_split_launch<QVIT_EPI_QKV_SPLIT>(A, M, K, lda, Wp, wfmt, N, npad, qkv_hi, ep, stream);
}

extern "C" int qvit_gemm_qkv_split(const int8_t* A, int64_t M, int64_t K, int64_t lda, const void* Wp, int wfmt,
                                   int64_t N, int64_t npad, const float* d_act, const float* d_wt, const float* bias,
                                   int64_t seq, float in_scale, void* qkv_hi, void* qkv_lo, hipStream_t stream) {
  return qkv_split(A, M, K, lda, Wp, wfmt, N, npad, d_act, d_wt, bias, seq, 64, in_scale, qkv_hi, qkv_lo, stream);
}

extern "C" int qvit_gemm_qkv_split_hd(const int8_t* A, int64_t M, int64_t K, int64_t lda, const void* Wp, int wfmt,
                                      int64_t N, int64_t npad, const float* d_act, const float* d_wt,
                                      const float* bias, int64_t seq, int64_t head_dim, float in_scale, void* qkv_hi,
                                      void* qkv_lo, hipStream_t stream) {
  return qkv_split(A, M, K, lda, Wp, wfmt, N, npad, d_act, d_wt, bias, seq, head_dim, in_scale, qkv_hi, qkv_lo,
                   stream);
}
```

### quantized_vit_amd/csrc/qvit_common.h

```cpp
#pragma once
#include <hip/hip_runtime.h>
#include <stdint.h>
#include "../../include/qvit_hip.h"

#define QVIT_DEV __device__ __forceinline__

#define QVIT_QT_FORCE_CAREFUL 0x100

QVIT_DEV float log_cr(float a) { return (float)log((double)a); }
QVIT_DEV float exp_cr(float a) { return (float)exp((double)a); }


struct QParams {
  int qtype;
  int careful;
  float d;
  float inv_d;
  float qm;
  float t;
  float L;
  float levels;
};

QVIT_DEV QParams load_qparams(int qtype, const float* d, const float* qm, const float* t, int levels) {
  QParams p;
  p.careful = (qtype & QVIT_QT_FORCE_CAREFUL) ? 1 : 0;
  p.qtype = qtype & 0xff;
  p.levels = (float)levels;
  p.d = 1.f; p.inv_d = 1.f; p.qm = 0.f; p.t = 1.f; p.L = 0.f;
  if (p.qtype == QVIT_QT_ULTRA_ACT) return p;
  p.d = *d;
  p.qm = *qm;
  p.t = (t != nullptr) ? *t : 1.f;
  p.inv_d = 1.f / p.d;
  if (!(fabsf(p.inv_d) < 3.0e38f)) p.careful = 1;
  if (p.qtype == QVIT_QT_LINEAR) {
    p.L = rintf(fabsf(p.qm) / p.d);
  } else {
    p.L = rintf(exp_cr(p.t * log_cr(fabsf(p.qm) + 1e-6f)) / p.d);
  }
  return p;
}

__device__ __noinline__ float code_mag_careful_ool(float a, int linear, float t, float d) {
  float pw = linear ? a : exp_cr(t * log_cr(a));
  return rintf(pw / d);
}
QVIT_DEV float code_mag_careful(float a, const QParams& p) {
  return code_mag_careful_ool(a, p.qtype == QVIT_QT_LINEAR, p.t, p.d);
}

QVIT_DEV float quant_fast(float x, const QParams& p, bool& need) {
  if (p.qtype == QVIT_QT_ULTRA_ACT) {
    need = false;
    return rintf(fminf(fmaxf(x, 0.f), 1.f) * p.levels);
  }
  const float a = fabsf(x);
  float q, relerr;
  if (p.qtype == QVIT_QT_LINEAR) {
    q = a * p.inv_d;
    relerr = 32.f * 1.1920929e-7f;
  } else {
    const float eb = fabsf(p.t) * (float)(abs(__builtin_amdgcn_frexp_expf(a)) + 1);
    const float pw = (p.t == 1.f) ? a : __builtin_amdgcn_exp2f(p.t * __builtin_amdgcn_logf(a));
    q = pw * p.inv_d;
    relerr = (eb * 0.6931472f + 4.f) * 8.f * 1.1920929e-7f;
  }
  const float f = q - floorf(q);
  const bool in_range = (a < p.qm) && (a > 0.f);
  const bool tiny = (p.qtype == QVIT_QT_NONLINEAR) && !(a > 1e-30f);
  need = in_range && ((fabsf(f - 0.5f) <= fabsf(q) * relerr + 1e-37f) || tiny || p.careful);
  float k = (a >= p.qm) ? p.L : rintf(q);
  k = copysignf(k, x);
  return (a > 0.f) ? k : 0.f;
}

QVIT_DEV float quant_fixup(float x, const QParams& p) {
  return copysignf(code_mag_careful(fabsf(x), p), x);
}

QVIT_DEV float quant_code(float x, const QParams& p) {
  bool need;
  const float k = quant_fast(x, p, need);
  return need ? quant_fixup(x, p) : k;
}

QVIT_DEV float quant_code_from_pow(float x, float pw, const QParams& p) {
  const float a = fabsf(x);
  float k = (a >= p.qm) ? p.L : rintf(pw / p.d);
  k = copysignf(k, x);
  return (a > 0.f) ? k : 0.f;
}

QVIT_DEV float fake_quant_value(float x, const QParams& p) {
  if (p.qtype == QVIT_QT_ULTRA_ACT) {
    return quant_code(x, p) / p.levels;
  }
  return p.d * quant_code(x, p);
}

QVIT_DEV int8_t to_i8_sat(float k) {
  k = fminf(fmaxf(k, -127.f), 127.f);
  return (int8_t)(int)k;
}


struct EpiTableHdr {
  float c0;
  float inv_w;
  int nb;
  int valid;
};
struct EpiTableEnt {
  float thr;
  int8_t lo, hi;
  int16_t pad;
};
QVIT_DEV float epi_top(int nb) { return __int_as_float(0x4B000000 + nb - 1); }
QVIT_DEV uint32_t epi_bucket_bits(float v, float C, float inv_w, float top) {
  return __float_as_uint(__builtin_amdgcn_fmed3f(fmaf(v, inv_w, C), 8388608.f, top));
}
QVIT_DEV int epi_bucket(float v, float C, float inv_w, float top) {
  return (int)(epi_bucket_bits(v, C, inv_w, top) - 0x4B000000u);
}
QVIT_DEV const uint2* epi_entry(const int8_t* ent, float v, float C, float inv_w, float top) {
  return reinterpret_cast<const uint2*>(ent + ((epi_bucket_bits(v, C, inv_w, top) << 3) - (0x4B000000u << 3)));
}

template <int J>
QVIT_DEV void epi_select_byte(uint32_t& wd, float v, float thr, uint32_t lohi) {
  if (J == 0)
    asm("v_cmp_ge_f32_e32 vcc, %1, %2\n\t"
        "v_cndmask_b32_sdwa %0, %3, %3, vcc dst_sel:BYTE_0 dst_unused:UNUSED_PAD src0_sel:BYTE_0 src1_sel:BYTE_1"
        : "=v"(wd) : "v"(v), "v"(thr), "v"(lohi) : "vcc");
  else if (J == 1)
    asm("v_cmp_ge_f32_e32 vcc, %1, %2\n\t"
        "v_cndmask_b32_sdwa %0, %3, %3, vcc dst_sel:BYTE_1 dst_unused:UNUSED_PRESERVE src0_sel:BYTE_0 src1_sel:BYTE_1"
        : "+v"(wd) : "v"(v), "v"(thr), "v"(lohi) : "vcc");
  else if (J == 2)
    asm("v_cmp_ge_f32_e32 vcc, %1, %2\n\t"
        "v_cndmask_b32_sdwa %0, %3, %3, vcc dst_sel:BYTE_2 dst_unused:UNUSED_PRESERVE src0_sel:BYTE_0 src1_sel:BYTE_1"
        : "+v"(wd) : "v"(v), "v"(thr), "v"(lohi) : "vcc");
  else
    asm("v_cmp_ge_f32_e32 vcc, %1, %2\n\t"
        "v_cndmask_b32_sdwa %0, %3, %3, vcc dst_sel:BYTE_3 dst_unused:UNUSED_PRESERVE src0_sel:BYTE_0 src1_sel:BYTE_1"
        : "+v"(wd) : "v"(v), "v"(thr), "v"(lohi) : "vcc");
}


QVIT_DEV float pow2i_f(int q) { return __int_as_float((q + 0x7f) << 23); }
QVIT_DEV float sleef_expf_u10(float d) {
#pragma clang fp contract(off)
  const float fq = fminf(fmaxf(rintf(d * 1.442695040888963407359924681001892137426645954152985934135449406931f),
                               -256.f), 256.f);
  const int q = (int)fq;
  float s = fmaf(fq, -0.693145751953125f, d);
  s = fmaf(fq, -1.428606765330187045e-06f, s);
  float u = 0.000198527617612853646278381f;
  u = fmaf(u, s, 0.00139304355252534151077271f);
  u = fmaf(u, s, 0.00833336077630519866943359f);
  u = fmaf(u, s, 0.0416664853692054748535156f);
  u = fmaf(u, s, 0.166666671633720397949219f);
  u = fmaf(u, s, 0.5f);
  u = 1.0f + fmaf(s * s, u, s);
  u = (u * pow2i_f(q >> 1)) * pow2i_f(q - (q >> 1));
  u = (d < -104.f) ? 0.f : u;
  return (d > 100.f) ? INFINITY : u;
}

QVIT_DEV float gelu_ref(float x) {
#pragma clang fp contract(off)
  const float u = x * 0.70710678118654752440f;
  const float t = 1.0f / fmaf(0.3275911f, fabsf(u), 1.0f);
  float r = fmaf(1.061405429f, t, -1.453152027f);
  r = fmaf(r, t, 1.421413741f);
  r = fmaf(r, t, -0.284496736f);
  r = fmaf(r, t, 0.254829592f);
  const float e = sleef_expf_u10(-(u * u));
  const float erf_abs = fmaf(-e * t, r, 1.0f);
  return (x * 0.5f) * (1.0f + copysignf(erf_abs, u));
}

QVIT_DEV int lane_opaque() {
  int l;
  asm volatile("v_mbcnt_lo_u32_b32 %0, -1, 0\n\tv_mbcnt_hi_u32_b32 %0, -1, %0" : "=v"(l));
  return l;
}

QVIT_DEV uint32_t lds_addr(const void* p) {
  return (uint32_t)(uintptr_t)(const __attribute__((address_space(3))) void*)p;
}

QVIT_DEV void dma16(const void* gsrc, uint32_t lds_base) {
  uint32_t keep;
  asm volatile(
      "s_mov_b32 %0, m0\n\t"
      "s_mov_b32 m0, %2\n\t"
      "s_nop 0\n\t"
      "global_load_lds_dwordx4 %1, off\n\t"
      "s_mov_b32 m0, %0"
      : "=&s"(keep)
      : "v"(gsrc), "s"(lds_base)
      : "memory");
}

QVIT_DEV void dma16s(const void* sbase, uint32_t voff, uint32_t lds_base) {
  uint32_t keep;
  asm volatile(
      "s_mov_b32 %0, m0\n\t"
      "s_mov_b32 m0, %3\n\t"
      "s_nop 0\n\t"
      "global_load_lds_dwordx4 %1, %2\n\t"
      "s_mov_b32 m0, %0"
      : "=&s"(keep)
      : "v"(voff), "s"(sbase), "s"(lds_base)
      : "memory");
}

static inline int qvit_hip_status(hipError_t e) {
  return e == hipSuccess ? QVIT_OK : (QVIT_EHIP - (int)e);
}
static inline int qvit_launch_status() { return qvit_hip_status(hipGetLastError()); }

template <typename... P>
static inline bool qvit_misaligned(uintptr_t mask, const P*... p) {
  return ((... | (uintptr_t)p) & mask) != 0;
}

static inline bool qvit_qtype_flags_ok(int qtype) { return (qtype & ~(0xff | QVIT_QT_FORCE_CAREFUL)) == 0; }

static inline int qvit_out_quant_status(int qtype, const float* d, const float* qm, int levels) {
  const int q = qtype & 0xff;
  if (q != QVIT_QT_LINEAR && q != QVIT_QT_NONLINEAR && q != QVIT_QT_ULTRA_ACT) return QVIT_EINVAL;
  if (q == QVIT_QT_ULTRA_ACT ? (levels < 1 || levels > 127) : (!d || !qm)) return QVIT_EINVAL;
  return QVIT_OK;
}
static inline int qvit_quant_status(int qtype, const float* d, const float* qm, int levels) {
  return qvit_qtype_flags_ok(qtype) ? qvit_out_quant_status(qtype, d, qm, levels) : QVIT_EINVAL;
}
static inline int qvit_backward_qtype_status(int qtype, bool& nonlinear) {
  const int q = qtype & 0xff;
  if (!qvit_qtype_flags_ok(qtype) || (q != QVIT_QT_LINEAR && q != QVIT_QT_NONLINEAR)) return QVIT_EINVAL;
  nonlinear = q == QVIT_QT_NONLINEAR;
  return QVIT_OK;
}

struct ConvShape {
  int64_t OH, OW, K, M;
};
static inline int qvit_conv_shape(int64_t B, int64_t C, int64_t H, int64_t W, int kh, int kw, int sh, int sw,
                                  int64_t ph, int64_t pw, int dh, int dw, ConvShape& s) {
  if (B < 0 || C < 1 || H < 1 || W < 1 || kh < 1 || kw < 1 || sh < 1 || sw < 1 || ph < 0 || pw < 0 || dh < 1 ||
      dw < 1)
    return QVIT_EINVAL;
  const int64_t eh = H + 2 * ph - (int64_t)dh * (kh - 1) - 1;
  const int64_t ew = W + 2 * pw - (int64_t)dw * (kw - 1) - 1;
  if (eh < 0 || ew < 0) return QVIT_EINVAL;
  s.OH = eh / sh + 1;
  s.OW = ew / sw + 1;
  s.K = C * kh * kw;
  s.M = B * s.OH * s.OW;
  return QVIT_OK;
}

inline int qvit_device_cus() {
  static const int cus = [] {
    int dev = 0, n = 0;
    if (hipGetDevice(&dev) != hipSuccess || hipDeviceGetAttribute(&n, hipDeviceAttributeMultiprocessorCount, dev) !=
                                                hipSuccess || n <= 0)
      n = 256;
    return n;
  }();
  return cus;
}
```

Baseline: 34600 img/s.

## Split GEMM row tail into short-height tiles to balance the last wave across CUs

For register-weight GEMMs with the residual F32 epilogue, the launcher now computes a tail map. Full 128-row blocks cover only as many rows as fill whole waves of persistent slots. The remaining rows are split into shorter tiles of 64 to 112 rows, so more CUs share the tail instead of a few CUs doing full 128-row tiles. The kernel gains a template tail-height parameter, masked LDS DMA for partial row groups, and lets full tiles prefetch into a following short tile. This adds code paths, more template instantiations and register pressure, and can be switched off with an environment variable.

```diff
diff --git a/include/qvit_hip.h b/include/qvit_hip.h
--- a/include/qvit_hip.h
+++ b/include/qvit_hip.h
@@ -167,6 +167,8 @@
               int epilogue, void* C, int64_t ldc,
               int out_qtype, const float* out_d, const float* out_qm, const float* out_t,
               int out_levels, const void* epi_table, hipStream_t stream);
+
+int qvit_gemm_tail_map(int64_t M, int64_t npad, int64_t slots, int64_t cus, int32_t* map3);
 
 int qvit_layernorm_quant_i8_t32(const float* x, int64_t rows, int64_t cols, int64_t ldx, const float* gamma,
                                 const float* beta, float eps, int qtype, const float* d_quant, const float* q_m,
diff --git a/quantized_vit_amd/_lib.py b/quantized_vit_amd/_lib.py
--- a/quantized_vit_amd/_lib.py
+++ b/quantized_vit_amd/_lib.py
@@ -96,6 +96,7 @@
     "qvit_layernorm_quant_i8_t32": [_c_p, _i64, _i64, _i64, _c_p, _c_p, _f32, _i32, _c_p, _c_p, _c_p, _i32, _c_p,
                                     _i64, _c_p, _c_p],
     "qvit_gemm_a32_fits": [_i64, _i32, _i64, _i64, _i32],
+    "qvit_gemm_tail_map": [_i64, _i64, _i64, _i64, _c_p],
     "qvit_gemm_a32": [_c_p, _i64, _i64, _c_p, _i32, _i64, _i64, _c_p, _c_p, _c_p, _i32, _c_p, _i64, _i32, _c_p, _c_p,
                       _c_p, _i32, _c_p, _c_p],
     "qvit_gemm_wonly": [_c_p, _i64, _i64, _i64, _c_p, _i32, _i64, _i64, _c_p, _c_p, _c_p, _i64, _c_p, _i64, _c_p],
@@ -602,6 +603,12 @@
     return C
 
 
+def gemm_tail_map(M: int, npad: int, slots: int, cus: int) -> Tuple[int, int, int]:
+    out = (ctypes.c_int32 * 3)()
+    _check(load().qvit_gemm_tail_map(M, npad, slots, cus, ctypes.addressof(out)), "qvit_gemm_tail_map")
+    return out[0], out[1], out[2]
+
+
 def t32_rows(M: int) -> int:
     return (M + 63) // 64 * 64
 
diff --git a/quantized_vit_amd/csrc/gemm_w4a8.hip b/quantized_vit_amd/csrc/gemm_w4a8.hip
--- a/quantized_vit_amd/csrc/gemm_w4a8.hip
+++ b/quantized_vit_amd/csrc/gemm_w4a8.hip
@@ -1,5 +1,6 @@
 #include <cmath>
 #include <cstddef>
+#include <cstdlib>
 #include <type_traits>
 
 #include "diag_stamps.h"
@@ -211,15 +212,19 @@
   }
 }
 
-template <int WFMT, int EPI, int WM, int RW, bool L2 = false>
+template <int WFMT, int EPI, int WM, int RW, bool L2 = false, int TL = 8>
 __global__ __launch_bounds__((Geo<WFMT, WM>::NT), (Geo<WFMT, WM>::MIN_BLOCKS)) void gemm_kernel(
     const int8_t* __restrict__ A, int M, int K, int64_t lda, const int8_t* __restrict__ Wp, int N, int npad,
-    void* __restrict__ C, int64_t ldc, EpiArgs ep) {
+    void* __restrict__ C, int64_t ldc, int frb, EpiArgs ep) {
   using G = Geo<WFMT, WM>;
   constexpr int BM = G::BM;
   constexpr int XBYTES = G::XBYTES;
   constexpr bool I8OUT = (EPI == QVIT_EPI_I8 || EPI == QVIT_EPI_I8_GELU);
   static_assert(!L2 || RW != 0, "the two-ahead activation ring is for register weights");
+  static_assert(TL == 8 || (L2 && TL >= 4 && TL < 8), "short tail tiles: the two-ahead ring, 64 to 112 rows");
+  constexpr bool TAIL = TL != 8;
+  using FullC = std::integral_constant<int, 8>;
+  using TailC = std::integral_constant<int, TL>;
   constexpr int RINGN = L2 ? ALEAD + 2 : RING;
   constexpr int SLOT = L2 ? XBYTES : G::STAGE;
   constexpr int RING_B = RINGN * SLOT;
@@ -242,13 +247,23 @@
   const int fq = lane >> 4;
 
   const int nb_n = npad / BN;
-  const int ntiles = nb_n * ((M + BM - 1) / BM);
+  const int ntiles = nb_n * (TAIL ? frb : (M + BM - 1) / BM);
   const int xcd = blockIdx.x & 7, slot = blockIdx.x >> 3, team = gridDim.x >> 3;
   const int per = ntiles >> 3, rem = ntiles & 7;
   const int lo = xcd * per + (xcd < rem ? xcd : rem);
   const int hi = lo + per + (xcd < rem ? 1 : 0);
+  int tail_t = -1;
+  if constexpr (TAIL) {
+    const int ntail = nb_n * ((M - frb * BM + 16 * TL - 1) / (16 * TL));
+    const int tper = ntail >> 3, trem = ntail & 7;
+    const int tlo = xcd * tper + (xcd < trem ? xcd : trem);
+    if (slot < tper + (xcd < trem ? 1 : 0)) tail_t = ntiles + tlo + slot;
+  }
   int t = lo + slot;
-  if (t >= hi) return;
+  if (t >= hi) {
+    if (tail_t < 0) return;
+    t = tail_t;
+  }
 
   float alpha = 0.f;
   if (EPI != QVIT_EPI_I32) alpha = (*ep.d_act) * (*ep.d_wt) * (WFMT == QVIT_W4 ? 0.0625f : 1.f);
@@ -275,18 +290,37 @@
   constexpr bool PEEL = !I8OUT && RW != 2;
   uint32_t wlane = 0;
   auto tile_w = [&](int tt) -> uint32_t {
+    if (TAIL && tt >= ntiles) tt -= ntiles;
     return __builtin_amdgcn_readfirstlane((uint32_t)(tt % nb_n) * (uint32_t)(nk * WIMG));
   };
-  auto tile_m0 = [&](int tt) -> int { return __builtin_amdgcn_readfirstlane((tt / nb_n) * BM); };
+  auto tile_m0 = [&](int tt) -> int {
+    if (TAIL && tt >= ntiles) return __builtin_amdgcn_readfirstlane(frb * BM + ((tt - ntiles) / nb_n) * (16 * TL));
+    return __builtin_amdgcn_readfirstlane((tt / nb_n) * BM);
+  };
   auto lane_a = [&](int ln) -> uint32_t {
     return (uint32_t)(ln >> 2) * (uint32_t)lda + (uint32_t)(((ln & 3) ^ (((ln >> 4) & 1) << 1)) << 4);
   };
   uint32_t alane = 0;
   const uint32_t lds0 = lds_addr(smem);
-  auto issue = [&](int m0, uint32_t wt, int kt, int rslot) __attribute__((always_inline)) {
+  auto issue = [&](int m0, uint32_t wt, int kt, int rslot, auto lvc) __attribute__((always_inline)) {
+    constexpr int LV = decltype(lvc)::value;
     const uint32_t sx = lds0 + (uint32_t)(rslot * SLOT);
     const uint32_t sw = sx + XBYTES;
-    if (m0 + BM <= M) {
+    if constexpr (LV != 8) {
+      constexpr int HQ = 4 * LV;
+      constexpr uint64_t PART_LANES = (1ull << (4 * (HQ - 16))) - 1;
+      const uint32_t d0 = __builtin_amdgcn_readfirstlane(sx + (HQ * wave) * BK);
+#pragma unroll
+      for (int j = 0; j < (LV > 4 ? 2 : 1); ++j) {
+        const int ln = lane_opaque();
+        const int row = HQ * wave + 16 * j + (ln >> 2);
+        int gm = m0 + row;
+        gm = gm < M ? gm : M - 1;
+        const uint32_t a = (uint32_t)gm * (uint32_t)lda + (uint32_t)(((ln & 3) ^ (((row >> 2) & 1) << 1)) * 16);
+        if (j == 0) dma16s(A + kt * BK, a, d0);
+        else dma16s_masked(A + kt * BK, a, d0 + 16 * BK, PART_LANES);
+      }
+    } else if (m0 + BM <= M) {
       const int8_t* abase = A + (int64_t)(m0 + 32 * wave) * lda + kt * BK;
 #pragma unroll
       for (int j = 0; j < G::XPIECES; ++j)
@@ -333,11 +367,12 @@
     wlane = (uint32_t)ln * 16u;
     alane = lane_a(ln);
   };
-  auto read_frags = [&](int rslot, Frags<WFMT>& f) {
+  auto read_frags = [&](int rslot, Frags<WFMT>& f, auto lvc) {
+    constexpr int LV = decltype(lvc)::value;
     const int8_t* sx = smem + rslot * SLOT;
     const int8_t* sw = sx + XBYTES;
 #pragma unroll
-    for (int s = 0; s < 8; ++s) f.x[s] = *reinterpret_cast<const v4i*>(sx + xoff + s * 16 * BK);
+    for (int s = 0; s < LV; ++s) f.x[s] = *reinterpret_cast<const v4i*>(sx + xoff + s * 16 * BK);
     if constexpr (!REGW) {
 #pragma unroll
       for (int r = 0; r < 4; ++r) {
@@ -350,8 +385,9 @@
   };
 
   v4i acc[4][8];
-  auto mfma_stage = [&](const Frags<WFMT>& f, auto zeroc) __attribute__((always_inline)) {
+  auto mfma_stage = [&](const Frags<WFMT>& f, auto zeroc, auto lvc) __attribute__((always_inline)) {
     constexpr bool ZERO = decltype(zeroc)::value;
+    constexpr int LV = decltype(lvc)::value;
 #pragma unroll
     for (int r = 0; r < 4; ++r) {
       v4i wf;
@@ -368,17 +404,17 @@
         wf = f.w8[r];
       }
 #pragma unroll
-      for (int s = 0; s < 8; ++s)
+      for (int s = 0; s < LV; ++s)
         acc[r][s] = __builtin_amdgcn_mfma_i32_16x16x64_i8(wf, f.x[s], ZERO ? v4i{0, 0, 0, 0} : acc[r][s], 0, 0, 0);
     }
   };
 
   constexpr int D = G::XPIECES + (REGW ? WREG : G::WPIECES);
-  auto step_core = [&](Frags<WFMT>& cur, Frags<WFMT>& nxt, int next_slot, bool read,
-                       auto zeroc) __attribute__((always_inline)) {
-    if (read) read_frags(next_slot, nxt);
+  auto step_core = [&](Frags<WFMT>& cur, Frags<WFMT>& nxt, int next_slot, bool read, auto zeroc,
+                       auto lvc) __attribute__((always_inline)) {
+    if (read) read_frags(next_slot, nxt, lvc);
     __builtin_amdgcn_sched_barrier(0);
-    mfma_stage(cur, zeroc);
+    mfma_stage(cur, zeroc, lvc);
     __builtin_amdgcn_sched_barrier(0);
   };
 
@@ -478,31 +514,38 @@
   };
 
   int g = 0;
-  {
+  auto prologue = [&](auto lvc) __attribute__((always_inline)) {
     lane_offsets(lane_opaque());
     const int am0 = tile_m0(t);
     const uint32_t w0 = tile_w(t);
-    issue(am0, w0, 0, 0);
-    issue(am0, w0, 1, 1);
+    issue(am0, w0, 0, 0, lvc);
+    issue(am0, w0, 1, 1, lvc);
     if constexpr (L2)
-      for (int j = 2; j <= ALEAD; ++j) issue(am0, w0, j, j);
-  }
+      for (int j = 2; j <= ALEAD; ++j) issue(am0, w0, j, j, lvc);
+  };
+  if (TAIL && t >= ntiles) prologue(TailC{});
+  else prologue(FullC{});
   Frags<WFMT> fa, fb;
   QVIT_STAMP_DECL
   QVIT_LSTAMP_DECL
-  for (;;) {
-    const int tnext = t + team;
-    const bool has_next = tnext < hi;
-    const int m0 = tile_m0(t), n0 = (t % nb_n) * BN;
+  int tnext = 0;
+  bool has_next_rt = false, next_short = false;
+  auto run_tile = [&](auto lvc) __attribute__((always_inline)) {
+    constexpr int LV = decltype(lvc)::value;
+    const bool has_next = LV == 8 && (TAIL ? __builtin_amdgcn_readfirstlane((int)has_next_rt) != 0 : has_next_rt);
+    const bool nshort = TAIL && __builtin_amdgcn_readfirstlane((int)next_short) != 0;
+    const int m0 = tile_m0(t), n0 = ((TAIL && t >= ntiles ? t - ntiles : t) % nb_n) * BN;
     if (nk == 2 || !PEEL) {
 #pragma unroll
       for (int r = 0; r < 4; ++r)
 #pragma unroll
-        for (int s = 0; s < 8; ++s) acc[r][s] = v4i{0, 0, 0, 0};
+        for (int s = 0; s < LV; ++s) acc[r][s] = v4i{0, 0, 0, 0};
     }
 
     if constexpr (L2) {
-    constexpr int XP = G::XPIECES;
+    constexpr int XPS = TL > 4 ? 2 : 1;
+    constexpr int XP = LV == 8 ? G::XPIECES : XPS;
+    constexpr int XPN = G::XPIECES;
     QVIT_STAMP(5);
     const uint32_t cw = tile_w(t);
     const int ln = lane_opaque();
@@ -514,29 +557,29 @@
     QVIT_LSTAMP(0);
     if (has_bias && wave == 0)
       dma16(ep.bias + n0 + ln * 4, __builtin_amdgcn_readfirstlane(lds0 + RING_B + G::EPI_BYTES));
-    read_frags(g % RINGN, fa);
+    read_frags(g % RINGN, fa, lvc);
     auto lstep = [&](int kt, Frags<WFMT>& cur, Frags<WFMT>& nxt, auto zeroc) __attribute__((always_inline)) {
       __builtin_amdgcn_s_waitcnt(0xC07F);
       __builtin_amdgcn_sched_barrier(0);
       issue_w(cw, kt + 1, nxt);
-      issue(m0, cw, kt + ALEAD + 1, (g + kt + ALEAD + 1) % RINGN);
+      issue(m0, cw, kt + ALEAD + 1, (g + kt + ALEAD + 1) % RINGN, lvc);
       QVIT_STAMP(1);
       stage_sync<2 * XP + WREG>();
       pin(cur);
       QVIT_STAMP(2);
-      step_core(cur, nxt, (g + kt + 1) % RINGN, true, zeroc);
+      step_core(cur, nxt, (g + kt + 1) % RINGN, true, zeroc, lvc);
       QVIT_STAMP(3);
     };
     __builtin_amdgcn_s_waitcnt(0xC07F);
     __builtin_amdgcn_sched_barrier(0);
     issue_w(cw, 1, fb);
-    issue(m0, cw, ALEAD + 1, (g + ALEAD + 1) % RINGN);
+    issue(m0, cw, ALEAD + 1, (g + ALEAD + 1) % RINGN, lvc);
     QVIT_STAMP(1);
     stage_sync<XP + WREG>();
     pin(fa);
     QVIT_STAMP(2);
-    if constexpr (PEEL) step_core(fa, fb, (g + 1) % RINGN, true, std::true_type{});
-    else step_core(fa, fb, (g + 1) % RINGN, true, std::false_type{});
+    if constexpr (PEEL) step_core(fa, fb, (g + 1) % RINGN, true, std::true_type{}, lvc);
+    else step_core(fa, fb, (g + 1) % RINGN, true, std::false_type{}, lvc);
     QVIT_STAMP(3);
     int kt = 1;
     if constexpr (ALEAD & 1) {
@@ -562,15 +605,21 @@
       if constexpr (j < ALEAD) issue_w(cw, tk + 1, nxt);
       constexpr int NW = j < ALEAD ? WREG : 0;
       if (has_next) {
-        issue(nm0, nw, j, (g + nk + j) % RINGN);
-        if constexpr (j < ALEAD) stage_sync<2 * XP + NW>();
-        else asm volatile("s_waitcnt vmcnt(%0)" ::"n"(2 * XP) : "memory");
+        if (TAIL && nshort) {
+          issue(nm0, nw, j, (g + nk + j) % RINGN, TailC{});
+          if constexpr (j < ALEAD) stage_sync<(j == 0 ? XP : XPS) + XPS + NW>();
+          else asm volatile("s_waitcnt vmcnt(%0)" ::"n"(2 * XPS) : "memory");
+        } else {
+          issue(nm0, nw, j, (g + nk + j) % RINGN, FullC{});
+          if constexpr (j < ALEAD) stage_sync<(j == 0 ? XP : XPN) + XPN + NW>();
+          else asm volatile("s_waitcnt vmcnt(%0)" ::"n"(2 * XPN) : "memory");
+        }
       } else {
         if constexpr (j < ALEAD) stage_sync<(j == 0 ? XP : 0) + NW>();
         else asm volatile("s_waitcnt vmcnt(0)" ::: "memory");
       }
       pin(cur);
-      step_core(cur, nxt, (g + tk + 1) % RINGN, j < ALEAD, std::false_type{});
+      step_core(cur, nxt, (g + tk + 1) % RINGN, j < ALEAD, std::false_type{}, lvc);
     };
     if constexpr (ALEAD & 1) {
       tstep(std::integral_constant<int, 0>{}, fa, fb);
@@ -598,51 +647,51 @@
       if (has_bias && wave == 0)
         dma16(ep.bias + n0 + ln * 4, __builtin_amdgcn_readfirstlane(lds0 + RING_B + G::EPI_BYTES));
     }
-    read_frags(g % RINGN, fa);
+    read_frags(g % RINGN, fa, lvc);
     int kt = 0;
     if (PEEL && nk > 2) {
       __builtin_amdgcn_s_waitcnt(0xC07F);
       __builtin_amdgcn_sched_barrier(0);
-      issue(m0, cw, 2, (g + 2) % RINGN);
+      issue(m0, cw, 2, (g + 2) % RINGN, lvc);
       issue_w(cw, 1, fb);
       QVIT_STAMP(1);
       stage_sync<D>();
       pin(fa);
       QVIT_STAMP(2);
-      step_core(fa, fb, (g + 1) % RING, true, std::true_type{});
+      step_core(fa, fb, (g + 1) % RING, true, std::true_type{}, lvc);
       QVIT_STAMP(3);
       __builtin_amdgcn_s_waitcnt(0xC07F);
       __builtin_amdgcn_sched_barrier(0);
-      issue(m0, cw, 3, (g + 3) % RINGN);
+      issue(m0, cw, 3, (g + 3) % RINGN, lvc);
       issue_w(cw, 2, fa);
       QVIT_STAMP(1);
       stage_sync<D>();
       pin(fb);
       QVIT_STAMP(2);
-      step_core(fb, fa, (g + 2) % RING, true, std::false_type{});
+      step_core(fb, fa, (g + 2) % RING, true, std::false_type{}, lvc);
       QVIT_STAMP(3);
       kt = 2;
     }
     for (; kt < nk - 2; kt += 2) {
       __builtin_amdgcn_s_waitcnt(0xC07F);
       __builtin_amdgcn_sched_barrier(0);
-      issue(m0, cw, kt + 2, (g + kt + 2) % RINGN);
+      issue(m0, cw, kt + 2, (g + kt + 2) % RINGN, lvc);
       issue_w(cw, kt + 1, fb);
       QVIT_STAMP(1);
       stage_sync<D>();
       pin(fa);
       QVIT_STAMP(2);
-      step_core(fa, fb, (g + kt + 1) % RING, true, std::false_type{});
+      step_core(fa, fb, (g + kt + 1) % RING, true, std::false_type{}, lvc);
       QVIT_STAMP(3);
       __builtin_amdgcn_s_waitcnt(0xC07F);
       __builtin_amdgcn_sched_barrier(0);
-      issue(m0, cw, kt + 3, (g + kt + 3) % RINGN);
+      issue(m0, cw, kt + 3, (g + kt + 3) % RINGN, lvc);
       issue_w(cw, kt + 2, fa);
       QVIT_STAMP(1);
       stage_sync<D>();
       pin(fb);
       QVIT_STAMP(2);
-      step_core(fb, fa, (g + kt + 2) % RING, true, std::false_type{});
+      step_core(fb, fa, (g + kt + 2) % RING, true, std::false_type{}, lvc);
       QVIT_STAMP(3);
     }
     __builtin_amdgcn_s_waitcnt(0xC07F);
@@ -651,23 +700,23 @@
     const int nm0 = has_next ? tile_m0(tnext) : 0;
     issue_w(cw, nk - 1, fb);
     if (has_next) {
-      issue(nm0, nw, 0, (g + nk) % RINGN);
+      issue(nm0, nw, 0, (g + nk) % RINGN, FullC{});
       stage_sync<D>();
     } else {
       stage_sync<REGW ? WREG : 0>();
     }
     pin(fa);
-    step_core(fa, fb, (g + nk - 1) % RING, true, std::false_type{});
+    step_core(fa, fb, (g + nk - 1) % RING, true, std::false_type{}, lvc);
     __builtin_amdgcn_s_waitcnt(0xC07F);
     __builtin_amdgcn_sched_barrier(0);
     if (has_next) {
-      issue(nm0, nw, 1, (g + nk + 1) % RINGN);
+      issue(nm0, nw, 1, (g + nk + 1) % RINGN, FullC{});
       if constexpr (REGW) asm volatile("s_waitcnt vmcnt(%0)" ::"n"(G::XPIECES) : "memory");
     } else {
       if constexpr (REGW) asm volatile("s_waitcnt vmcnt(0)" ::: "memory");
     }
     pin(fb);
-    step_core(fb, fa, 0, false, std::false_type{});
+    step_core(fb, fa, 0, false, std::false_type{}, lvc);
     QVIT_STAMP(3);
     QVIT_LSTAMP(1);
 
@@ -677,7 +726,7 @@
 #pragma unroll
       for (int r = 0; r < 4; ++r)
 #pragma unroll
-        for (int sr = 0; sr < 8; ++sr)
+        for (int sr = 0; sr < LV; ++sr)
 #pragma unroll
           for (int j = 0; j < 4; ++j) acc[r][sr][j] >>= 4;
     }
@@ -709,9 +758,9 @@
       };
       look(0, 0);
 #pragma unroll
-      for (int sr = 0; sr < 8; ++sr) {
+      for (int sr = 0; sr < LV; ++sr) {
         const int cb = sr & 1;
-        if (sr + 1 < 8) look(sr + 1, cb ^ 1);
+        if (sr + 1 < LV) look(sr + 1, cb ^ 1);
         __builtin_amdgcn_sched_barrier(0);
         const int m = m0 + 128 * wm + 16 * sr + efr;
         uint32_t wd[4];
@@ -741,7 +790,7 @@
       if (has_bias) b4 = *reinterpret_cast<const float4*>(bias_l + (n - n0));
       float* Cf = reinterpret_cast<float*>(C);
       float4 old[2][4];
-      if (m0 + BM <= M && n0 + BN <= N) {
+      if (m0 + 16 * LV <= M && n0 + BN <= N) {
         typedef float f4v __attribute__((ext_vector_type(4)));
         f4v ov0[4], ov1[4];
         auto ld = [&](int sr, f4v (&ov)[4]) __attribute__((always_inline)) {
@@ -758,7 +807,7 @@
             *reinterpret_cast<v4i*>(stg + efr * EPI_LD + 16 * efq + 4 * r) = acc[r][sr];
           __builtin_amdgcn_s_waitcnt(0xC07F);
           __builtin_amdgcn_wave_barrier();
-          if (sr == 0 || sr == 7)
+          if (sr == 0 || sr == LV - 1)
             asm volatile("s_waitcnt vmcnt(4)\n\t; qvit_pin %0 %1 %2 %3"
                          : "+v"(ov[0]), "+v"(ov[1]), "+v"(ov[2]), "+v"(ov[3]) :: "memory");
           else
@@ -777,11 +826,11 @@
         };
         ld(0, ov0);
 #pragma unroll
-        for (int sr = 0; sr < 8; sr += 2) {
-          ld(sr + 1, ov1);
+        for (int sr = 0; sr < LV; sr += 2) {
+          if (sr + 1 < LV) ld(sr + 1, ov1);
           pass(sr, ov0);
-          if (sr + 2 < 8) ld(sr + 2, ov0);
-          pass(sr + 1, ov1);
+          if (sr + 2 < LV) ld(sr + 2, ov0);
+          if (sr + 1 < LV) pass(sr + 1, ov1);
         }
       } else {
       auto load_old = [&](int sr, float4 (&ov)[4]) __attribute__((always_inline)) {
@@ -794,8 +843,8 @@
       };
       load_old(0, old[0]);
 #pragma unroll
-      for (int sr = 0; sr < 8; ++sr) {
-        if (sr + 1 < 8) load_old(sr + 1, old[(sr + 1) & 1]);
+      for (int sr = 0; sr < LV; ++sr) {
+        if (sr + 1 < LV) load_old(sr + 1, old[(sr + 1) & 1]);
         __builtin_amdgcn_s_waitcnt(0xC07F);
 #pragma unroll
         for (int r = 0; r < 4; ++r)
@@ -834,7 +883,7 @@
       for (int j = 0; j < 8; ++j) bb[j] = has_bias ? bias_l[nw - n0 + pcol + j] : 0.f;
       const int64_t pstride = (int64_t)ep.seq * PD;
 #pragma unroll
-      for (int sr = 0; sr < 8; ++sr) {
+      for (int sr = 0; sr < LV; ++sr) {
         __builtin_amdgcn_s_waitcnt(0xC07F);
 #pragma unroll
         for (int r = 0; r < 4; ++r)
@@ -884,7 +933,7 @@
       QParams qp;
       if (I8OUT) qp = *qp_l;
 #pragma unroll
-      for (int sr = 0; sr < 8; ++sr) {
+      for (int sr = 0; sr < LV; ++sr) {
         __builtin_amdgcn_s_waitcnt(0xC07F);
 #pragma unroll
         for (int r = 0; r < 4; ++r)
@@ -958,7 +1007,23 @@
       ln_after_tile(m0);
       QVIT_STAMP(6);
     }
-    if (!has_next) break;
+  };
+  for (;;) {
+    tnext = t + team;
+    has_next_rt = tnext < hi;
+    if constexpr (TAIL) {
+      const bool is_short = t >= ntiles;
+      next_short = !is_short && !has_next_rt && tail_t >= 0;
+      if (next_short) {
+        tnext = tail_t;
+        has_next_rt = true;
+      }
+      if (is_short) run_tile(TailC{});
+      else run_tile(FullC{});
+    } else {
+      run_tile(FullC{});
+    }
+    if (!has_next_rt) break;
     t = tnext;
     g += nk;
   }
@@ -971,6 +1036,53 @@
 #define QVIT_GEMM_L2 1
 #endif
 constexpr bool GEMM_L2 = QVIT_GEMM_L2 != 0;
+
+struct TailMap {
+  int frb;
+  int h;
+  int trb;
+};
+
+constexpr int TAIL_HEIGHTS[] = {64, 80, 96, 112};
+
+TailMap tail_map(int64_t M, int64_t ntn, int64_t slots, int64_t ncu) {
+  const int64_t rb = (M + 127) / 128;
+  TailMap m{(int)rb, 0, 0};
+  if (M <= 0 || ntn <= 0 || slots <= 0 || ncu <= 0) return m;
+  const int64_t frb = (rb * ntn / slots) * slots / ntn;
+  const int64_t rest = M - frb * 128;
+  if (rest <= 0) return m;
+  int64_t h = 16;
+  while (h < 128 && (rest + h - 1) / h * ntn > ncu) h += 16;
+  for (const int s : TAIL_HEIGHTS)
+    if (h <= s) {
+      m.frb = (int)frb;
+      m.h = s;
+      m.trb = (int)((rest + s - 1) / s);
+      return m;
+    }
+  return m;
+}
+
+struct TailEnv {
+  bool on;
+  int64_t slots, cus;
+};
+
+const TailEnv& tail_env() {
+  static const TailEnv env = [] {
+    auto num = [](const char* name) -> int64_t {
+      const char* v = std::getenv(name);
+      const long n = v ? std::strtol(v, nullptr, 10) : 0;
+      return n > 0 ? n : 0;
+    };
+    const char* t = std::getenv("QVIT_GEMM_TAIL");
+    return TailEnv{!(t && t[0] == '0' && t[1] == 0), num("QVIT_GEMM_TAIL_SLOTS"), num("QVIT_GEMM_TAIL_CUS")};
+  }();
+  return env;
+}
+
+constexpr bool tail_kernel(int epi, int rw) { return rw != 0 && epi == QVIT_EPI_F32_RESID; }
 
 template <int WFMT, int EPI, int RW = 0>
 int launch(const int8_t* A, int64_t M, int64_t K, int64_t lda, const void* Wp, int64_t N, int64_t npad,
@@ -995,14 +1107,35 @@
       epc.ln_cnt = ep.ln_cnt + m0 / G::BM;
       epc.ln_codes = ep.ln_codes + m0 * ep.ln_ldc;
     }
-    if (RW != 0 && K / BK >= ALEAD + 2 && GEMM_L2)
+    const bool l2 = RW != 0 && K / BK >= ALEAD + 2 && GEMM_L2;
+    bool launched = false;
+    if constexpr (tail_kernel(EPI, RW)) {
+      const TailEnv& env = tail_env();
+      if (l2 && env.on) {
+        const TailMap tm = tail_map(mc, npad / BN, env.slots ? env.slots : grid, env.cus ? env.cus : qvit_device_cus());
+        auto go = [&](auto tlc) {
+          hipLaunchKernelGGL((gemm_kernel<WFMT, EPI, WMV, RW, RW != 0, decltype(tlc)::value>), dim3((unsigned)grid),
+                             dim3(G::NT), 0, stream, A + m0 * lda, (int)mc, (int)K, lda,
+                             reinterpret_cast<const int8_t*>(Wp), (int)N, (int)npad, Cc, ldc, tm.frb, epc);
+          launched = true;
+        };
+        if (tm.h != 0 && ((int64_t)tm.trb * (npad / BN) + 7) / 8 <= grid / 8) {
+          if (tm.h == 64) go(std::integral_constant<int, 4>{});
+          else if (tm.h == 80) go(std::integral_constant<int, 5>{});
+          else if (tm.h == 96) go(std::integral_constant<int, 6>{});
+          else if (tm.h == 112) go(std::integral_constant<int, 7>{});
+        }
+      }
+    }
+    if (launched) {
+    } else if (l2)
       hipLaunchKernelGGL((gemm_kernel<WFMT, EPI, WMV, RW, RW != 0>), dim3((unsigned)grid), dim3(G::NT), 0, stream,
                          A + m0 * lda, (int)mc, (int)K, lda, reinterpret_cast<const int8_t*>(Wp), (int)N, (int)npad, Cc,
-                         ldc, epc);
+                         ldc, 0, epc);
     else
       hipLaunchKernelGGL((gemm_kernel<WFMT, EPI, WMV, RW>), dim3((unsigned)grid), dim3(G::NT), 0, stream,
                          A + m0 * lda, (int)mc, (int)K, lda, reinterpret_cast<const int8_t*>(Wp), (int)N, (int)npad, Cc,
-                         ldc, epc);
+                         ldc, 0, epc);
     const hipError_t e = hipGetLastError();
     if (e != hipSuccess) return qvit_hip_status(e);
   }
@@ -1043,6 +1176,17 @@
                      epilogue == QVIT_EPI_I8_GELU ? 1 : 0, out_qtype, out_d, out_qm, out_t, out_levels,
                      -(v_lo * (1.0f / w)), 1.0f / w, (int)nb, reinterpret_cast<int8_t*>(table));
   return qvit_launch_status();
+}
+
+extern "C" int qvit_gemm_tail_map(int64_t M, int64_t npad, int64_t slots, int64_t cus, int32_t* map3) {
+  if (!map3) return QVIT_ENULL;
+  if (M <= 0 || M > INT32_MAX / 2 || npad <= 0 || npad % BN || npad > INT32_MAX / 2 || slots <= 0 || cus <= 0)
+    return QVIT_EINVAL;
+  const TailMap m = tail_map(M, npad / BN, slots, cus);
+  map3[0] = m.frb;
+  map3[1] = m.h;
+  map3[2] = m.trb;
+  return QVIT_OK;
 }
 
 extern "C" int qvit_pack_weight_w4r(const void* packed, int64_t npad, int64_t kpad, void* out, hipStream_t stream) {
diff --git a/quantized_vit_amd/csrc/qvit_common.h b/quantized_vit_amd/csrc/qvit_common.h
--- a/quantized_vit_amd/csrc/qvit_common.h
+++ b/quantized_vit_amd/csrc/qvit_common.h
@@ -217,6 +217,22 @@
       : "memory");
 }
 
+QVIT_DEV void dma16s_masked(const void* sbase, uint32_t voff, uint32_t lds_base, uint64_t mask) {
+  uint32_t keep;
+  uint64_t keepx;
+  asm volatile(
+      "s_mov_b32 %0, m0\n\t"
+      "s_mov_b32 m0, %4\n\t"
+      "s_mov_b64 %1, exec\n\t"
+      "s_mov_b64 exec, %5\n\t"
+      "global_load_lds_dwordx4 %2, %3\n\t"
+      "s_mov_b64 exec, %1\n\t"
+      "s_mov_b32 m0, %0"
+      : "=&s"(keep), "=&s"(keepx)
+      : "v"(voff), "s"(sbase), "s"(lds_base), "s"(mask)
+      : "memory");
+}
+
 static inline int qvit_hip_status(hipError_t e) {
   return e == hipSuccess ? QVIT_OK : (QVIT_EHIP - (int)e);
 }
```

After: 34730 img/s, median of 6. Within noise of the previous version (+0.4%).
